# moyun/deneva

Measured on AMD Instinct MI355X. Metric: OCC-validated txns/sec, YCSB theta=0.9, higher is better.
Workload: dtype u64; 1 GPU; YCSB OCC epoch validation, 1048576 txns x 16 keys, zipf theta=0.9, 16,777,216-key table, 50% RO txns, 50% WR tuples; global_batch=1048576, keys_per_txn=16, parallelism=single GPU

## Files before the change

### deneva_amd/_abi.py

```python
from __future__ import annotations

import ctypes as C
import os

_HERE = os.path.dirname(os.path.abspath(__file__))
LIB_PATH = os.environ.get("DENEVA_AMD_LIB") or os.path.join(_HERE, "libdcc.so")

DCC_OK = 0
DCC_EIO = -5
DCC_ENOMEM = -12
DCC_ENODEV = -19
DCC_EINVAL = -22
DCC_ERANGE = -34
DCC_ECOMM = -70
DCC_ENOTSUP = -95

RD, WR, XP, SCAN = 0, 1, 2, 3
RC_RCOK, RC_ABORT, RC_WAIT = 0, 2, 3
KEY_RESERVED = 0xFFFFFFFFFFFFFFFF
GROUP_NONE = 0xFFFFFFFF
ACCESS_NONE = 0xFFFFFFFF
VTS_BASE, VTS_NONE = 0, 0xFFFFFFFFFFFFFFFF
DEVICE_PTRS = 0x1
OCC_APPEND_HISTORY = 0x2
OCC_DEFER_FINISH = 0x8
KEYS_U32 = 0x10
ACCTYPE_2BIT = 0x20
TN_U32 = 0x40
SHARD_SELF = 0x80
MAAT_READ_AND_PREWRITE = 0x4
ROW_NONE = 0xFFFFFFFFFFFFFFFF
UNIQUE_ID_BYTES = 128
EXCHANGE_FN = C.CFUNCTYPE(C.c_int, C.c_void_p, C.POINTER(C.c_uint8), C.c_uint64)
BACKOFF_REFERENCE, BACKOFF_NONE, BACKOFF_EXP = 0, 1, 2
ABORTQ_SORT_FULL = 0x1
LOCK_EX, LOCK_SH = 0, 1
WD_RUN, WD_GONE = 0x10, 0x11
OPT_RECHECK = 1
OPT_BATCH_MAX = 2
OPT_SOLVER = 5
OPT_SWEEP_LEVELS = 6
OPT_HIST_MERGE = 7
OPT_FAIL_RANK = 8
OPT_RO_SPLIT = 10
OPT_PIPELINE = 11
OPT_CALVIN_PATH = 12
OPT_COMM_SOLO = 13
OPT_PIPE_PARTITION = 14
OPT_PIPE_CHAIN = 15


class Batch(C.Structure):
    _fields_ = [
        ("n_txn", C.c_uint64),
        ("nnz", C.c_uint64),
        ("offsets", C.c_void_p),
        ("keys", C.c_void_p),
        ("acctype", C.c_void_p),
        ("start_tn", C.c_void_p),
        ("finish_tn", C.c_void_p),
        ("order", C.c_void_p),
        ("flags", C.c_uint32),
        ("reserved", C.c_uint32),
    ]


class Snapshot(C.Structure):
    _fields_ = [
        ("hist_top", C.c_void_p),
        ("active_off", C.c_void_p),
        ("active_idx", C.c_void_p),
    ]


class CalvinHeld(C.Structure):
    _fields_ = [("n", C.c_uint64), ("keys", C.c_void_p), ("acctype", C.c_void_p)]


class SelectOut(C.Structure):
    _fields_ = [
        ("cap_txn", C.c_uint64),
        ("cap_nnz", C.c_uint64),
        ("txn_base", C.c_uint64),
        ("nnz_base", C.c_uint64),
        ("offsets", C.c_void_p),
        ("keys", C.c_void_p),
        ("acctype", C.c_void_p),
        ("start_tn", C.c_void_p),
        ("finish_tn", C.c_void_p),
        ("order", C.c_void_p),
        ("src", C.c_void_p),
    ]


class WaitdieCarryArgs(C.Structure):
    _fields_ = [
        ("batch", C.POINTER(Batch)),
        ("ts", C.c_void_p),
        ("rc", C.c_void_p),
        ("pos", C.c_void_p),
        ("revive", C.c_void_p),
        ("src_in", C.c_void_p),
        ("fresh", C.POINTER(Batch)),
        ("fresh_ts", C.c_void_p),
        ("fresh_src_base", C.c_uint32),
        ("out", C.POINTER(SelectOut)),
        ("out_ts", C.c_void_p),
        ("out_rc", C.c_void_p),
        ("out_pos", C.c_void_p),
    ]


class AbortqParams(C.Structure):
    _fields_ = [
        ("cap_txn", C.c_uint64),
        ("cap_nnz", C.c_uint64),
        ("penalty", C.c_uint64),
        ("penalty_max", C.c_uint64),
        ("policy", C.c_uint32),
        ("flags", C.c_uint32),
    ]


class LocktabParams(C.Structure):
    _fields_ = [("cap_rows", C.c_uint64), ("flags", C.c_uint32), ("reserved", C.c_uint32)]


class Stats(C.Structure):
    _fields_ = [
        ("rounds", C.c_uint32),
        ("n_shards", C.c_uint32),
        ("n_commit", C.c_uint64),
        ("n_abort", C.c_uint64),
        ("n_readonly", C.c_uint64),
        ("nnz_w", C.c_uint64),
        ("alg_bytes", C.c_uint64),
        ("device_ms", C.c_double),
        ("total_ms", C.c_double),
        ("phase_ms", C.c_double * 4),
        ("phase_bytes", C.c_uint64 * 4),
        ("peel_prefix", C.c_uint64),
        ("n_survivors", C.c_uint64),
        ("fallback", C.c_uint32),
        ("fin_where", C.c_uint32),
    ]

    def as_dict(self) -> dict:
        out = {}
        for name, _ in self._fields_:
            v = getattr(self, name)
            out[name] = list(v) if name.startswith("phase_") else v
        return out


class YcsbParams(C.Structure):
    _fields_ = [
        ("n_txn", C.c_uint64),
        ("req_per_query", C.c_uint32),
        ("part_cnt", C.c_uint32),
        ("table_size", C.c_uint64),
        ("zipf_theta", C.c_double),
        ("txn_write_perc", C.c_double),
        ("tup_write_perc", C.c_double),
        ("part_per_txn", C.c_uint32),
        ("strict_ppt", C.c_uint32),
        ("first_part_local", C.c_uint32),
        ("chunk_txns", C.c_uint32),
        ("seed", C.c_uint64),
        ("n_threads", C.c_uint32),
        ("reserved", C.c_uint32),
    ]


class TpccParams(C.Structure):
    _fields_ = [
        ("n_txn", C.c_uint64),
        ("num_wh", C.c_uint32),
        ("part_cnt", C.c_uint32),
        ("perc_payment", C.c_double),
        ("wh_update", C.c_uint32),
        ("max_items", C.c_uint32),
        ("cust_per_dist", C.c_uint32),
        ("dist_per_wh", C.c_uint32),
        ("max_items_per_txn", C.c_uint32),
        ("part_per_txn", C.c_uint32),
        ("mpr", C.c_double),
        ("first_part_local", C.c_uint32),
        ("chunk_txns", C.c_uint32),
        ("seed", C.c_uint64),
        ("n_threads", C.c_uint32),
        ("reserved", C.c_uint32),
    ]


class FileInfo(C.Structure):
    _fields_ = [
        ("version", C.c_uint32),
        ("kind", C.c_uint32),
        ("sections", C.c_uint32),
        ("reserved", C.c_uint32),
        ("n_txn", C.c_uint64),
        ("nnz", C.c_uint64),
# ... 170 lines not shown
```

### deneva_amd/csrc/dcc_ctx.h

```cpp
#pragma once
#include <hip/hip_runtime.h>

#include <algorithm>
#include <chrono>
#include <cstring>
#include <memory>
#include <string>
#include <utility>
#include <vector>

#include "dcc.h"
#include "occ_history.h"

namespace dcc {
struct SwShard;
struct Slot;
}

struct dcc_ctx;


struct DevBuf {
  void* p = nullptr;
  size_t cap = 0;
// ... 15 lines not shown
    return *this;
  }
  ~DevBuf() { release(); }
  int ensure(dcc_ctx* c, size_t bytes, const char* what);
  void release();
};

struct RowTab {
  const char* name;
  DevBuf buf, ctl;
  uint32_t bits = 0;
  uint64_t rows = 0;
  uint32_t mask() const { return (uint32_t)((1ull << bits) - 1); }
  uint64_t size() const { return rows; }
  template <class P>
  int reserve(dcc_ctx* ctx, uint64_t want);
  int clear(dcc_ctx* ctx);
  template <class P>
  int set(dcc_ctx* ctx, const uint64_t* keys, const uint64_t* a, const uint64_t* b, uint64_t n);
  template <class P>
  int get(dcc_ctx* ctx, const uint64_t* keys, uint64_t* a, uint64_t* b, uint64_t n);
};

struct SegWork {
  static constexpr uint64_t TILE = 1024;
  static constexpr uint32_t C_WORDS = 84;
  static constexpr size_t AGG_BYTES = 40;
  DevBuf misc;
  DevBuf stp;
  DevBuf arec;
  DevBuf k[2], v[2];
  DevBuf stxn, sinfo, sts;
  DevBuf agg;
  DevBuf tdone;
  int reserve(dcc_ctx* ctx, uint64_t n, uint64_t nnz);
};

struct DevBatch {
  uint64_t n = 0, nnz = 0;
  const uint32_t* off = nullptr;
  const uint64_t* keys = nullptr;
  const uint8_t* acctype = nullptr;
  const uint64_t* start_tn = nullptr;
  const uint64_t* finish_tn = nullptr;
  const uint64_t* order = nullptr;
};

struct dcc_comm_state;
struct dcc_multi;

struct HistStore {
  DevBuf fk, ft;
  DevBuf skey, stn, hash;
  DevBuf bm;
  DevBuf nx, tcnt;
  uint64_t m = 0;
  uint32_t hbits = 0;
  bool built = true;
  bool mono = true;
  uint64_t max_tn = 0;
  uint64_t min_tn = ~0ull;
  uint64_t max_key = 0;
  bool chained = false;
  bool overflowed = false;
  uint64_t last_app = 0;
  void reset() {
    m = 0;
    built = false;
    mono = true;
    max_tn = 0;
    min_tn = ~0ull;
    max_key = 0;
  }
};

struct SubProb {
  uint64_t n = 0, nnz = 0, w_bound = 0;
  const uint32_t* off = nullptr;
  const uint64_t* keys = nullptr;
  const uint8_t* acctype = nullptr;
  uint8_t* state = nullptr;
  uint8_t* hasw = nullptr;
  bool hasw_global = false;
};
struct PeelInfo {
  uint64_t prefix = 0, survivors = 0;
};
struct SubBufs {
  DevBuf tid, off, keys, acctype, state;
};

struct dcc_abortq {
  dcc_ctx* owner = nullptr;
  dcc_abortq_params P{};
  struct Pool {
    DevBuf off, keys, at, src, cnt, due;
  } pool[2];
  DevBuf sk[2], sv[2], scratch;
  DevBuf ctl, part;
  DevBuf st_cnt, st_out;
  int cur = 0;
  uint64_t n = 0, nnz = 0;
  uint64_t seq = 0;
  uint64_t due_lo = ~0ull;
};

struct dcc_locktab {
  dcc_ctx* owner = nullptr;
  dcc_locktab_params P{};
  DevBuf tab[2];
  DevBuf ctl;
  DevBuf st_keys, st_type, st_cnt;
  DevBuf st_rc;
  int cur = 0;
  uint64_t n_slots = 0;
  uint64_t slots_used = 0;
  uint64_t rows_held = 0;
  uint64_t holds = 0;
  uint64_t rebuilds = 0;
  double pass_ms[3] = {};
  bool rebuilt = false;
};

struct LtEpoch {
  uint64_t n = 0;
  const uint32_t* off = nullptr;
  const uint64_t* keys = nullptr;
  const uint8_t* at = nullptr;
  const uint32_t* sid = nullptr;
  const uint8_t* state = nullptr;
  dcc::Slot* tab = nullptr;
  uint32_t lp = 0;
  const uint32_t* err = nullptr;
  unsigned grid = 1;
};

struct dcc_ctx {
  int device = 0;
  int n_cu = 256;
  hipStream_t own_stream = nullptr;
  hipStream_t stream = nullptr;
  hipEvent_t ev0 = nullptr, ev1 = nullptr;
  bool profiling = false;
  uint64_t recheck_max = 16384;
  uint32_t batch_max = 8;
  bool bars_used = false;
  int solver = 0;
  bool use_sweep() const { return solver != 1; }
  bool ro_split = true;
  bool ro_on = false;
  uint32_t wt_bits = 18;
  uint32_t wf_bits = 0;
  uint32_t sw_levels = 0;
  uint32_t sw_mode = 1;
  uint32_t sw_l1_last = ~0u;
  bool sw_debug = false;
  hipEvent_t pev[8] = {};
  std::string last_error;
  void* hmisc = nullptr;
  void* hpart = nullptr;
  struct GraphKey {
    const void *off, *keys, *acc;
    uint64_t n, nnz;
    const void* out_rc;
    bool dev_out;
    uint32_t levels;
    uint64_t gen;
    const void *start_tn, *finish_tn, *out_tn;
    uint32_t fin;
    bool operator==(const GraphKey& o) const {
      return off == o.off && keys == o.keys && acc == o.acc && n == o.n && nnz == o.nnz &&
             out_rc == o.out_rc && dev_out == o.dev_out && levels == o.levels && gen == o.gen &&
             start_tn == o.start_tn && finish_tn == o.finish_tn && out_tn == o.out_tn && fin == o.fin;
    }
  };
  hipGraphExec_t graph_exec = nullptr;
  struct CvGraphKey {
    const void *off, *keys, *acc, *order, *grp, *rc;
    uint64_t n, nnz, gen;
    uint32_t ulen, have_seq, bucket;
    uint8_t kp[112], op[112];
  };
  hipGraphExec_t cv_graph_exec = nullptr;
  CvGraphKey cv_graph_key{}, cv_seen_key{};
  bool cv_seen = false;
  bool cv_last_sorted = false, cv_last_bucket = false;
  uint64_t cv_spec_miss = 0;
  GraphKey graph_key{};
  uint64_t buf_gen = 0;
  void* hmisc_dev = nullptr;
  void* hpart_dev = nullptr;
  void* hdyn = nullptr;
  void* hdyn_dev = nullptr;
  static constexpr size_t HDYN_TOTALS = 256, HDYN_BYTES = 512;

  DevBuf misc;
  DevBuf part;
  DevBuf off, keys, acctype, start_tn, finish_tn, order;
  DevBuf nar_keys, nar_at, nar_tn;
  DevBuf table;
  DevBuf state, hasw, rc, stat;
  DevBuf cflag, bsum, tn;
  DevBuf dyn, fin_part;
  DevBuf gst;
  DevBuf hasw_scr;
  DevBuf sw_ctl, sw_status, sw_ckeys, sw_dbg;
  DevBuf sw_rec, sw_rk, sw_gtab, sw_fw, sw_aent, sw_mg;
  DevBuf sw_rflag, sw_ro, sw_wtab, sw_cw, sw_wtab_big;
  DevBuf sw_xcnt, sw_xsend, sw_xrec, sw_mcnt, sw_moff, sw_mkeys, sw_mat, sw_kill;
  SubBufs sw_list[2];
  DevBuf l_tid[2], l_coff[2], l_cent[2];
  HistStore hs[2];
  uint64_t hist_merge_min = 65536;
  DevBuf h_K[2], h_V[2], h_scr, h_bsum;
  DevBuf h_bm;
  bool h_bm_stale = true;
  uint32_t fin_tag = 0;
  DevBuf perm, calvin_a, calvin_b, calvin_c, calvin_d;
  DevBuf cv_scratch, cv_agg, cv_group, cv_wave, cv_pgx, cv_gsx, cv_gsize, cv_done, cv_maxl, cv_cwmax, cv_cwpos, cv_cwmark, cv_cwhot, cv_cwpa, cv_cwoa, cv_cwhelp, cv_cwrec2;
  DevBuf cv_seq_b, cv_ok, cv_len, cv_off2, cv_tsum;
  DevBuf held_keys, held_at;
  DevBuf cb_e, cb_out, cb_cnt, cb_small;
  DevBuf snap_top, snap_aoff, snap_aidx, snap_cnt;
  RowTab mt_rows{"maat"};
  uint64_t mt_new_last = 0;
  uint64_t mt_full_redo = 0;
  DevBuf mt_misc, mt_slot, mt_sval, mt_slot2, mt_sval2, mt_sfl, mt_stx, mt_txn, mt_agg;
  DevBuf mt_sflB, mt_stxB, mt_k1, mt_tcnt, mt_ul;
  DevBuf mt_lb;
  DevBuf mt_ptab;
  uint32_t mt_tag = 0;
  DevBuf ix_keys, ix_ord, ix_rows, ix_cnt, wv_buf, ix_scr, wv_hbuf, wv_obuf;
  DevBuf nw_misc, nw_sid, nw_list, nw_conf;
  DevBuf sel_misc, sel_part, sel_rc, sel_src, sel_out;
  std::vector<std::unique_ptr<dcc_abortq>> abortqs;
  uint32_t ix_bits = 0;
  uint64_t ix_nkeys = 0, ix_nrows = 0;
  double ix_last_ms = 0;
  uint64_t tnc = 0;

  dcc_comm_state* comm = nullptr;
  dcc_multi* multi = nullptr;
  int comm_ranks() const;
  bool sharded() const;
  bool comm_solo = false;
  int comm_allreduce_max_u8(uint8_t* dev, uint64_t n);
  int comm_allgather_u8(const uint8_t* send, uint8_t* recv, uint64_t bytes);
  int comm_rank() const;

  int fail(int code, const char* fmt, ...);
  int hip_fail(hipError_t e, const char* what);
  int reserve_occ(uint64_t n, uint64_t nnz, uint64_t nnz_w, uint32_t tw);
  void list_geometry(uint64_t n, uint32_t tw, uint64_t& seg_ts, uint64_t& seg_es) const;
  static uint64_t table_capacity(uint64_t nnz_w);
  uint64_t hist_size() const { return hs[0].m + hs[1].m; }
  int hist_grow_flat(HistStore& h, uint64_t need);
  dcc::HistInsert hist_insert_args(HistStore& h);
  void hist_note(HistStore& h, uint64_t lo_tn, uint64_t hi_tn);
  int hist_build(HistStore& h);
  int hist_prepare();
  dcc::HistView hist_view() const;
  int hist_append_epoch(const DevBatch& d, const uint64_t* tn_dev, uint64_t nnz_w, uint64_t n_cw);
  int check_batch(const dcc_batch* b, bool scan_offsets = true);
  int stage_batch(const dcc_batch* b, DevBatch& d);
  template <typename T>
  int stage(DevBuf& buf, const T* src, size_t bytes, bool dev, const char* what, const T*& out) {
    if (dev) {
      out = src;
      return DCC_OK;
    }
    if (int e = buf.ensure(this, bytes, what)) return e;
    if (bytes) {
      const hipError_t he = hipMemcpyAsync(buf.p, src, bytes, hipMemcpyHostToDevice, stream);
      if (he != hipSuccess) return hip_fail(he, what);
    }
    out = (const T*)buf.p;
    return DCC_OK;
  }
  int stage_held(const dcc_calvin_held* held, bool dev, const uint64_t*& keys, const uint8_t*& at);
  int device_prep(const DevBatch& d, uint32_t& maxlen, uint64_t& nnz_w, uint64_t p = 0,
                  uint64_t* nnz_w_prefix = nullptr);
  int read_partials(size_t bytes);
  int occ_epoch(const dcc_batch* b, uint8_t* out_rc, uint64_t* out_tn, dcc_stats* st);
  struct OccRun {
    uint64_t n_txn = 0;
    uint32_t flags = 0;
    uint8_t* out_rc = nullptr;
    uint64_t* out_tn = nullptr;
    DevBatch d;
    bool sh = false, dev_out = false, defer = false, sweep = false, want_tn = false;
    bool app = false, hist_on = false;
    bool whole = false;
    DevBatch full;
    bool replay = false, capturing = false, pending = false, active = false;
    uint32_t glv = 0, maxlen = 0, rounds = 0, handoffs = 0;
    uint64_t nnz_w = 0;
    int next_level = 0, serial_tail = -1;
    uint8_t* rc_dev = nullptr;
    uint32_t* cf = nullptr;
    uint64_t* tn_dev = nullptr;
    PeelInfo info;
    GraphKey gkey{};
    dcc_stats S;
    double t_wall0 = 0;
    uint64_t n_cw = 0;
    uint32_t fin_runs = 0;
    bool fin_later = false;
  };
  OccRun run;
  int occ_begin(const dcc_batch* b, uint8_t* out_rc, uint64_t* out_tn, bool async, bool fin_later = false);
  int pipe_finish(dcc_ctx* l, bool chained = false);
  int chain_enqueue(dcc_ctx* l, uint64_t seq, hipEvent_t after, bool reset);
  int chain_set(dcc_ctx* l, uint64_t seq);
  int chain_accept(dcc_ctx* l);
  uint64_t hist_room() const;
  DevBuf fin_ctl;
  DevBuf fdyn;
  void* hfin = nullptr;
  void* hfin_dev = nullptr;
  hipEvent_t ev_done = nullptr;
  uint32_t pipe_chain = 1;
  int occ_end(dcc_stats* st);
  int occ_final(bool async);
  struct OccPipe* pipe = nullptr;
  uint32_t pipe_lanes = 3;
  uint32_t pipe_part = 0;
// ... 155 lines not shown
```

### deneva_amd/csrc/dcc_ctx.hip

```cpp
#include <hip/hip_runtime.h>

#include <algorithm>
#include <chrono>
#include <cstdarg>
#include <cstdio>
#include <cstring>
#include <string>
#include <vector>

#include "dcc.h"
#include "dcc_ctx.h"
#include "dcc_env.h"
#include "radix_sort.h"
#include "dcc_device.h"
#include "occ_kernels.h"

using namespace dcc;

int dcc_ctx::fail(int code, const char* fmt, ...) {
  char buf[512];
  va_list ap;
  va_start(ap, fmt);
  vsnprintf(buf, sizeof buf, fmt, ap);
  va_end(ap);
// ... 56 lines not shown
  int n = 0;
  if (hipGetDeviceCount(&n) != hipSuccess) {
    (void)hipGetLastError();
    return 0;
  }
  int g = 0;
  for (int i = 0; i < n; i++) {
    hipDeviceProp_t p;
    if (hipGetDeviceProperties(&p, i) == hipSuccess && strncmp(p.gcnArchName, "gfx950", 6) == 0) g++;
  }
  return g;
}

extern "C" int dcc_version(void) { return 100; }

extern "C" const char* dcc_strerror(int code) {
  switch (code) {
    case DCC_OK: return "success";
    case DCC_EIO: return "HIP runtime failure";
    case DCC_ENOMEM: return "out of memory";
    case DCC_ENODEV: return "no usable gfx950 device";
    case DCC_EINVAL: return "invalid argument or malformed batch";
    case DCC_ERANGE: return "size exceeds an engine limit";
    case DCC_ECOMM: return "RCCL communicator failure";
    case DCC_ENOTSUP: return "not supported";
    default: return "unknown error";
  }
}

extern "C" const char* dcc_last_error(const dcc_ctx* ctx) {
  return ctx ? ctx->last_error.c_str() : "null context";
}

extern "C" int dcc_init(dcc_ctx** out, int device_id) {
  if (!out) return DCC_EINVAL;
  *out = nullptr;
  int ndev = 0;
  if (hipGetDeviceCount(&ndev) != hipSuccess || ndev == 0) {
    (void)hipGetLastError();
    return DCC_ENODEV;
  }
  if (device_id < 0) {
    if (hipGetDevice(&device_id) != hipSuccess) return DCC_ENODEV;
  }
  if (device_id >= ndev) return DCC_ENODEV;
  hipDeviceProp_t prop;
  if (hipGetDeviceProperties(&prop, device_id) != hipSuccess) return DCC_ENODEV;
  if (strncmp(prop.gcnArchName, "gfx950", 6) != 0) return DCC_ENODEV;
  if (hipSetDevice(device_id) != hipSuccess) return DCC_ENODEV;
  dcc_ctx* ctx = new dcc_ctx();
  ctx->device = device_id;
  ctx->n_cu = prop.multiProcessorCount;
  CK(hipStreamCreateWithFlags(&ctx->own_stream, hipStreamNonBlocking));
  ctx->stream = ctx->own_stream;
  CK(hipEventCreate(&ctx->ev0));
  CK(hipEventCreate(&ctx->ev1));
  for (auto& e : ctx->pev) CK(hipEventCreate(&e));
  CK(hipHostMalloc((void**)&ctx->hmisc, 16384, hipHostMallocDefault));
  CK(hipHostMalloc((void**)&ctx->hpart, 1 << 17, hipHostMallocDefault));
  CK(hipHostGetDevicePointer(&ctx->hmisc_dev, ctx->hmisc, 0));
  CK(hipHostGetDevicePointer(&ctx->hpart_dev, ctx->hpart, 0));
  ctx->hs[1].chained = true;
  CK(hipHostMalloc((void**)&ctx->hdyn, dcc_ctx::HDYN_BYTES, hipHostMallocDefault));
  CK(hipHostGetDevicePointer(&ctx->hdyn_dev, ctx->hdyn, 0));
  memset(ctx->hdyn, 0, dcc_ctx::HDYN_BYTES);
  int rc = ctx->misc.ensure(ctx, 16384, "misc");
  if (!rc) rc = ctx->part.ensure(ctx, 1 << 17, "partials");
  if (!rc && (hipMemset(ctx->misc.p, 0, 16384) != hipSuccess ||
              hipMemset(ctx->part.p, 0, 1 << 17) != hipSuccess))
    rc = DCC_EIO;
  if (rc) {
    dcc_destroy(ctx);
    return rc;
  }
  *out = ctx;
  return DCC_OK;
}

extern "C" void dcc_destroy(dcc_ctx* ctx) {
  if (!ctx) return;
  dcc_pipe_destroy(ctx);
  ctx->abortqs.clear();
  ctx->locktabs.clear();
  dcc_multi_destroy(ctx);
  (void)hipSetDevice(ctx->device);
  if (ctx->stream) (void)hipStreamSynchronize(ctx->stream);
  if (ctx->graph_exec) (void)hipGraphExecDestroy(ctx->graph_exec);
  if (ctx->cv_graph_exec) (void)hipGraphExecDestroy(ctx->cv_graph_exec);
  dcc_comm_destroy(ctx);
  if (ctx->hmisc) (void)hipHostFree(ctx->hmisc);
  if (ctx->hpart) (void)hipHostFree(ctx->hpart);
  if (ctx->hdyn) (void)hipHostFree(ctx->hdyn);
  if (ctx->hfin) (void)hipHostFree(ctx->hfin);
  if (ctx->ev_done) (void)hipEventDestroy(ctx->ev_done);
  if (ctx->ev0) (void)hipEventDestroy(ctx->ev0);
  if (ctx->ev1) (void)hipEventDestroy(ctx->ev1);
  for (auto& e : ctx->pev)
    if (e) (void)hipEventDestroy(e);
  if (ctx->own_stream) (void)hipStreamDestroy(ctx->own_stream);
  delete ctx;
}

extern "C" int dcc_set_profiling(dcc_ctx* ctx, int enable) {
  if (!ctx) return DCC_EINVAL;
  if (ctx->multi)
    for (int r = 0; r < dcc_multi_size(ctx); r++) dcc_multi_sub(ctx, r)->profiling = enable != 0;
  ctx->profiling = enable != 0;
  return DCC_OK;
}

int dcc_multi_set_fail_rank(dcc_ctx* ctx, int rank);

extern "C" int dcc_set_option(dcc_ctx* ctx, int option, int64_t value) {
  if (!ctx) return DCC_EINVAL;
  if (option == DCC_OPT_FAIL_RANK) {
    if (!ctx->multi) return ctx->fail(DCC_EINVAL, "DCC_OPT_FAIL_RANK: multi-GPU contexts only");
    return dcc_multi_set_fail_rank(ctx, (int)value);
  }
  if (option == DCC_OPT_PIPELINE) {
    if (value < 1 || value > 8) return DCC_EINVAL;
    dcc_pipe_drain(ctx);
    ctx->pipe_lanes = (uint32_t)value;
    return DCC_OK;
  }
  if (option == DCC_OPT_PIPE_PARTITION) {
    if (value != 0 && value != 1) return DCC_EINVAL;
    dcc_pipe_drain(ctx);
    ctx->pipe_part = (uint32_t)value;
    return DCC_OK;
  }
  if (option == DCC_OPT_PIPE_CHAIN) {
    if (value != 0 && value != 1) return DCC_EINVAL;
    dcc_pipe_drain(ctx);
    ctx->pipe_chain = (uint32_t)value;
    return DCC_OK;
  }
  if (ctx->multi)
    for (int r = 0; r < dcc_multi_size(ctx); r++) {
      const int e = dcc_set_option(dcc_multi_sub(ctx, r), option, value);
      if (e != DCC_OK) return e;
    }
  switch (option) {
    case DCC_OPT_RECHECK:
      if (value < 0) return DCC_EINVAL;
      ctx->recheck_max = (uint64_t)value;
      return DCC_OK;
    case DCC_OPT_SOLVER:
      if (value != 0 && value != 1 && value != 3) return DCC_EINVAL;
      ctx->solver = (int)value;
      return DCC_OK;
    case DCC_OPT_SWEEP_LEVELS:
      if (value < 0 || value > SW_MAX_LEVEL) return DCC_EINVAL;
      ctx->sw_levels = (uint32_t)value;
      return DCC_OK;
    case DCC_OPT_RO_SPLIT:
      if (value != 0 && value != 1 && (value < 4 || value > 24)) return DCC_EINVAL;
      ctx->ro_split = value != 0;
      ctx->wt_bits = value >= 4 ? (uint32_t)value : WT_BITS_DEFAULT;
      return DCC_OK;
    case DCC_OPT_HIST_MERGE:
      if (value < 1) return DCC_EINVAL;
      ctx->hist_merge_min = (uint64_t)value;
      return DCC_OK;
    case DCC_OPT_CALVIN_PATH:
      if (value < 0 || value > 2) return DCC_EINVAL;
      ctx->cv_path = (int)value;
      return DCC_OK;
    case DCC_OPT_COMM_SOLO:
      if (value != 0 && value != 1) return DCC_EINVAL;
      if (ctx->comm) return ctx->fail(DCC_EINVAL, "DCC_OPT_COMM_SOLO: set before dcc_comm_init");
      ctx->comm_solo = value != 0;
      return DCC_OK;
    case DCC_OPT_BATCH_MAX:
      if (value < 1 || value > 32) return DCC_EINVAL;
      ctx->batch_max = (uint32_t)value;
      return DCC_OK;
    default: return DCC_EINVAL;
  }
}

extern "C" int dcc_set_stream(dcc_ctx* ctx, void* s) {
  if (!ctx) return DCC_EINVAL;
  if (ctx->multi) return ctx->fail(DCC_ENOTSUP, "multi-GPU context: one stream per sub-context");
  ctx->stream = s ? (hipStream_t)s : ctx->own_stream;
  return DCC_OK;
}

extern "C" int dcc_reserve(dcc_ctx* ctx, uint64_t max_txn, uint64_t max_nnz) {
  if (!ctx) return DCC_EINVAL;
  if (ctx->multi)
    for (int r = 0; r < dcc_multi_size(ctx); r++) {
      const int e = dcc_reserve(dcc_multi_sub(ctx, r), max_txn, max_nnz);
      if (e != DCC_OK) return e;
    }
  (void)hipSetDevice(ctx->device);
  const uint32_t tw = ROUND_CAP / MAX_TXN_LEN;
  int rc = ctx->state.ensure(ctx, max_txn + 16, "state");
  if (!rc) rc = ctx->hasw.ensure(ctx, max_txn + 16, "hasw");
  if (!rc) rc = ctx->rc.ensure(ctx, max_txn + 16, "rc");
  if (!rc) rc = ctx->nowait_reserve(max_txn, max_nnz, true);
  if (!rc) rc = ctx->select_reserve(max_txn, max_nnz);
  if (!rc) rc = ctx->tso_reserve(max_txn, max_nnz, true);
  if (!rc) rc = ctx->mvcc_reserve(max_txn, max_nnz, true, true);
  if (!rc) rc = ctx->waitdie_reserve(max_txn, max_nnz, true);
  if (!rc) rc = ctx->carry_reserve(max_txn, max_nnz);
  if (rc) return rc;
  return ctx->reserve_occ(max_txn, max_nnz, max_nnz, tw);
}

int dcc_ctx::hist_grow_flat(HistStore& h, uint64_t need) {
  dcc_ctx* ctx = this;
  if (need * 8 <= h.fk.cap && need * 8 <= h.ft.cap && (!h.chained || need * 4 <= h.nx.cap)) return DCC_OK;
  if (h.chained && need >= HIST_NIL) return fail(DCC_ENOMEM, "history delta level of %llu pairs",
                                                 (unsigned long long)need);
  const uint64_t want = std::max<uint64_t>(need + need / 2, 4096);
  for (DevBuf* b : {&h.fk, &h.ft, &h.nx}) {
    if (b == &h.nx && !h.chained) continue;
    const uint64_t w = b == &h.nx ? 4 : 8;
    DevBuf nb;
    CR(nb.ensure(this, want * w, "history pairs"));
    if (h.m) CK(hipMemcpyAsync(nb.p, b->p, h.m * w, hipMemcpyDeviceToDevice, stream));
    CK(hipStreamSynchronize(stream));
    *b = std::move(nb);
  }
  return DCC_OK;
}

void dcc_ctx::hist_note(HistStore& h, uint64_t lo_tn, uint64_t hi_tn) {
  if (lo_tn < h.max_tn) h.mono = false;
  h.max_tn = std::max(h.max_tn, hi_tn);
  h.min_tn = std::min(h.min_tn, lo_tn);
  h.built = false;
}

int dcc_ctx::hist_build(HistStore& h) {
  dcc_ctx* ctx = this;
  if (h.built) return DCC_OK;
  h_bm_stale = true;
  if (h.m == 0 && !h.chained) {
    h.built = true;
    h.mono = true;
    return DCC_OK;
  }
  static const uint64_t slots_per_pair = [] {
    const char* e = DCC_ENV("DCC_HIST_SLOTS");
    return e && atoi(e) >= 2 ? (uint64_t)atoi(e) : 4ull;
  }();
  uint64_t need = slots_per_pair * h.m;
  if (h.chained)
    need = std::max<uint64_t>({need, 65536,
                               4 * (std::max<uint64_t>(hist_merge_min, hs[0].m / 4) + h.last_app)});
  if (h.overflowed) need = std::max<uint64_t>(need, 4ull << h.hbits);
  h.hbits = 4;
  while ((1ull << h.hbits) < need) h.hbits++;
  const uint64_t mm = std::max<uint64_t>(h.m, 1);
  CR(h.skey.ensure(this, mm * 8, "history keys"));
  CR(h.stn.ensure(this, mm * 8, "history tns"));
  CR(h.hash.ensure(this, 32ull << h.hbits, "history table"));
  CR(h.tcnt.ensure(this, 16, "history table overflow flag"));
  CR(h.bm.ensure(this, (1u << HIST_BM_LOG) / 8, "history key bitmap"));
  CK(hipMemsetAsync(h.tcnt.p, 0, 16, stream));
  if (h.m == 0) {
    CK(hipMemsetAsync(h.hash.p, 0xFF, 32ull << h.hbits, stream));
    CK(hipMemsetAsync(h.bm.p, 0, (1u << HIST_BM_LOG) / 8, stream));
    h.built = true;
    h.mono = true;
    h.overflowed = false;
    return DCC_OK;
  }
  for (int q = 0; q < 2; q++) {
    CR(h_K[q].ensure(this, h.m * 8, "history sort keys"));
    CR(h_V[q].ensure(this, h.m * 4, "history sort values"));
  }
  CR(h_scr.ensure(this, rs_scratch_words(h.m) * 4, "history sort scratch"));
  HistBuild b{h.m,
              (const uint64_t*)h.fk.p,
              (const uint64_t*)h.ft.p,
              h.mono,
              {(uint64_t*)h_K[0].p, (uint64_t*)h_K[1].p},
              {(uint32_t*)h_V[0].p, (uint32_t*)h_V[1].p},
              (uint32_t*)h_scr.p,
              (uint64_t*)h.skey.p,
              (uint64_t*)h.stn.p,
              (uint64_t*)h.hash.p,
              h.hbits,
              h.max_key ? 64u - (uint32_t)__builtin_clzll(h.max_key) : 1u,
              64u - (uint32_t)__builtin_clzll(h.max_tn | 1ull),
              (uint32_t*)h.tcnt.p};
  if (hist_build_level(b, stream)) CK(hipGetLastError());
  launch_hist_bm((const uint64_t*)h.fk.p, h.m, (uint32_t*)h.bm.p, stream);
  CK(hipGetLastError());
  CK(hipMemcpyAsync(hmisc, h.tcnt.p, 4, hipMemcpyDeviceToHost, stream));
  CK(hipStreamSynchronize(stream));
  if (*(const uint32_t*)hmisc) {
    h.overflowed = true;
    return hist_build(h);
  }
  h.overflowed = false;
  h.built = true;
  return DCC_OK;
}

HistInsert dcc_ctx::hist_insert_args(HistStore& h) {
  return HistInsert{(const uint64_t*)h.fk.p, (const uint64_t*)h.ft.p, (uint64_t*)h.hash.p,
                    (uint32_t*)h.nx.p, (uint32_t*)h.bm.p, (uint32_t*)h_bm.p, (uint32_t*)h.tcnt.p,
                    h.hbits, 0u};
// ... 410 lines not shown
```

### deneva_amd/csrc/occ_driver.hip

```cpp
#include <hip/hip_runtime.h>

#include <algorithm>
#include <chrono>
#include <cstdio>
#include <cstdlib>
#include <cstring>
#include <vector>

#include "dcc.h"
#include "dcc_ctx.h"
#include "dcc_device.h"
#include "dcc_env.h"
#include "occ_kernels.h"

using namespace dcc;

static uint64_t next_pow2(uint64_t x) {
  uint64_t p = 1;
  while (p < x) p <<= 1;
  return p;
}

uint64_t dcc_ctx::table_capacity(uint64_t nnz_w) {
  return std::max<uint64_t>(1024, next_pow2(nnz_w + nnz_w / 4 + 1));
// ... 88 lines not shown
  BuildArgs ba{sp.n, tw_b, sp.off, sp.keys, sp.acctype, tab, mask, sp.state, sp.hasw, err};
  if (prof) CK(hipEventRecord(pev[0], stream));
  launch_build(ba, (unsigned)n_cu * 16, stream);
  CK(hipGetLastError());
  if (sh && sp.hasw_global) CR(comm_allreduce_max_u8(sp.hasw, sp.n));
  if (prof) CK(hipEventRecord(pev[1], stream));

  int cur = 0;
  uint32_t rt = 1;
  uint32_t k = 0;
  uint64_t m_bound = sp.n;
  uint32_t rounds = 0;
  const unsigned max_grid = (unsigned)n_cu * 8;
  const unsigned resident_grid = (unsigned)n_cu * 4;
  uint32_t batch = std::min<uint32_t>(sp.n > 65536 ? 2 : 4, batch_max);
  bool done = false;
  while (!done) {
    const uint32_t k0 = k;
    for (uint32_t q = 0; q < batch; q++, k++) {
      const bool first = k == 0;
      const unsigned long long* prev = first ? nullptr : &ring[((k - 1) % CTR_RING) * NSEG];
      if (!first) {
        PubArgs pa;
        pa.m_in = prev;
        pa.tw = tw;
        pa.kill_flag = sh ? one : &kflag[(k - 1) % CTR_RING];
        pa.force = 0;
        pa.state = sp.state;
        if (rt > MAX_ROUND_TAG) {
          launch_retag(tab, cap, stream);
          rt = 1;
          pa.kill_flag = one;
          pa.force = 1;
        }
        pa.r = rt;
        pa.tid = (const uint32_t*)l_tid[cur].p;
        pa.coff = (const uint32_t*)l_coff[cur].p;
        pa.cent = (const uint64_t*)l_cent[cur].p;
        pa.seg_ts = seg_ts;
        pa.seg_es = seg_es;
        pa.tab = tab;
        pa.err = err;
        launch_pub(pa, m_bound, (unsigned)n_cu * 2, stream);
      }
      RoundArgs ra;
      ra.m_in = prev;
      ra.m = sp.n;
      ra.tw = tw;
      ra.r = rt;
      ra.k = k + 1;
      ra.end_total = 0;
      ra.tid = first ? nullptr : (const uint32_t*)l_tid[cur].p;
      ra.coff = first ? sp.off : (const uint32_t*)l_coff[cur].p;
      ra.keys = sp.keys;
      ra.acctype = sp.acctype;
      ra.cent = first ? nullptr : (const uint64_t*)l_cent[cur].p;
      ra.seg_ts = seg_ts;
      ra.seg_es = seg_es;
      ra.tab = tab;
      ra.mask = mask;
      ra.state = sp.state;
      ra.tid_out = (uint32_t*)l_tid[cur ^ 1].p;
      ra.coff_out = (uint32_t*)l_coff[cur ^ 1].p;
      ra.cent_out = (uint64_t*)l_cent[cur ^ 1].p;
      ra.ctr = &ring[(k % CTR_RING) * NSEG];
      ra.ctr_zero = &ring[((k + 1) % CTR_RING) * NSEG];
      ra.kill_flag = &kflag[k % CTR_RING];
      ra.kill_zero = &kflag[(k + 1) % CTR_RING];
      const bool recheck = !sh && !first && m_bound <= recheck_max;
      ra.bar = recheck ? (GridBar*)(bars + (k % CTR_RING) * 16) : nullptr;
      bars_used |= recheck;
      ra.bar_zero = (uint32_t*)(bars + ((k + 1) % CTR_RING) * 16);
      ra.gst = gstat;
      ra.err = err;
      launch_round(ra, first, m_bound, recheck ? resident_grid : max_grid, stream);
      if (sh) {
        CR(comm_allreduce_max_u8(gstat, sp.n));
        launch_decide(sp.state, gstat, sp.n, st_abort(k + 1), &und[k % CTR_RING],
                      &und[(k + 1) % CTR_RING], stream);
      }
      if (prof && first) CK(hipEventRecord(pev[2], stream));
      cur ^= 1;
      rt++;
    }
    CK(hipGetLastError());
    CK(hipMemcpyAsync(hmisc, ring, CTR_RING * NSEG * 8, hipMemcpyDeviceToHost, stream));
    if (sh) CK(hipMemcpyAsync((char*)hmisc + MISC_UND, und, CTR_RING * 4, hipMemcpyDeviceToHost, stream));
    CK(hipStreamSynchronize(stream));
    const unsigned long long* hr = (const unsigned long long*)hmisc;
    const uint32_t* hu = (const uint32_t*)((const char*)hmisc + MISC_UND);
    for (uint32_t q = k0; q < k; q++) {
      uint64_t mq = 0;
      for (uint32_t g = 0; g < NSEG; g++) mq += hr[(q % CTR_RING) * NSEG + g] >> CTR_E_BITS;
      if (sh ? hu[q % CTR_RING] == 0 : mq == 0) {
        rounds = q + 1;
        done = true;
        break;
      }
      m_bound = mq;
    }
    if (!done && k > sp.n + 2) return fail(DCC_EIO, "fixed point did not converge");
    batch = std::min<uint32_t>(batch * 2, batch_max);
  }
  if (prof) CK(hipEventRecord(pev[4], stream));
  rounds_out = rounds;
  return DCC_OK;
}

static constexpr size_t SW_PREP_OFF = 32768;
static constexpr size_t SW_HCTL = 13312;
static constexpr uint32_t SW_PMAX_TOP = 65536;
static uint32_t sw_pmax(int level, int mode) {
  static const std::vector<uint32_t> ov = [] {
    std::vector<uint32_t> v;
    if (const char* e = DCC_ENV("DCC_SW_PMAX"))
      for (const char* c = e; *c;) {
        char* x;
        const unsigned long p = strtoul(c, &x, 10);
        if (x == c) break;
        v.push_back((uint32_t)std::min<unsigned long>(std::max<unsigned long>(p, SW_T), SW_PMAX_TOP));
        c = *x ? x + 1 : x;
      }
    return v;
  }();
  if (level < (int)ov.size()) return ov[level];
  if (mode == 2) {
    if (level == 0) return 1024u;
    return level >= 4 ? SW_PMAX_TOP : (8192u << (level - 1));
  }
  if (mode) {
    if (level == 0) return 1024u;
    if (level == 1) return 3072u;
    return level >= 5 ? SW_PMAX_TOP : (8192u << (level - 2));
  }
  return level >= 6 ? SW_PMAX_TOP : (1024u << level);
}
static size_t sw_ctl_bytes() { return (SW_MAX_LEVEL + 2) * sizeof(SwLevel) + 64; }
static uint32_t sw_budget_bits(int level, int mode) {
  uint32_t b = 12;
  while (b < SW_GBITS_MAX && (1ull << b) < 4ull * sw_pmax(level, mode) * 16) b++;
  return b;
}
static uint32_t sw_budget(int level, int mode) { return 1u << (sw_budget_bits(level, mode) - 2); }
static uint32_t sw_gbits(int level, int mode) {
  static const int ov = [] {
    const char* c = DCC_ENV("DCC_SW_GBITS");
    return c ? atoi(c) : 0;
  }();
  uint32_t b = ov > 0 ? (uint32_t)ov : (level == 0 ? 18u : 19u);
  b = std::max(b, sw_budget_bits(level, mode));
  return std::min<uint32_t>(b, SW_GBITS_MAX);
}

int dcc_ctx::sweep_reserve(const DevBatch& d) {
  const uint64_t tiles = SW_PMAX_TOP / SW_T;
  sw_debug = DCC_ENV("DCC_SW_DEBUG") != nullptr;
  if (sw_debug) {
    CR(sw_dbg.ensure(this, (4096 + 4 * 256 * 8 + 4 * 64 * 8) * 8, "sweep debug"));
    dcc_ctx* ctx = this;
    CK(hipMemsetAsync(sw_dbg.p, 0, (4096 + 4 * 256 * 8 + 4 * 64 * 8) * 8, stream));
  }
  CR(sw_ctl.ensure(this, sw_ctl_bytes(), "sweep control"));
  CR(sw_status.ensure(this, ((d.n + 63) / 64 + 64) * 16 + (4ull * n_cu + 64) * 8,
                        "sweep survivor bits + tile counts"));
  CR(sw_ckeys.ensure(this, ((1ull << SW_GBITS_MAX) / 32 + (1ull << SW_BLOOM_LOG) / 32) * 4 +
                                (1ull << SW_GBITS_MAX) * 8,
                     "sweep committed set"));
  CR(sw_rec.ensure(this, tiles * sizeof(SwRec), "sweep tile records"));
  CR(sw_rk.ensure(this, tiles * SW_OVF * 4, "sweep tile-list overflow"));
  CR(sw_gtab.ensure(this, 2 * (1ull << SW_GBITS_MAX) * 8, "sweep key tables"));
  CR(sw_fw.ensure(this, 2 * (1ull << SW_GBITS_MAX) * 4, "sweep first writer / last accessor"));
  CR(sw_aent.ensure(this, 2 * (1ull << (SW_GBITS_MAX - 1)) * 4, "sweep access entries"));
  CR(sw_mg.ensure(this, SW_PMAX_TILES * 8, "sweep tile commit masks"));
  if (ro_on) {
    const uint64_t n64 = (d.n + 63) / 64 + 32;
    CR(sw_rflag.ensure(this, (2 * n64 + 4ull * n_cu + 64) * 8, "sweep read-only survivor bits"));
    CR(sw_ro.ensure(this, d.n * sizeof(RoEnt) + 64, "sweep read-only list"));
    CR(sw_wtab.ensure(this, sizeof(WrSlot) << wt_bits, "committed-writer table"));
    CR(sw_cw.ensure(this, d.n * 4 + 64, "committed writers"));
  }
  for (SubBufs& b : sw_list) {
    CR(b.tid.ensure(this, d.n * 4 + 16, "sweep list tid"));
    CR(b.off.ensure(this, (d.n + 1) * 4 + 16, "sweep list offsets"));
    CR(b.keys.ensure(this, std::max<uint64_t>(8, d.nnz * 8), "sweep list keys"));
    CR(b.acctype.ensure(this, std::max<uint64_t>(16, d.nnz), "sweep list acctype"));
    CR(b.state.ensure(this, d.n + 16, "sweep list state"));
  }
  return DCC_OK;
}

int dcc_ctx::sweep_enqueue(const DevBatch& d, int l0, int l1, const SwShard* shl, bool resume,
                           bool tail_serial) {
  dcc_ctx* ctx = this;
  SwLevel* ctl = (SwLevel*)sw_ctl.p;
  uint32_t* abandon = (uint32_t*)(ctl + SW_MAX_LEVEL + 1);
  uint32_t* err = (uint32_t*)misc.p;
  const uint32_t n = (uint32_t)d.n;
  static const unsigned fgrid_ov = [] {
    const char* e = DCC_ENV("DCC_SW_FGRID");
    return e ? (unsigned)atoi(e) : 0u;
  }();
  const unsigned fgrid = fgrid_ov ? fgrid_ov : (unsigned)std::max<uint64_t>(1, 4ull * n_cu);
  static const unsigned fgrid1_ov = [] {
    const char* e = DCC_ENV("DCC_SW_FGRID1");
    return e ? (unsigned)atoi(e) : 0u;
  }();
  uint64_t* gtab0 = (uint64_t*)sw_gtab.p;
  uint32_t* cbits_d = (uint32_t*)sw_ckeys.p;
  uint32_t* bloom_d = cbits_d + (1u << SW_GBITS_MAX) / 32;
  uint64_t* ckeys_d = (uint64_t*)(bloom_d + (1u << SW_BLOOM_LOG) / 32);
  const uint64_t n64 = (d.n + 63) / 64;
  uint64_t* sflag_d = (uint64_t*)sw_status.p;
  unsigned long long* tcount_d = (unsigned long long*)(sflag_d + n64 + 32);
  unsigned long long* bsum_d = tcount_d + n64 + 32;
  const bool ros = ro_on && (!shl || shl->full_off);
  const int rmode = ros ? (int)sw_mode : 0;
  uint32_t* const wctl = abandon;
  for (int l = l0; l < l1; l++) {
    const bool top = l == 0;
    SwList in;
    if (top) {
      in = SwList{nullptr, d.off, d.keys, d.acctype, d.nnz};
    } else {
      const SubBufs& b = sw_list[(l - 1) & 1];
      in = SwList{(const uint32_t*)b.tid.p, (const uint32_t*)b.off.p, (const uint64_t*)b.keys.p,
                  (const uint8_t*)b.acctype.p, d.nnz};
    }
    SubBufs& out = sw_list[l & 1];
    SwLevel* lv = ctl + l;
    const uint32_t* mdev = top ? nullptr : &lv->m;
    const uint32_t pmax = sw_pmax(l, rmode);
    const uint64_t tiles = (std::min<uint64_t>(pmax, d.n) + SW_T - 1) / SW_T;
    uint32_t* fw = (uint32_t*)sw_fw.p;
    uint32_t* la = fw + (1u << SW_GBITS_MAX);
    uint32_t* aent = (uint32_t*)sw_aent.p;
    uint32_t* apos = aent + (1u << (SW_GBITS_MAX - 1));
    const SwList sin = shl ? shl->serial : in;
    const uint32_t* smdev = shl ? shl->m_dev : mdev;
    const uint32_t sm_host = (shl && !shl->m_dev) ? shl->P : n;
    SwPreArgs pa{sin, smdev, sm_host, pmax, top ? (const uint8_t*)state.p : nullptr,
                 (SwRec*)sw_rec.p, (uint32_t*)sw_rk.p,
                 gtab0 + (size_t)(l & 1) * (1ull << SW_GBITS_MAX), sw_gbits(l, rmode),
                 sw_budget(l, rmode), fw, la, aent, apos, abandon, err, nullptr};
    if (sw_debug && l < 4) pa.dbg = (uint64_t*)sw_dbg.p + 4096 + 4 * 256 * 8 + (size_t)l * 64 * 8;
    const bool serial_part = !(resume && l == l0);
    if (serial_part) {
      launch_sw_pre(pa, (unsigned)tiles, stream);
      launch_sw_rows(pa, (unsigned)tiles, stream);
    }
    SwSeqArgs sa{smdev, sm_host, pmax, top ? 1 : 0, (const SwRec*)sw_rec.p, (const uint32_t*)sw_rk.p,
                 gtab0 + (size_t)(l & 1) * (1ull << SW_GBITS_MAX), sw_gbits(l, rmode),
                 (uint8_t*)state.p, (uint8_t*)hasw.p,
                 cbits_d, ckeys_d, bloom_d, lv, lv + 1, (uint32_t*)out.off.p, (uint64_t*)sw_mg.p,
                 abandon, err, nullptr};
    if (sw_debug && l < 4) sa.dbg = (uint64_t*)sw_dbg.p + (size_t)l * 1024;
    if (ros) {
      sa.cw_list = (uint32_t*)sw_cw.p;
      sa.cw_count = wctl + 4;
    }
    if (serial_part) launch_sw_seq(sa, stream);
    if (tail_serial && l == l1 - 1) break;
    SwCoutArgs ca{sin,     aent,    apos,    (const uint64_t*)sw_mg.p, lv, cbits_d, ckeys_d,
                  bloom_d, abandon, smdev, sm_host, shl ? 0 : 1};
    if (top && serial_part) {
      const bool whole = shl && shl->full_off;
      ca.prep_off = whole ? shl->full_off : d.off;
      ca.prep_n = d.n;
      ca.prep_at = whole ? shl->full_at : d.acctype;
      ca.prep_nnz = whole ? shl->full_nnz : d.nnz;
      ca.prep_part = (PrepPart*)((char*)hpart_dev + SW_PREP_OFF);
      ca.hasw = (uint8_t*)hasw.p;
      ca.prep_err = err;
      if (ros) {
        ca.wclear = (uint4*)sw_wtab.p;
        ca.wclear_n16 = (sizeof(WrSlot) << wt_bits) / 16;
      }
    }
    launch_sw_cout(ca, (unsigned)std::min<uint64_t>((pa.budget + 1023) / 1024, 4ull * n_cu), stream);
    SwFilterArgs fa;
    fa.in = in;
    fa.m_dev = mdev;
    fa.m_host = n;
    fa.cand_state = top ? 1 : 0;
    fa.level = (uint32_t)l;
    fa.gtab = gtab0 + (size_t)(l & 1) * (1ull << SW_GBITS_MAX);
    fa.gbits = sw_gbits(l, rmode);
    fa.cbits = cbits_d;
    fa.bloom = bloom_d;
    fa.ckeys = ckeys_d;
    fa.sflag = sflag_d;
    fa.tcount = tcount_d;
    fa.bsum = bsum_d;
    const unsigned lgrid = (!top && fgrid1_ov) ? std::min(fgrid1_ov, fgrid) : fgrid;
    fa.nblocks = lgrid;
    fa.lv = lv;
    fa.lv_next = lv + 1;
    fa.state = (uint8_t*)state.p;
    fa.hasw = (uint8_t*)hasw.p;
    fa.tid_out = (uint32_t*)out.tid.p;
    fa.off_out = (uint32_t*)out.off.p;
    fa.keys_out = (uint64_t*)out.keys.p;
    fa.acc_out = (uint8_t*)out.acctype.p;
    fa.abandon = abandon;
    fa.abandon_out = abandon;
    fa.abandon_min = 65536;
    fa.abandon_num = top ? 1 : 3;
    fa.abandon_den = 4;
    fa.gclear = gtab0 + (size_t)((l + 1) & 1) * (1ull << SW_GBITS_MAX);
    fa.gclear_n = 1ull << sw_gbits(l + 1, rmode);
    fa.fw_clear = fw;
    fa.la_clear = la;
    fa.err = err;
    fa.dbg = (sw_debug && l < 4) ? (uint64_t*)sw_dbg.p + 4096 + (size_t)l * 256 * 8 : nullptr;
    fa.cdbg = pa.dbg ? pa.dbg + 32 : nullptr;
    fa.kill_out = shl ? shl->kill_out : nullptr;
    fa.kill_in = shl ? shl->kill_all : nullptr;
    fa.kill_ranks = shl ? (uint32_t)comm_ranks() : 0u;
    fa.kill_stride = shl ? shl->kill_words : 0u;
    fa.ro_split = (ros && top) ? 1 : 0;
    fa.rflag = (uint64_t*)sw_rflag.p;
    fa.rtcount = (unsigned long long*)(fa.rflag + n64 + 32);
    fa.rbsum = fa.rtcount + n64 + 32;
    fa.ro_out = (RoEnt*)sw_ro.p;
    fa.ro_count = wctl + 2;
    if (top && profiling) CK(hipEventRecord(pev[1], stream));
    launch_sw_filter(fa, lgrid, stream);
    if (top && profiling) CK(hipEventRecord(pev[2], stream));
    if (shl) {
      CR(comm_allgather_u8((const uint8_t*)shl->kill_out, (uint8_t*)shl->kill_all, shl->kill_words * 8));
      if (top && !shl->full_off) CR(comm_allreduce_max_u8((uint8_t*)hasw.p, d.n));
      launch_sw_apply(fa, lgrid, stream);
    }
    launch_sw_compact(fa, lgrid, stream);
  }
  CK(hipGetLastError());
  return DCC_OK;
}

int dcc_ctx::sweep_sharded(const DevBatch& d, int& next_level) {
  dcc_ctx* ctx = this;
  const int R = comm_ranks(), me = comm_rank();
  SwLevel* ctl = (SwLevel*)sw_ctl.p;
  const uint32_t* abandon = (const uint32_t*)(ctl + SW_MAX_LEVEL + 1);
  CR(sw_xcnt.ensure(this, 64ull * R + 64, "sweep exchange counts"));
  for (int l = 0; l < SW_MAX_LEVEL - 1; l++) {
    next_level = l;
    const bool top = l == 0;
    SwList in;
    if (top) {
      in = SwList{nullptr, d.off, d.keys, d.acctype, d.nnz};
    } else {
      const SubBufs& b = sw_list[(l - 1) & 1];
      in = SwList{(const uint32_t*)b.tid.p, (const uint32_t*)b.off.p, (const uint64_t*)b.keys.p,
                  (const uint8_t*)b.acctype.p, d.nnz};
    }
    uint32_t* cnt = (uint32_t*)sw_xcnt.p;
    CK(hipMemsetAsync(cnt, 0, 4ull * (R + 2), stream));
    launch_sw_share(top ? nullptr : &ctl[l].m, (uint32_t)d.n, abandon, top ? d.off : in.off,
                    sw_pmax(l, 0), (uint32_t)me, cnt, stream);
    CR(comm_allreduce_max_u8((uint8_t*)cnt, 4ull * (R + 2)));
    std::vector<uint32_t> hc(R + 2);
    CK(hipMemcpyAsync(hc.data(), cnt, 4ull * (R + 2), hipMemcpyDeviceToHost, stream));
    CK(hipStreamSynchronize(stream));
    const uint32_t m = hc[0];
    if (hc[1]) return DCC_OK;
    if (m == 0) return DCC_OK;
    const uint32_t P = std::min<uint32_t>(sw_pmax(l, 0), m);
    const uint32_t* share = hc.data() + 2;
    uint64_t total = 0, before = 0;
    for (int r = 0; r < R; r++) {
      if (r < me) before += share[r];
      total += share[r];
    }
    uint32_t maxshare = 0;
    for (int r = 0; r < R; r++) maxshare = std::max(maxshare, share[r]);
    const uint64_t chunk = std::max<uint64_t>(1, maxshare) * 12;
    CR(sw_xsend.ensure(this, chunk, "sweep exchange send"));
    CR(sw_xrec.ensure(this, chunk * R, "sweep exchange records"));
    CR(sw_mcnt.ensure(this, 8ull * (P + 1) + 64, "sweep merge counts"));
    CR(sw_moff.ensure(this, 4ull * (P + 1) + 64, "sweep merged offsets"));
    CR(sw_mkeys.ensure(this, std::max<uint64_t>(64, total * 8), "sweep merged keys"));
    CR(sw_mat.ensure(this, std::max<uint64_t>(64, total), "sweep merged types"));
    const uint64_t kw = (m + 63) / 64 + 1;
    CR(sw_kill.ensure(this, kw * 8 * (R + 1) + 64, "sweep kill bits"));
    uint32_t* xrec = (uint32_t*)sw_xrec.p;
    uint32_t* mcnt = (uint32_t*)sw_mcnt.p;
    CK(hipMemsetAsync(sw_xsend.p, 0xFF, chunk, stream));
    CK(hipMemsetAsync(mcnt, 0, 4ull * (P + 1), stream));
    launch_sw_merge(in, P, (uint32_t*)sw_xsend.p, 0, 0, nullptr, nullptr, nullptr, nullptr,
                    nullptr, true, stream);
    CR(comm_allgather_u8((const uint8_t*)sw_xsend.p, (uint8_t*)xrec, chunk));
    (void)before;
    launch_sw_merge(in, P, xrec, 0, (uint32_t)(R * (chunk / 12)), mcnt, mcnt + (P + 1),
                    (uint32_t*)sw_moff.p, (uint64_t*)sw_mkeys.p, (uint8_t*)sw_mat.p, false, stream);
    CK(hipGetLastError());
    SwShard shl{};
    shl.serial = SwList{top ? nullptr : in.tid, (const uint32_t*)sw_moff.p,
                        (const uint64_t*)sw_mkeys.p, (const uint8_t*)sw_mat.p, total};
    shl.P = P;
    shl.kill_out = (uint64_t*)sw_kill.p;
    shl.kill_all = (uint64_t*)sw_kill.p + kw;
    shl.kill_words = kw;
    CR(sweep_enqueue(d, l, l + 1, &shl));
  }
  next_level = SW_MAX_LEVEL - 1;
  return DCC_OK;
}


int dcc_ctx::sweep_sharded_full(const DevBatch& d, const DevBatch& full, int l0, int L) {
  dcc_ctx* ctx = this;
  const int R = comm_ranks();
  SwLevel* ctl = (SwLevel*)sw_ctl.p;
  uint32_t* err = (uint32_t*)misc.p;
  uint64_t cap = d.n, wmax = 0;
  std::vector<uint64_t> words(std::max(L, 1));
  for (int l = 0; l < L; l++) {
    words[l] = (cap + 63) / 64 + 1;
    wmax = std::max(wmax, words[l]);
    cap = std::min<uint64_t>(cap, std::max<uint64_t>(65536, l == 0 ? (cap + 3) / 4 : (cap * 3 + 3) / 4));
  }
  CR(sw_kill.ensure(this, wmax * 8 * (R + 1) + 64, "sweep kill bits"));
  const uint32_t pm = sw_pmax(SW_MAX_LEVEL - 1, ro_on ? (int)sw_mode : 0);
  CR(sw_moff.ensure(this, 4ull * (std::min<uint64_t>(pm, d.n) + 1) + 64, "sweep serial offsets"));
  CR(sw_mkeys.ensure(this, 8ull * std::min<uint64_t>(pm, d.n) * MAX_TXN_LEN + 64, "sweep serial keys"));
  CR(sw_mat.ensure(this, std::min<uint64_t>(pm, d.n) * MAX_TXN_LEN + 64, "sweep serial types"));
  for (int l = l0; l < L; l++) {
    SwShard shl{};
    if (l == 0) {
      shl.serial = SwList{nullptr, full.off, full.keys, full.acctype, full.nnz};
      shl.P = (uint32_t)d.n;
    } else {
      const SubBufs& b = sw_list[(l - 1) & 1];
      launch_sw_sgather((const uint32_t*)b.tid.p, &ctl[l].m, sw_pmax(l, ro_on ? (int)sw_mode : 0), full.off, full.keys,
                        full.acctype, full.nnz, (uint32_t*)sw_moff.p, (uint64_t*)sw_mkeys.p,
                        (uint8_t*)sw_mat.p, err, stream);
      CK(hipGetLastError());
      shl.serial = SwList{(const uint32_t*)b.tid.p, (const uint32_t*)sw_moff.p, (const uint64_t*)sw_mkeys.p,
                          (const uint8_t*)sw_mat.p, std::min<uint64_t>(pm, d.n) * MAX_TXN_LEN};
      shl.m_dev = &ctl[l].m;
    }
    shl.kill_out = (uint64_t*)sw_kill.p;
    shl.kill_all = (uint64_t*)sw_kill.p + wmax;
    shl.kill_words = words[l];
    shl.full_off = full.off;
    shl.full_at = full.acctype;
    shl.full_nnz = full.nnz;
// ... 218 lines not shown
    HistStore& D = hs[1];
    if (tot[1] > d.nnz) return fail(DCC_EIO, "history append: %llu writes > %llu accesses",
                                    (unsigned long long)tot[1], (unsigned long long)d.nnz);
    if (tot[1]) {
      D.m += tot[1];
      D.max_key = std::max<uint64_t>(D.max_key, tot[2]);
      D.last_app = tot[1];
      const bool b = D.built;
      hist_note(D, tnc + 1, tnc + r.n_cw);
      D.built = b;
    }
    if (tot[3]) {
      D.overflowed = true;
      D.built = false;
    }
  }
  tnc += r.n_cw;
  return DCC_OK;
}

int dcc_ctx::chain_set(dcc_ctx* l, uint64_t seq) {
  dcc_ctx* ctx = this;
  CR(fin_ctl.ensure(this, sizeof(FinCtl), "chained finish control"));
  launch_fin_ctl_set((FinCtl*)fin_ctl.p, tnc, hs[1].m, seq, l->stream);
  CK(hipGetLastError());
  return DCC_OK;
}

int dcc_ctx::sweep_ro(const DevBatch& d0, bool big, bool scan, uint64_t nnz_w, const DevBatch* full) {
  const DevBatch& d = full ? *full : d0;
  dcc_ctx* ctx = this;
  uint32_t* wctl = (uint32_t*)((SwLevel*)sw_ctl.p + SW_MAX_LEVEL + 1);
  WrTab wt{(WrSlot*)sw_wtab.p, wt_bits, WT_PROBES, wctl + 1};
  if (big) {
    uint32_t bits = 10;
    while (bits < 31 && (1ull << bits) < 2 * std::max<uint64_t>(nnz_w, 1)) bits++;
    CR(sw_wtab_big.ensure(this, sizeof(WrSlot) << bits, "committed-writer fallback table"));
    CK(hipMemsetAsync(sw_wtab_big.p, 0xFF, sizeof(WrSlot) << bits, stream));
    wt = WrTab{(WrSlot*)sw_wtab_big.p, bits, 1u << bits, wctl + 3};
  }
  SwWallArgs wa{d.n, d.off, d.keys, d.acctype, d.nnz, (const uint8_t*)state.p,
                (const uint8_t*)hasw.p, scan ? nullptr : (const uint32_t*)sw_cw.p, wctl + 4, wt};
  launch_sw_wall(wa, (unsigned)std::max<uint64_t>(1, std::min<uint64_t>(scan ? 4096 : 256, (d.n + 255) / 256)),
                 stream);
  SwRoArgs ra{(const RoEnt*)sw_ro.p, wctl + 2, d.keys, wt, (uint8_t*)state.p, full ? full->off : nullptr};
  static const uint64_t ro_grid = [] {
    const char* e = DCC_ENV("DCC_SW_ROGRID");
    return e && atoi(e) > 0 ? (uint64_t)atoi(e) : 1024ull;
  }();
  launch_sw_ro(ra, (unsigned)std::max<uint64_t>(1, std::min<uint64_t>(ro_grid, (d.n + 255) / 256)), stream);
  CK(hipGetLastError());
  return DCC_OK;
}

int dcc_ctx::occ_epoch(const dcc_batch* b, uint8_t* out_rc, uint64_t* out_tn, dcc_stats* st) {
  CR(occ_begin(b, out_rc, out_tn, false));
  return occ_end(st);
}

static double wall_ms() {
  return std::chrono::duration<double, std::milli>(std::chrono::steady_clock::now().time_since_epoch())
      .count();
}

int dcc_ctx::occ_begin(const dcc_batch* b, uint8_t* out_rc, uint64_t* out_tn, bool async, bool fin_later) {
  dcc_ctx* ctx = this;
  if (run.active) return fail(DCC_EINVAL, "an epoch of this context is still in flight");
  run = OccRun{};
  OccRun& r = run;
  r.out_rc = out_rc;
  r.out_tn = out_tn;
  r.sh = sharded();
  r.t_wall0 = wall_ms();
  CR(check_batch(b, !(use_sweep() && !r.sh)));
  r.n_txn = b->n_txn;
  r.flags = b->flags;
  r.dev_out = (b->flags & DCC_DEVICE_PTRS) != 0;
  r.defer = (b->flags & DCC_OCC_DEFER_FINISH) != 0;
  if (fin_pending)
    return fail(DCC_EINVAL, "an epoch validated with DCC_OCC_DEFER_FINISH awaits dcc_occ_finish_epoch");
  if (r.defer && (out_tn || (b->flags & DCC_OCC_APPEND_HISTORY)))
    return fail(DCC_EINVAL, "DCC_OCC_DEFER_FINISH: commit tn and history come from dcc_occ_finish_epoch");
  r.S.n_shards = (uint32_t)comm_ranks();
  if (b->n_txn == 0) {
    if (r.defer) {
      fin_d = DevBatch{};
      fin_nnz_w = 0;
      fin_pending = true;
    }
    r.active = true;
    return DCC_OK;
  }
  DevBatch& d = r.d;
  const bool self_shard = r.sh && (b->flags & DCC_SHARD_SELF);
  r.whole = self_shard && use_sweep();
  if (self_shard) {
    dcc_batch sb;
    CR(shard_stage(b, (uint32_t)comm_rank(), (uint32_t)comm_ranks(), sb, r.whole ? &r.full : nullptr));
    CR(stage_batch(&sb, d));
  } else {
    CR(stage_batch(b, d));
  }
  r.sweep = use_sweep();
  const bool sh = r.sh, sweep = r.sweep;
  ro_on = sweep && ro_split && (!sh || r.whole);
  if (sweep) CR(sweep_reserve(d));
  CR(state.ensure(this, d.n + 16, "state"));
  CR(hasw.ensure(this, d.n + 16, "hasw"));
  CR(rc.ensure(this, d.n + 16, "rc"));
  r.want_tn = out_tn != nullptr || (b->flags & DCC_OCC_APPEND_HISTORY);
  r.app = (b->flags & DCC_OCC_APPEND_HISTORY) != 0;
  r.fin_later = fin_later && r.want_tn;
  const bool app_here = r.app && !r.fin_later;
  if (r.want_tn) {
    CR(cflag.ensure(this, d.n * 4, "cflag"));
    {
      const size_t old_cap = fin_part.cap;
      CR(fin_part.ensure(this, fin_part_bytes(d.n), "finish look-back words"));
      if (fin_part.cap != old_cap || fin_tag + 4 >= (1u << 30)) {
        CK(hipMemsetAsync(fin_part.p, 0, fin_part.cap, stream));
        fin_tag = 0;
      }
    }
    CR(tn.ensure(this, d.n * 8, "tn"));
  }
  CR(dyn.ensure(this, sizeof(OccDyn), "epoch parameters"));
  r.hist_on = d.start_tn && hist_size() > 0;
  if (r.hist_on || app_here) CR(hist_prepare());
  if (app_here) CR(hist_grow_flat(hs[1], hs[1].m + d.nnz));
  static_assert(sizeof(OccDyn) <= HDYN_TOTALS, "epoch parameters overlap the totals");
  {
    OccDyn& y = *(OccDyn*)hdyn;
    y.tnc = tnc;
    y.fin_tag = ++fin_tag;
    y.hist_m = hs[1].m;
    y.app_k = app_here ? (uint64_t*)hs[1].fk.p : nullptr;
    y.app_t = app_here ? (uint64_t*)hs[1].ft.p : nullptr;
    y.ins = app_here ? hist_insert_args(hs[1]) : HistInsert{};
    y.view = hist_view();
  }
  if (app_here) hs[1].built = false;
  const bool graph_ok = sweep && !profiling && !sw_debug && !sh && !DCC_ENV("DCC_NO_GRAPH");
  if (ro_on && !sw_levels && !sh) {
    if (sw_l1_last <= 6144) sw_mode = 2;
    else if (sw_l1_last > 8192) sw_mode = 1;
  } else {
    sw_mode = 1;
  }
  r.glv = sw_levels ? sw_levels : (ro_on ? (sw_mode == 2 ? 2u : 3u) : 4u);
  r.gkey = GraphKey{d.off, d.keys, d.acctype, d.n, d.nnz, r.dev_out ? out_rc : nullptr, r.dev_out,
                    r.glv | (ro_on ? 0x80u | (wt_bits << 8) : 0u), buf_gen,
                    d.start_tn, d.finish_tn, r.dev_out ? out_tn : (const void*)(uintptr_t)(out_tn != nullptr),
                    (r.want_tn ? 1u : 0u) | (r.app ? 2u : 0u) | (r.hist_on ? 4u : 0u) |
                        (r.fin_later ? 8u : 0u)};
  r.replay = graph_ok && graph_exec && r.gkey == graph_key;
  struct CaptureGuard {
    hipStream_t s;
    bool* on;
    ~CaptureGuard() {
      if (*on) {
        *on = false;
        hipGraph_t g = nullptr;
        (void)hipStreamEndCapture(s, &g);
        if (g) (void)hipGraphDestroy(g);
        (void)hipGetLastError();
      }
    }
  } capture_guard{stream, &r.capturing};
  if (graph_ok && !r.replay) {
    if (graph_exec) {
      (void)hipGraphExecDestroy(graph_exec);
      graph_exec = nullptr;
    }
    CK(hipStreamBeginCapture(stream, hipStreamCaptureModeThreadLocal));
    r.capturing = true;
  }
  if (!r.replay && !r.capturing) CK(hipEventRecord(ev0, stream));

  if (!sweep) CR(device_prep(d, r.maxlen, r.nnz_w));
  if (!r.replay) {
    uint32_t* mw = (uint32_t*)misc.p;
    FillArgs fa{};
    fa.job[fa.n++] = FillJob{mw, 1, 0u};
    fa.job[fa.n++] = FillJob{mw + 1, 1, 1u};
    fa.job[fa.n++] = FillJob{mw + 2, 14, 0u};
    fa.job[fa.n++] = FillJob{(uint32_t*)state.p, (d.n + 3) / 4, 0u};
    fa.job[fa.n++] = FillJob{(uint32_t*)dyn.p, sizeof(OccDyn) / 4, 0u, (const uint32_t*)hdyn_dev};
    if (sweep) {
      fa.job[fa.n++] = FillJob{(uint32_t*)sw_ctl.p, sw_ctl_bytes() / 4, 0u};
      const int m0 = ro_on ? (int)sw_mode : 0;
      fa.job[fa.n++] = FillJob{(uint32_t*)sw_gtab.p, (1ull << sw_gbits(0, m0)) * 2, 0xFFFFFFFFu};
      fa.job[fa.n++] = FillJob{(uint32_t*)sw_fw.p, 1ull << sw_gbits(0, m0), 0xFFFFFFFFu};
      fa.job[fa.n++] = FillJob{(uint32_t*)sw_fw.p + (1u << SW_GBITS_MAX), 1ull << sw_gbits(0, m0), 0u};
    }
    launch_fill(fa, stream);
  }

  if (r.hist_on && !r.replay) {
    HistArgs ha{d.n, d.nnz, d.off, d.keys, d.acctype, d.start_tn, d.finish_tn, (const OccDyn*)dyn.p, 0u,
                (uint8_t*)state.p, (uint32_t*)misc.p};
    launch_hist(ha, stream);
  }
  if (sh && d.start_tn) CR(comm_allreduce_max_u8((uint8_t*)state.p, d.n));

  SubProb top;
  top.n = d.n;
  top.nnz = d.nnz;
  top.off = d.off;
  top.keys = d.keys;
  top.acctype = d.acctype;
  top.state = (uint8_t*)state.p;
  top.hasw = (uint8_t*)hasw.p;
  top.hasw_global = true;
  top.w_bound = r.nnz_w;
  bars_used = false;
  if (sweep) {
    if (profiling) CK(hipEventRecord(pev[0], stream));
    r.next_level = (int)std::min<uint32_t>(r.glv, SW_MAX_LEVEL - 1);
    if (!sh && r.next_level >= 2) r.serial_tail = r.next_level - 1;
    if (r.whole) {
      CR(sweep_sharded_full(d, r.full, 0, r.next_level));
      if (ro_on) CR(sweep_ro(d, false, false, 0, &r.full));
    } else if (sh) {
      CR(sweep_sharded(d, r.next_level));
    } else if (!r.replay) {
      CR(sweep_enqueue(d, 0, r.next_level, nullptr, false, r.serial_tail >= 0));
      if (ro_on) CR(sweep_ro(d, false, false, 0));
    }
  } else {
    CR(occ_rounds(top, r.maxlen, profiling, r.rounds));
  }
  if (profiling) CK(hipEventRecord(pev[3], stream));

  r.rc_dev = (r.dev_out && out_rc) ? out_rc : (uint8_t*)rc.p;
  r.cf = r.want_tn ? (uint32_t*)cflag.p : nullptr;
  r.tn_dev = r.want_tn ? ((r.dev_out && out_tn) ? out_tn : (uint64_t*)tn.p) : nullptr;
  const bool go_async = async && r.replay;
  CR(occ_final(go_async));
  r.pending = go_async;
  r.active = true;
  return DCC_OK;
}

int dcc_ctx::occ_final(bool async) {
  dcc_ctx* ctx = this;
  OccRun& r = run;
  const DevBatch& d = r.d;
  auto copy_out = [&]() -> int {
    if (r.dev_out) return DCC_OK;
    if (r.out_rc) CK(hipMemcpyAsync(r.out_rc, rc.p, d.n, hipMemcpyDeviceToHost, stream));
    if (r.out_tn && !r.fin_later) CK(hipMemcpyAsync(r.out_tn, tn.p, d.n * 8, hipMemcpyDeviceToHost, stream));
    return DCC_OK;
  };
  if (r.replay) {
    r.replay = false;
    if (r.want_tn) r.fin_runs = 1;
    CK(hipEventRecord(ev0, stream));
    CK(hipGraphLaunch(graph_exec, stream));
    CR(copy_out());
    CK(hipEventRecord(ev1, stream));
    if (!async) CK(hipStreamSynchronize(stream));
    return DCC_OK;
  }
  GatherArgs ga{};
  auto job = [&](void* hdst_dev, const void* src, size_t bytes) {
    ga.job[ga.n++] = CopyJob{(const uint32_t*)src, (uint32_t*)hdst_dev, (uint32_t)(bytes / 4)};
  };
  job(hmisc_dev, misc.p, 64);
  job((char*)hmisc_dev + MISC_BARS, (char*)misc.p + MISC_BARS, CTR_RING * 16);
  if (r.sweep) job((char*)hmisc_dev + SW_HCTL, sw_ctl.p, sw_ctl_bytes());
  FinalArgs fa{d.n, (const uint8_t*)state.p, (const uint8_t*)hasw.p, r.rc_dev, r.cf,
               (FinalPart*)hpart_dev};
  launch_final(fa, ga, stream);
  if (r.want_tn && !r.fin_later)
    launch_fin(OccFinArgs{d.n, d.nnz, r.cf, d.off, d.keys, d.acctype, (uint64_t*)fin_part.p,
                          (const OccDyn*)dyn.p, r.tn_dev, (uint64_t*)((char*)hdyn_dev + HDYN_TOTALS),
                          r.fin_runs++ ? ++fin_tag : 0u, 0u},
               stream);
  CK(hipGetLastError());
  if (r.capturing) {
    r.capturing = false;
    hipGraph_t g = nullptr;
    CK(hipStreamEndCapture(stream, &g));
    const hipError_t ie = hipGraphInstantiate(&graph_exec, g, nullptr, nullptr, 0);
    (void)hipGraphDestroy(g);
    if (ie != hipSuccess) {
      graph_exec = nullptr;
      return fail(DCC_EIO, "hipGraphInstantiate: %s", hipGetErrorString(ie));
    }
    graph_key = r.gkey;
    CK(hipEventRecord(ev0, stream));
    CK(hipGraphLaunch(graph_exec, stream));
  }
  CR(copy_out());
  CK(hipEventRecord(ev1, stream));
  CK(hipStreamSynchronize(stream));
  return DCC_OK;
}

int dcc_ctx::occ_end(dcc_stats* st) {
  dcc_ctx* ctx = this;
  OccRun& r = run;
  if (!r.active) return fail(DCC_EINVAL, "no epoch of this context is in flight");
  struct Inactive {
    bool* a;
    ~Inactive() { *a = false; }
  } inactive{&r.active};
// ... 296 lines not shown
```

### deneva_amd/csrc/occ_kernels.h

```cpp
#pragma once
#include <hip/hip_runtime.h>
#include <stdint.h>
#include <string>
#include "occ_history.h"

namespace dcc {

struct Slot;

constexpr int TILE_CAP = 1024;
constexpr int ROUND_CAP = 512;
constexpr int TILE_WAVES = 4;
constexpr int PUB_LDS = 2048;
constexpr int PUB_WAVES = 16;
constexpr uint32_t MAX_TXN_LEN = 64;
constexpr uint32_t MAX_ROUND_TAG = 61;

constexpr uint32_t CTR_E_BITS = 38;
constexpr unsigned long long CTR_E_MASK = (1ull << CTR_E_BITS) - 1ull;
constexpr uint32_t CTR_RING = 64;
constexpr uint32_t NSEG = 8;

constexpr uint32_t ERR_OFFSETS = 1;
constexpr uint32_t ERR_TILE = 2;
// ... 131 lines not shown
__host__ __device__ constexpr uint32_t sw_ppack(uint32_t id) {
  return ((id >> 5) << 7) | (id & 31u);
}
__host__ __device__ constexpr uint32_t sw_ipack(uint32_t id, uint32_t t) {
  return ((id >> 5) << 13) | ((id & 31u) << 6) | t;
}
constexpr uint32_t SW_ID_NONE = 1u << SW_GBITS_MAX;
constexpr uint32_t SW_A_NONE = sw_apack(SW_ID_NONE, false);
constexpr uint32_t SW_P_NONE = sw_ppack(SW_ID_NONE);
__host__ __device__ constexpr uint32_t sw_idummy(uint32_t q) {
  return sw_ipack(SW_ID_NONE + 32u * (1u + (q & 63u)), 0);
}
constexpr uint32_t SWM_VALID = 1, SWM_PRE = 2, SWM_HASW = 4, SWM_STOP = 16;
constexpr uint32_t SW_RC = 3;
constexpr uint32_t SW_RC_I = 2;
struct SwRec {
  uint32_t probe[SW_PL];
  uint32_t ins[SW_IL];
  uint64_t dep[SW_T];
  uint32_t meta[SW_T];
  uint32_t rtid[SW_T];
  uint32_t pspan[SW_T];
  uint64_t seg[SW_RC][SW_T];
  uint32_t np, ni;
  uint32_t hdr;
  uint32_t pad[5 + 128];
};
constexpr uint32_t SWH_PLONG = 1, SWH_ILONG = 2, SWH_STOP = 4;
struct SwLevel {
  uint32_t m;
  uint32_t acc;
  uint32_t pos;
  uint32_t ccount;
  uint32_t ticket;
  uint32_t pad[3];
};
struct SwList {
  const uint32_t* tid;
  const uint32_t* off;
  const uint64_t* keys;
  const uint8_t* acctype;
  uint64_t nnz;
};
struct __attribute__((aligned(16))) WrSlot {
  uint64_t key;
  uint32_t tid;
  uint32_t pad;
};
struct WrTab {
  WrSlot* slot;
  uint32_t bits;
  uint32_t probes;
  uint32_t* full;
};
constexpr uint32_t WT_PROBES = 64;
constexpr uint32_t WT_BITS_DEFAULT = 18;
struct RoEnt {
  uint32_t tid, s, e, pad;
};
struct SwRoArgs {
  const RoEnt* ro;
  const uint32_t* ro_count;
  const uint64_t* keys;
  WrTab wt;
  uint8_t* state;
  const uint32_t* full_off;
};
struct SwWallArgs {
  uint64_t n;
  const uint32_t* off;
  const uint64_t* keys;
  const uint8_t* acctype;
  uint64_t nnz;
  const uint8_t* state;
  const uint8_t* hasw;
  const uint32_t* cw_list;
  const uint32_t* cw_count;
  WrTab wt;
};
void launch_sw_ro(const SwRoArgs& a, unsigned grid, hipStream_t st);
void launch_sw_wall(const SwWallArgs& a, unsigned grid, hipStream_t st);

struct SwPreArgs {
  SwList in;
  const uint32_t* m_dev;
  uint32_t m_host;
  uint32_t p_max;
  const uint8_t* state;
  SwRec* rec;
  uint32_t* lst_ovf;
  uint64_t* gtab;
  uint32_t gbits;
  uint32_t budget;
  uint32_t* first_w;
  uint32_t* last_a;
  uint32_t* aent;
  uint32_t* apos;
  const uint32_t* abandon;
  uint32_t* err;
  uint64_t* dbg;
};
struct SwSeqArgs {
  const uint32_t* m_dev;
  uint32_t m_host;
  uint32_t p_max;
  int write_hasw;
  const SwRec* rec;
  const uint32_t* lst_ovf;
  const uint64_t* gtab;
  uint32_t gbits;
  uint8_t* state;
  uint8_t* hasw;
  uint32_t* cbits_out;
  uint64_t* ckeys_out;
  uint32_t* bloom_out;
  SwLevel* lv;
  SwLevel* lv_next;
  uint32_t* next_off;
  uint64_t* mg;
  const uint32_t* abandon;
  uint32_t* err;
  uint64_t* dbg;
  uint32_t* cw_list;
  uint32_t* cw_count;
};
#ifndef DCC_SW_PREP_BLOCKS
#define DCC_SW_PREP_BLOCKS 1024
#endif
constexpr unsigned SW_PREP_BLOCKS = DCC_SW_PREP_BLOCKS;
struct SwCoutArgs {
  SwList in;
  const uint32_t* aent;
  const uint32_t* apos;
  const uint64_t* mg;
  SwLevel* lv;
  uint32_t* cbits_out;
  uint64_t* ckeys_out;
  uint32_t* bloom_out;
  const uint32_t* abandon;
  const uint32_t* m_dev;
  uint32_t m_host;
  int skip_done;
  uint32_t cout_grid;
  const uint32_t* prep_off;
  uint64_t prep_n;
  const uint8_t* prep_at;
  uint64_t prep_nnz;
  PrepPart* prep_part;
  uint8_t* hasw;
  uint4* wclear;
  uint64_t wclear_n16;
  uint32_t* prep_err;
};
struct SwFilterArgs {
  SwList in;
  const uint32_t* m_dev;
  uint32_t m_host;
  int cand_state;
  uint32_t level;
  const uint64_t* gtab;
  uint32_t gbits;
  const uint32_t* cbits;
  const uint32_t* bloom;
  const uint64_t* ckeys;
  SwLevel* lv;
  SwLevel* lv_next;
  uint8_t* state;
  uint8_t* hasw;
  uint64_t* sflag;
  unsigned long long* tcount;
  unsigned long long* bsum;
  uint32_t nblocks;
  uint32_t* tid_out;
  uint32_t* off_out;
  uint64_t* keys_out;
  uint8_t* acc_out;
  const uint32_t* abandon;
  uint32_t* abandon_out;
  uint32_t abandon_min, abandon_num, abandon_den;
  uint64_t* kill_out;
  const uint64_t* kill_in;
  uint32_t kill_ranks;
  uint64_t kill_stride;
  int ro_split;
  uint64_t* rflag;
  unsigned long long* rtcount;
  unsigned long long* rbsum;
  RoEnt* ro_out;
  uint32_t* ro_count;
  uint64_t* gclear;
  uint64_t gclear_n;
  uint32_t* fw_clear;
  uint32_t* la_clear;
  uint32_t* err;
  uint64_t* dbg;
  uint64_t* cdbg;
};
struct SwShard {
  SwList serial;
  const uint32_t* m_dev;
  uint32_t P;
  uint64_t* kill_out;
  uint64_t* kill_all;
  uint64_t kill_words;
  const uint32_t* full_off;
  const uint8_t* full_at;
  uint64_t full_nnz;
};
void launch_sw_sgather(const uint32_t* tid, const uint32_t* m_dev, uint32_t p_max,
                       const uint32_t* full_off, const uint64_t* full_keys, const uint8_t* full_at,
                       uint64_t full_nnz, uint32_t* soff, uint64_t* skeys, uint8_t* sat,
                       uint32_t* err, hipStream_t st);
void launch_sw_pre(const SwPreArgs& a, unsigned grid, hipStream_t st);
void launch_sw_seq(const SwSeqArgs& a, hipStream_t st);
void launch_sw_rows(const SwPreArgs& a, unsigned grid, hipStream_t st);
void launch_sw_cout(const SwCoutArgs& a, unsigned grid, hipStream_t st);
void launch_sw_filter(const SwFilterArgs& a, unsigned grid, hipStream_t st);
void launch_sw_compact(const SwFilterArgs& a, unsigned grid, hipStream_t st);
void launch_sw_apply(const SwFilterArgs& a, unsigned grid, hipStream_t st);
void launch_sw_share(const uint32_t* m_dev, uint32_t m_host, const uint32_t* abandon,
                     const uint32_t* off, uint32_t p_max, uint32_t rank, uint32_t* cnt,
                     hipStream_t st);
void launch_sw_merge(const SwList& in, uint32_t P, uint32_t* xbuf, uint32_t xoff_words,
                     uint32_t n_all, uint32_t* cnt, uint32_t* cur, uint32_t* moff,
                     uint64_t* mkeys, uint8_t* mat, bool export_only, hipStream_t st);

struct WidenArgs {
  uint64_t n, nnz;
  const uint32_t* k32;
  uint64_t* k64;
  const uint8_t* a2;
  uint8_t* a8;
  const uint32_t *s32, *f32;
  uint64_t *s64, *f64;
};
void launch_widen(const WidenArgs& a, unsigned n_cu, hipStream_t st);
void launch_copy16(const void* src, void* dst, uint64_t bytes, unsigned grid, hipStream_t st);
void launch_copy16_chunk(const void* src, void* dst, uint64_t bytes, unsigned grid, hipStream_t st);

struct FillJob {
  uint32_t* p;
  uint64_t words;
  uint32_t value;
  const uint32_t* src = nullptr;
};
struct FillArgs {
  FillJob job[12];
  uint32_t n;
};
void launch_fill(const FillArgs& a, hipStream_t st);
struct CopyJob {
  const uint32_t* src;
  uint32_t* dst;
  uint32_t words;
};
struct GatherArgs {
  CopyJob job[12];
  uint32_t n;
};
void launch_gather(const GatherArgs& a, hipStream_t st);

void launch_prep(const uint32_t* off, uint64_t n, const uint8_t* at, uint64_t nnz, uint64_t p,
                 PrepPart* part, hipStream_t st);
void launch_hist(const HistArgs& a, hipStream_t st);
void launch_build(const BuildArgs& a, unsigned max_grid, hipStream_t st);
void launch_round(const RoundArgs& a, bool from_keys, uint64_t m_bound, unsigned max_grid,
                  hipStream_t st);
void launch_retag(Slot* tab, uint64_t cap, hipStream_t st);
void launch_pub(const PubArgs& a, uint64_t m_bound, unsigned max_grid, hipStream_t st);
void launch_final(const FinalArgs& a, const GatherArgs& g, hipStream_t st);
void launch_decide(uint8_t* state, uint8_t* gst, uint64_t n, uint8_t abort_byte, uint32_t* und,
                   uint32_t* und_next, hipStream_t st);
struct FinCtl {
  uint64_t tnc, hist_m, seq, pad;
};
struct OccFinArgs {
  uint64_t n, nnz;
  const uint32_t* cflag;
  const uint32_t* off;
  const uint64_t* keys;
  const uint8_t* acctype;
  uint64_t* part;
  const OccDyn* dyn;
  uint64_t* tn;
  uint64_t* totals;
  uint32_t tag;
  uint32_t var;
  FinCtl* ctl;
  uint64_t seq;
  const uint8_t* state;
  const uint32_t* err;
  const uint32_t* wfull;
  uint64_t cap;
};
void launch_fin(const OccFinArgs& a, hipStream_t st);
void launch_fin_prep(const uint32_t* src, OccDyn* dyn, const FinCtl* ctl, uint64_t seq, hipStream_t st);
void launch_fin_ctl_set(FinCtl* ctl, uint64_t tnc, uint64_t hist_m, uint64_t seq, hipStream_t st);
uint64_t fin_part_bytes(uint64_t n);
std::string fin_diag(const void* words, uint64_t n, uint32_t tag);
void launch_commit_tn(const uint32_t* cflag, uint64_t n, uint64_t* bsum, uint64_t tnc,
                      uint64_t* tn, hipStream_t st);
void launch_finish_flags(const uint8_t* final_rc, const uint8_t* state, const uint8_t* hasw,
                         uint64_t n, uint32_t* cflag, uint32_t* cnt, hipStream_t st);

}
```

### deneva_amd/csrc/occ_pipe.cpp

```cpp
#include <hip/hip_ext.h>
#include <hip/hip_runtime.h>

#include <algorithm>
#include <deque>
#include <string>
#include <unordered_map>
#include <vector>

#include "dcc.h"
#include "dcc_ctx.h"

struct OccPipe {
  std::vector<dcc_ctx*> lanes;
  struct Flight {
    uint64_t ticket;
    int lane;
    uint64_t seq;
    bool chain;
    bool app;
    uint64_t res;
  };
  std::deque<Flight> flight;
  struct Result {
    int rc;
    dcc_stats st;
    std::string err;
  };
  std::unordered_map<uint64_t, Result> done;
  uint64_t next = 1;
  uint32_t next_lane = 0;
  hipEvent_t ready = nullptr;
  uint32_t part = 0;
  uint32_t app_in_flight = 0;
  uint64_t seq = 0;
  uint64_t app_res = 0;
  uint64_t app_max = 0;
  bool broken = false;
};

static bool chain_behind(const OccPipe* p) {
  for (const OccPipe::Flight& f : p->flight)
    if (f.chain) return true;
  return false;
}

static void pipe_complete_front(dcc_ctx* ctx) {
  OccPipe* p = ctx->pipe;
  const OccPipe::Flight f = p->flight.front();
  p->flight.pop_front();
  dcc_ctx* lane = p->lanes[f.lane];
  OccPipe::Result r{};
  (void)hipSetDevice(lane->device);
  r.rc = lane->occ_end(&r.st);
  if (r.rc != DCC_OK) r.err = lane->last_error;
  bool host_done = true;
  if (f.chain) {
    uint64_t st = 0;
    const hipError_t e = hipEventSynchronize(lane->ev_done);
    if (e == hipSuccess) {
      st = ((const uint64_t*)((const char*)lane->hfin + dcc_ctx::HDYN_TOTALS))[4];
    } else if (r.rc == DCC_OK) {
      r.rc = ctx->hip_fail(e, "chained central_finish");
      r.err = ctx->last_error;
    }
    if (st == 2 && lane->run.app) ctx->hs[1].built = false;
    if (p->broken) {
      r.rc = DCC_EIO;
      r.err = "an epoch before this one in the pipeline failed after its central_finish ran on the device";
      host_done = false;
    } else if (r.rc != DCC_OK) {
      if (st == 1) {
        p->broken = true;
        ctx->hs[1].built = false;
        host_done = false;
      }
    } else if (st == 1) {
      r.rc = ctx->chain_accept(lane);
      r.st.fin_where = 1;
      host_done = false;
      if (r.rc != DCC_OK) {
        r.err = ctx->last_error;
        p->broken = true;
        ctx->hs[1].built = false;
      }
    } else {
      r.rc = ctx->pipe_finish(lane, true);
      r.st.fin_where = 2;
      if (r.rc != DCC_OK) r.err = ctx->last_error;
    }
  } else if (r.rc == DCC_OK && lane->run.fin_later) {
    r.rc = ctx->pipe_finish(lane, chain_behind(p));
    r.st.fin_where = 2;
    if (r.rc != DCC_OK) r.err = ctx->last_error;
  } else if (r.rc == DCC_OK) {
    ctx->tnc += lane->run.n_cw;
  }
  if (host_done && !p->broken && chain_behind(p) && ctx->chain_set(lane, f.seq + 1) != DCC_OK) {
    p->broken = true;
    ctx->hs[1].built = false;
  }
  if (lane->run.fin_later && lane->run.app) p->app_in_flight--;
  if (f.chain && f.app) {
    p->app_res -= f.res;
    p->app_max = std::max<uint64_t>(p->app_max, ctx->hs[1].last_app);
  }
  lane->tnc = 0;
  p->done[f.ticket] = std::move(r);
}

void dcc_pipe_drain(dcc_ctx* ctx) {
  if (!ctx || !ctx->pipe) return;
  while (!ctx->pipe->flight.empty()) pipe_complete_front(ctx);
  ctx->pipe->broken = false;
}

void dcc_pipe_destroy(dcc_ctx* ctx) {
  if (!ctx || !ctx->pipe) return;
  dcc_pipe_drain(ctx);
  for (dcc_ctx* l : ctx->pipe->lanes) dcc_destroy(l);
  if (ctx->pipe->ready) (void)hipEventDestroy(ctx->pipe->ready);
  delete ctx->pipe;
  ctx->pipe = nullptr;
}

static int lane_partition(dcc_ctx* ctx, dcc_ctx* l, uint32_t i, uint32_t L) {
  const uint32_t n = (uint32_t)ctx->n_cu;
  if (L < 2 || n % (8 * L)) return DCC_OK;
  std::vector<uint32_t> mask((n + 31) / 32, 0u);
  const uint32_t b0 = i * n / L, b1 = (i + 1) * n / L;
  for (uint32_t b = b0; b < b1; b++) mask[b / 32] |= 1u << (b % 32);
  hipStream_t s = nullptr;
  const hipError_t e = hipExtStreamCreateWithCUMask(&s, (uint32_t)mask.size(), mask.data());
  if (e != hipSuccess) return ctx->hip_fail(e, "pipeline lane: hipExtStreamCreateWithCUMask");
  if (l->own_stream) (void)hipStreamDestroy(l->own_stream);
  l->own_stream = l->stream = s;
  l->n_cu = (int)(b1 - b0);
  return DCC_OK;
}

static int pipe_lanes(dcc_ctx* ctx) {
  OccPipe* p = ctx->pipe;
  const size_t want = ctx->pipe_lanes;
  if (p->lanes.size() == want && p->part == ctx->pipe_part) return DCC_OK;
  dcc_pipe_drain(ctx);
  if (p->part != ctx->pipe_part) {
    for (dcc_ctx* l : p->lanes) dcc_destroy(l);
    p->lanes.clear();
    p->part = ctx->pipe_part;
  }
  while (p->lanes.size() > want) {
    dcc_destroy(p->lanes.back());
    p->lanes.pop_back();
  }
  if (p->part)
    while (!p->lanes.empty() && p->lanes.size() != want) {
      dcc_destroy(p->lanes.back());
      p->lanes.pop_back();
    }
  while (p->lanes.size() < want) {
    dcc_ctx* l = nullptr;
    const int e = dcc_init(&l, ctx->device);
    if (e != DCC_OK) return ctx->fail(e, "pipeline lane on device %d: %s", ctx->device, dcc_strerror(e));
    p->lanes.push_back(l);
    if (p->part) {
      const int x = lane_partition(ctx, l, (uint32_t)p->lanes.size() - 1, (uint32_t)want);
      if (x != DCC_OK) return x;
    }
  }
  p->next_lane = 0;
  return DCC_OK;
}

static void lane_options(const dcc_ctx* ctx, dcc_ctx* l) {
  l->solver = ctx->solver;
  l->ro_split = ctx->ro_split;
  l->wt_bits = std::max(l->wt_bits, ctx->wt_bits);
  l->sw_levels = ctx->sw_levels;
  l->recheck_max = ctx->recheck_max;
  l->batch_max = ctx->batch_max;
}

extern "C" int dcc_occ_submit_epoch(dcc_ctx* ctx, const dcc_batch* b, uint8_t* out_rc,
                                    uint64_t* out_tn, uint64_t* out_ticket) {
  if (!ctx || !b || !out_ticket) return DCC_EINVAL;
  if (hipSetDevice(ctx->device) != hipSuccess) return DCC_ENODEV;
  if (!ctx->pipe) {
    ctx->pipe = new OccPipe();
    if (hipEventCreateWithFlags(&ctx->pipe->ready, hipEventDisableTiming) != hipSuccess) {
      (void)hipGetLastError();
      ctx->pipe->ready = nullptr;
      return ctx->fail(DCC_EIO, "pipeline event");
    }
  }
  OccPipe* p = ctx->pipe;
  const uint64_t ticket = p->next;
  const bool shared = (b->flags & DCC_OCC_DEFER_FINISH) || ctx->fin_pending ||
                      (b->start_tn && (ctx->hist_size() > 0 || p->app_in_flight > 0));
  const bool lanes_ok = !ctx->multi && !ctx->sharded() && !ctx->profiling &&
                        ctx->use_sweep() && !shared && b->n_txn > 0;
  if (!lanes_ok) {
    dcc_pipe_drain(ctx);
    OccPipe::Result r{};
    r.rc = dcc_occ_validate_epoch(ctx, b, out_rc, out_tn, &r.st);
    if (r.rc != DCC_OK) r.err = ctx->last_error;
    p->next++;
    p->done[ticket] = std::move(r);
    *out_ticket = ticket;
    return DCC_OK;
  }
  if (int e = pipe_lanes(ctx)) return e;
  const bool fin = out_tn || (b->flags & DCC_OCC_APPEND_HISTORY);
  const bool chain = fin && ctx->pipe_chain;
  const bool app = chain && (b->flags & DCC_OCC_APPEND_HISTORY);
  const uint64_t res = app ? (p->app_max ? 2 * p->app_max : b->nnz / 16) + 4096 : 0;
  if (p->broken) dcc_pipe_drain(ctx);
  if (app && ctx->hs[1].m + p->app_res + res > ctx->hist_room()) dcc_pipe_drain(ctx);
  const int li = (int)(p->next_lane++ % p->lanes.size());
  dcc_ctx* lane = p->lanes[li];
  while (lane->run.active && !p->flight.empty()) pipe_complete_front(ctx);
  const bool reset = chain && p->flight.empty();
  if (reset && app) {
    if (int e = ctx->hist_prepare()) return e;
    const uint64_t want = ctx->hs[1].m + 4 * (p->lanes.size() + 1) * res;
    if (want > ctx->hist_room())
      if (int e = ctx->hist_grow_flat(ctx->hs[1], want)) return e;
  }
  lane_options(ctx, lane);
  if (hipEventRecord(p->ready, ctx->stream) != hipSuccess ||
      hipStreamWaitEvent(lane->stream, p->ready, 0) != hipSuccess)
    return ctx->hip_fail(hipGetLastError(), "pipeline stream ordering");
  p->next++;
  *out_ticket = ticket;
  const int e = lane->occ_begin(b, out_rc, out_tn, true, true);
  if (e == DCC_OK && lane->run.fin_later && lane->run.app) p->app_in_flight++;
  if (e != DCC_OK) {
    OccPipe::Result r{};
    r.rc = e;
    r.err = lane->last_error;
    p->done[ticket] = std::move(r);
    return DCC_OK;
  }
  OccPipe::Flight f{ticket, li, ++p->seq, false, false, 0};
  if (ctx->pipe_chain) {
    if (!lane->ev_done && hipEventCreateWithFlags(&lane->ev_done, hipEventDisableTiming) != hipSuccess)
      return ctx->hip_fail(hipGetLastError(), "pipeline lane event");
    if (chain && lane->run.fin_later) {
      hipEvent_t after = p->flight.empty() ? nullptr : p->lanes[p->flight.back().lane]->ev_done;
      f.chain = ctx->chain_enqueue(lane, f.seq, after, reset) == DCC_OK;
      if (!f.chain) {
        (void)hipGetLastError();
        ctx->hs[1].built = false;
      }
      f.app = f.chain && app;
      f.res = f.app ? res : 0;
      p->app_res += f.res;
    }
    if (hipEventRecord(lane->ev_done, lane->stream) != hipSuccess)
      return ctx->hip_fail(hipGetLastError(), "pipeline lane event");
  }
  p->flight.push_back(f);
  return DCC_OK;
}

extern "C" int dcc_occ_wait_epoch(dcc_ctx* ctx, uint64_t ticket, dcc_stats* st) {
  if (!ctx) return DCC_EINVAL;
  OccPipe* p = ctx->pipe;
  if (!p || ticket == 0 || ticket >= p->next) return ctx->fail(DCC_EINVAL, "unknown epoch ticket %llu",
                                                               (unsigned long long)ticket);
  while (!p->done.count(ticket) && !p->flight.empty() && p->flight.front().ticket <= ticket)
    pipe_complete_front(ctx);
  auto it = p->done.find(ticket);
  if (it == p->done.end())
    return ctx->fail(DCC_EINVAL, "epoch ticket %llu was already waited", (unsigned long long)ticket);
  const int rc = it->second.rc;
  if (st) *st = it->second.st;
  if (rc != DCC_OK) ctx->last_error = it->second.err;
  p->done.erase(it);
  return rc;
}
```

### deneva_amd/csrc/occ_sweep.hip

```cpp
#include <hip/hip_runtime.h>

#include <algorithm>

#include "dcc_device.h"
#include "occ_kernels.h"
#include "prep_body.h"

namespace dcc {

constexpr uint32_t LB_ACC_BITS = 34;

__device__ inline uint32_t sw_hash(uint64_t key, uint32_t log2s) {
  const uint32_t h = (uint32_t)key * 0x9E3779B1u ^ (uint32_t)(key >> 32) * 0x85EBCA77u;
  return h >> (32 - log2s);
}

__device__ inline uint32_t gtab_step(uint64_t key, uint32_t gbits, uint32_t step) {
  const uint32_t h = sw_hash(key, gbits);
  const uint32_t nbm = (1u << (gbits - 2)) - 1u;
  const uint32_t b = ((h >> 2) + (step >> 2)) & nbm;
  return 4 * b + (((h & 3u) + step) & 3u);
}
__device__ inline unsigned long long gtab_cas(uint64_t* gt, uint32_t slot, uint64_t key) {
  return atomicCAS((unsigned long long*)(gt + slot), (unsigned long long)KEY_EMPTY,
                   (unsigned long long)key);
}
__device__ inline uint32_t gtab_insert(uint64_t* gt, uint32_t gbits, uint64_t key, uint32_t step) {
  for (uint32_t q = step; q < (4u << (gbits - 2)); q++) {
    const uint32_t sl = gtab_step(key, gbits, q);
    const unsigned long long prev = gtab_cas(gt, sl, key);
    if (prev == KEY_EMPTY || prev == key) return sl;
  }
  return 0;
}

__device__ inline void bloom_bits(uint64_t key, uint32_t& b1, uint32_t& b2) {
  const uint32_t h = (uint32_t)key * 0x9E3779B1u ^ (uint32_t)(key >> 32) * 0x85EBCA77u;
  b1 = h >> (32 - SW_BLOOM_LOG);
  b2 = (h * 0xC2B2AE35u + 0x27D4EB2Fu) >> (32 - SW_BLOOM_LOG);
}

__device__ inline void wt_insert(const WrTab& wt, uint64_t key, uint32_t tid) {
  const uint32_t mask = (1u << wt.bits) - 1u;
  uint32_t s = sw_hash(key, wt.bits);
  for (uint32_t q = 0; q < wt.probes; q++, s = (s + 1) & mask) {
    const unsigned long long prev = atomicCAS((unsigned long long*)&wt.slot[s].key,
                                              (unsigned long long)KEY_EMPTY, (unsigned long long)key);
    if (prev == KEY_EMPTY || prev == key) {
      wt.slot[s].tid = tid;
      return;
    }
  }
  atomicOr(wt.full, 1u);
}
__device__ inline uint32_t wt_find(const WrTab& wt, uint64_t key) {
  const uint32_t mask = (1u << wt.bits) - 1u;
  uint32_t s = sw_hash(key, wt.bits);
  for (uint32_t q = 0; q < wt.probes; q++, s = (s + 1) & mask) {
    const uint4 v = *(const uint4*)&wt.slot[s];
    const uint64_t k = ((uint64_t)v.y << 32) | v.x;
    if (k == key) return v.z;
    if (k == KEY_EMPTY) break;
  }
  return ~0u;
}

template <uint32_t S>
__device__ inline bool lset_find(const uint64_t* cs, uint64_t key) {
  constexpr uint32_t NB = S / 4, LB = __builtin_ctz(NB);
  uint32_t b = sw_hash(key, LB);
#pragma unroll 1
  for (uint32_t q = 0; q < NB; q++) {
    const uint4* p = (const uint4*)(cs + 4 * b);
    const uint4 x = p[0], y = p[1];
    const uint64_t v0 = ((uint64_t)x.y << 32) | x.x, v1 = ((uint64_t)x.w << 32) | x.z;
    const uint64_t v2 = ((uint64_t)y.y << 32) | y.x, v3 = ((uint64_t)y.w << 32) | y.z;
    if (v0 == key || v1 == key || v2 == key || v3 == key) return true;
    if (v3 == KEY_EMPTY) return false;
    b = (b + 1) & (NB - 1);
  }
  return false;
}
template <uint32_t S>
__device__ inline bool lset_insert(uint64_t* cs, uint64_t key) {
  constexpr uint32_t NB = S / 4, LB = __builtin_ctz(NB);
  uint32_t b = sw_hash(key, LB);
#pragma unroll 1
  for (uint32_t q = 0; q < NB; q++) {
#pragma unroll
    for (uint32_t i = 0; i < 4; i++) {
      uint64_t* slot = cs + 4 * b + i;
      const uint64_t v = *slot;
      if (v == key) return false;
      if (v == KEY_EMPTY) {
        const unsigned long long prev = atomicCAS((unsigned long long*)slot,
                                                  (unsigned long long)KEY_EMPTY,
                                                  (unsigned long long)key);
        if (prev == KEY_EMPTY) return true;
        if (prev == key) return false;
      }
    }
    b = (b + 1) & (NB - 1);
  }
  return false;
}

__device__ inline bool range_any(const uint64_t* bm, uint32_t lo, uint32_t len) {
  if (len == 0) return false;
  const uint32_t hi = lo + len - 1;
  const uint32_t w0 = lo >> 6, w1 = hi >> 6;
  uint64_t acc = 0;
  for (uint32_t w = w0; w <= w1; w++) {
    uint64_t m = ~0ull;
    if (w == w0) m &= ~0ull << (lo & 63);
    if (w == w1) m &= ~0ull >> (63 - (hi & 63));
    acc |= bm[w] & m;
  }
  return acc != 0;
}
__device__ inline uint32_t range_next(const uint64_t* bm, uint32_t lo, uint32_t hi) {
  for (uint32_t w = lo >> 6; (w << 6) < hi; w++) {
    uint64_t v = bm[w];
    if (w == (lo >> 6)) v &= ~0ull << (lo & 63);
    if (v) {
      const uint32_t x = (w << 6) + (uint32_t)__builtin_ctzll(v);
      return x < hi ? x : hi;
    }
  }
  return hi;
}
__device__ inline void range_set(uint64_t* bm, uint32_t lo, uint32_t len) {
  if (len == 0) return;
  const uint32_t hi = lo + len - 1;
  const uint32_t w0 = lo >> 6, w1 = hi >> 6;
  for (uint32_t w = w0; w <= w1; w++) {
    uint64_t m = ~0ull;
    if (w == w0) m &= ~0ull << (lo & 63);
    if (w == w1) m &= ~0ull >> (63 - (hi & 63));
    atomicOr((unsigned long long*)&bm[w], (unsigned long long)m);
  }
}

__device__ inline uint32_t list_len(const uint32_t* m_dev, uint32_t m_host) {
  return m_dev ? *m_dev : m_host;
}

__device__ inline uint32_t sw_tiles_per_wg(uint32_t n64, uint32_t nblocks) {
  return max((n64 + nblocks - 1) / nblocks, SW_CHUNK / 64);
}

constexpr uint32_t PRE_MAP = 4096;
constexpr uint32_t PRE_B = 1024;

__device__ inline uint32_t pre_map_insert(uint64_t* mkey, uint64_t key, bool& first) {
  uint32_t h = sw_hash(key, 12);
  for (uint32_t q = 0; q < PRE_MAP; q++) {
    const uint64_t v = mkey[h];
    if (v == key) {
      first = false;
      return h;
    }
    if (v == KEY_EMPTY) {
      const unsigned long long prev = atomicCAS((unsigned long long*)&mkey[h],
                                                (unsigned long long)KEY_EMPTY,
                                                (unsigned long long)key);
      if (prev == KEY_EMPTY) {
        first = true;
        return h;
      }
      if (prev == key) {
        first = false;
        return h;
      }
    }
    h = (h + 1) & (PRE_MAP - 1);
  }
  first = false;
  return 0;
}

struct PreLds {
  uint64_t mkey[PRE_MAP];
  uint64_t mmask[PRE_MAP];
  uint64_t mamask[PRE_MAP];
  uint32_t mgid[PRE_MAP];
  uint64_t s_dep[SW_T];
  uint32_t s_off[SW_T + 1];
  uint32_t s_meta[SW_T];
  uint32_t s_bad;
};
template <uint32_t U>
__device__ inline void pre_tile(const SwPreArgs& a, PreLds& L, uint32_t k, uint32_t j, uint32_t nt,
                                uint32_t A0, uint32_t cnt, uint64_t off0) {
  uint64_t* const mkey = L.mkey;
  uint64_t* const mmask = L.mmask;
  uint64_t* const mamask = L.mamask;
  uint32_t* const mgid = L.mgid;
  uint64_t* const s_dep = L.s_dep;
  const uint32_t* const s_off = L.s_off;
  uint32_t* const s_meta = L.s_meta;
  uint64_t key[U];
  uint32_t lt[U], slot[U];
  uint32_t vm = 0, wmk = 0;
  {
    uint8_t atv[U];
    const uint32_t xmax = cnt ? A0 + cnt - 1 : A0;
#pragma unroll
    for (uint32_t u = 0; u < U; u++) {
      const uint32_t x = min(A0 + j + PRE_B * u, xmax);
      key[u] = a.in.keys[x];
      atv[u] = a.in.acctype[x];
    }
    uint32_t bad_key = 0;
#pragma unroll
    for (uint32_t u = 0; u < U; u++) {
      lt[u] = 0;
      slot[u] = 0;
      const uint32_t xr = j + PRE_B * u;
      if (xr >= cnt) continue;
      const uint32_t x = A0 + xr;
      uint32_t lo = 0, hi = nt;
      while (hi - lo > 1) {
        const uint32_t mid = (lo + hi) >> 1;
        if (s_off[mid] <= x) lo = mid;
        else hi = mid;
      }
      lt[u] = lo;
      if (atv[u] == 1) {
        wmk |= 1u << u;
        atomicOr(&s_meta[lo], SWM_HASW);
      }
      if (key[u] == KEY_EMPTY) {
        bad_key = 1;
        a.aent[A0 - (uint32_t)off0 + xr] = SW_A_NONE;
        a.apos[A0 - (uint32_t)off0 + xr] = k * SW_T;
      } else {
        vm |= 1u << u;
      }
    }
    if (bad_key) atomicOr(a.err, ERR_KEY);
  }
  const uint32_t P = cnt <= PRE_MAP / 2 ? 1u : 2u;
  for (uint32_t p = 0; p < P; p++) {
    for (uint32_t q = j; q < PRE_MAP; q += PRE_B) {
      mkey[q] = KEY_EMPTY;
      mmask[q] = 0;
      mamask[q] = 0;
    }
    __syncthreads();
  if (a.dbg && blockIdx.x == 0 && threadIdx.x == 0) a.dbg[3] = __builtin_amdgcn_s_memrealtime();
    uint32_t pm = vm;
    if (P > 1)
#pragma unroll
      for (uint32_t u = 0; u < U; u++)
        if ((sw_hash(key[u], 13) & 1u) != p) pm &= ~(1u << u);
    uint32_t fm = 0;
#pragma unroll
    for (uint32_t u = 0; u < U; u++) {
      if (!((pm >> u) & 1u)) continue;
      bool first;
      slot[u] = pre_map_insert(mkey, key[u], first);
      if (first) fm |= 1u << u;
      if ((wmk >> u) & 1u) atomicOr((unsigned long long*)&mmask[slot[u]], 1ull << lt[u]);
      atomicOr((unsigned long long*)&mamask[slot[u]], 1ull << lt[u]);
    }
    if (a.dbg && blockIdx.x == 0) {
      __syncthreads();
      if (j == 0 && p == 0) a.dbg[12] = __builtin_amdgcn_s_memrealtime();
    }
    {
      unsigned long long prev[U];
      uint32_t gid[U];
#pragma unroll
      for (uint32_t u = 0; u < U; u++) {
        gid[u] = gtab_step(key[u], a.gbits, 0);
        prev[u] = KEY_EMPTY;
        if ((fm >> u) & 1u) prev[u] = gtab_cas(a.gtab, gid[u], key[u]);
      }
      uint32_t lost = 0;
#pragma unroll
      for (uint32_t u = 0; u < U; u++)
        if (((fm >> u) & 1u) && prev[u] != KEY_EMPTY && prev[u] != key[u]) lost |= 1u << u;
      if (a.dbg && blockIdx.x == 0) {
        __syncthreads();
        if (j == 0 && p == 0) a.dbg[13] = __builtin_amdgcn_s_memrealtime();
      }
#pragma unroll
      for (uint32_t u = 0; u < U; u++)
        if ((lost >> u) & 1u) {
          gid[u] = gtab_step(key[u], a.gbits, 1);
          prev[u] = gtab_cas(a.gtab, gid[u], key[u]);
        }
      uint32_t slow = 0;
#pragma unroll
      for (uint32_t u = 0; u < U; u++)
        if (((lost >> u) & 1u) && prev[u] != KEY_EMPTY && prev[u] != key[u]) slow |= 1u << u;
      if (a.dbg && blockIdx.x == 0) {
        __syncthreads();
        if (j == 0 && p == 0) a.dbg[14] = __builtin_amdgcn_s_memrealtime();
        if (lost) atomicAdd((unsigned long long*)&a.dbg[15], (unsigned long long)__popc(lost));
        if (fm) atomicAdd((unsigned long long*)&a.dbg[16], (unsigned long long)__popc(fm));
// ... 440 lines not shown
          cb_insert_m(cbits, e, M);
        }
      }
      s_M[k] = M;
      __hip_atomic_store(&s_done, kn, __ATOMIC_RELAXED, __HIP_MEMORY_SCOPE_WORKGROUP);
      slot = sn;
    }
    if (lane == 0) {
      s_k = k;
      lds_st(&s_stop, 1u);
      if (dbg) {
        dbg[2] = __builtin_amdgcn_s_memrealtime();
        dbg[5] = cw;
        dbg[6] = k;
        dbg[8] = __builtin_amdgcn_s_memtime() - cyc0;
        dbg[9] = st_u;
        dbg[10] = st_it;
      }
    }
  }
  __syncthreads();
  const uint32_t k = s_k;
  constexpr uint32_t WO_U = 8;
  for (uint32_t q0 = 0; q0 < k * SW_T; q0 += SEQ_B * WO_U) {
    uint32_t mt[WO_U], tid[WO_U];
#pragma unroll
    for (uint32_t u = 0; u < WO_U; u++) {
      const uint32_t q = q0 + u * SEQ_B + j;
      mt[u] = 0;
      tid[u] = 0;
      if (q < k * SW_T) {
        mt[u] = a.rec[q / SW_T].meta[q % SW_T];
        tid[u] = a.rec[q / SW_T].rtid[q % SW_T];
      }
    }
    bool cw[WO_U];
#pragma unroll
    for (uint32_t u = 0; u < WO_U; u++) {
      const uint32_t q = q0 + u * SEQ_B + j;
      cw[u] = false;
      if (mt[u] & SWM_VALID) {
        const bool com = (s_M[q / SW_T] >> (q % SW_T)) & 1ull;
        if (!(mt[u] & SWM_PRE)) a.state[tid[u]] = com ? ST_COMMIT : ST_ABORT;
        if (a.write_hasw) a.hasw[tid[u]] = (mt[u] & SWM_HASW) ? 1 : 0;
        cw[u] = com && !(mt[u] & SWM_PRE) && (mt[u] & SWM_HASW);
      }
    }
    if (a.cw_list) {
      uint64_t bm[WO_U];
      uint32_t tot = 0;
#pragma unroll
      for (uint32_t u = 0; u < WO_U; u++) {
        bm[u] = ballot64(cw[u]);
        tot += (uint32_t)__popcll(bm[u]);
      }
      uint32_t base = 0;
      if (lane == 0 && tot) base = atomicAdd(a.cw_count, tot);
      base = __shfl(base, 0);
#pragma unroll
      for (uint32_t u = 0; u < WO_U; u++) {
        if (cw[u]) a.cw_list[base + (uint32_t)__popcll(bm[u] & lanemask_lt())] = tid[u];
        base += (uint32_t)__popcll(bm[u]);
      }
    }
  }
  if (dbg) {
    __syncthreads();
    if (j == 0) dbg[3] = __builtin_amdgcn_s_memrealtime();
  }
  for (uint32_t q = j; q < k; q += SEQ_B) a.mg[q] = s_M[q];
  for (uint32_t q = j; q < nwords; q += SEQ_B) a.cbits_out[q] = 0;
  for (uint32_t q = j; q < (1u << SW_BLOOM_LOG) / 32; q += SEQ_B) a.bloom_out[q] = 0;
  if (j == 0) {
    a.lv->pos = min(k * SW_T, lim);
    a.lv->ccount = 0;
    if (dbg) dbg[4] = __builtin_amdgcn_s_memrealtime();
  }
}

__global__ __launch_bounds__(256) void k_sw_cout(SwCoutArgs a) {
  __shared__ uint32_t s_cnt[4];
  __shared__ uint32_t s_base;
  if (blockIdx.x >= a.cout_grid) {
    const uint32_t b = blockIdx.x - a.cout_grid, nb = gridDim.x - a.cout_grid;
    prep_body_hasw(a.prep_off, a.prep_n, a.prep_at, a.prep_nnz, a.hasw, a.prep_part, b, nb, a.prep_err);
    const uint4 e = make_uint4(~0u, ~0u, ~0u, ~0u);
    for (uint64_t q = (uint64_t)b * 256 + threadIdx.x; q < a.wclear_n16; q += (uint64_t)nb * 256)
      a.wclear[q] = e;
    return;
  }
  const uint32_t ab = *a.abandon;
  const uint32_t pos = a.lv->pos;
  const uint32_t m = list_len(a.m_dev, a.m_host);
  const uint32_t o0_raw = a.in.off[0];
  if (ab) return;
  if (a.skip_done && pos >= m) return;
  const uint32_t lane = lane_id(), wv = threadIdx.x >> 6;
  const uint64_t nnz = a.in.nnz;
  const uint32_t off0 = (uint32_t)min((uint64_t)o0_raw, nnz);
  const uint32_t range = (uint32_t)min((uint64_t)a.in.off[pos], nnz) - off0;
  for (uint32_t x0 = blockIdx.x * 1024; x0 < range; x0 += gridDim.x * 1024) {
    uint32_t ent[4], ap[4];
    uint64_t kx[4];
    bool c[4];
#pragma unroll
    for (uint32_t u = 0; u < 4; u++) {
      const uint32_t x = x0 + wv * 256 + u * 64 + lane;
      const bool in = x < range;
      ent[u] = in ? a.aent[x] : 0u;
      ap[u] = in ? a.apos[x] : 0u;
      kx[u] = in ? a.in.keys[off0 + x] : 0ull;
    }
    uint64_t mw[4];
#pragma unroll
    for (uint32_t u = 0; u < 4; u++) mw[u] = (ent[u] & 32u) ? a.mg[ap[u] >> 6] : 0ull;
#pragma unroll
    for (uint32_t u = 0; u < 4; u++) c[u] = (ent[u] & 32u) && ((mw[u] >> (ap[u] & 63u)) & 1ull);
    uint64_t cm[4];
    uint32_t wc = 0;
#pragma unroll
    for (uint32_t u = 0; u < 4; u++) {
      cm[u] = ballot64(c[u]);
      wc += (uint32_t)__popcll(cm[u]);
    }
    if (lane == 0) s_cnt[wv] = wc;
    __syncthreads();
    if (threadIdx.x == 0) {
      const uint32_t tot = s_cnt[0] + s_cnt[1] + s_cnt[2] + s_cnt[3];
      s_base = tot ? atomicAdd(&a.lv->ccount, tot) : 0u;
    }
    __syncthreads();
    uint32_t base = s_base;
    for (uint32_t w = 0; w < wv; w++) base += s_cnt[w];
#pragma unroll
    for (uint32_t u = 0; u < 4; u++) {
      if (c[u]) {
        const uint64_t key = kx[u];
        a.ckeys_out[base + (uint32_t)__popcll(cm[u] & lanemask_lt())] = key;
        const uint32_t id = sw_aid(ent[u]);
        if (id < SW_ID_NONE) atomicOr(&a.cbits_out[id >> 5], 1u << (id & 31u));
        uint32_t b1, b2;
        bloom_bits(key, b1, b2);
        atomicOr(&a.bloom_out[b1 >> 5], 1u << (b1 & 31));
        atomicOr(&a.bloom_out[b2 >> 5], 1u << (b2 & 31));
      }
      base += (uint32_t)__popcll(cm[u]);
    }
    __syncthreads();
  }
}

constexpr uint32_t FW = SW_CHUNK / 64;
constexpr uint32_t FK = 16;
constexpr uint32_t SW_CMP_MAXR = 4096;

__device__ inline bool c_exact(const SwFilterArgs& a, uint64_t key) {
  const uint32_t nbm = (1u << (a.gbits - 2)) - 1u;
  uint32_t b = sw_hash(key, a.gbits - 2);
  for (uint32_t q = 0; q <= nbm; q++) {
    const uint4* p = (const uint4*)(a.gtab + 4 * (uint64_t)b);
    const uint4 x = p[0], y = p[1];
    const uint32_t nib = (a.cbits[b >> 3] >> ((b & 7u) * 4u)) & 15u;
    const uint64_t v0 = ((uint64_t)x.y << 32) | x.x, v1 = ((uint64_t)x.w << 32) | x.z;
    const uint64_t v2 = ((uint64_t)y.y << 32) | y.x, v3 = ((uint64_t)y.w << 32) | y.z;
    if (v0 == key) return nib & 1u;
    if (v1 == key) return (nib >> 1) & 1u;
    if (v2 == key) return (nib >> 2) & 1u;
    if (v3 == key) return (nib >> 3) & 1u;
    if (v0 == KEY_EMPTY || v1 == KEY_EMPTY || v2 == KEY_EMPTY || v3 == KEY_EMPTY) return false;
    b = (b + 1) & nbm;
  }
  return false;
}
constexpr uint32_t F_STASH = 256;
#ifndef DCC_F_XS
#define DCC_F_XS 2048
#endif
#ifndef DCC_F_WPE
#define DCC_F_WPE 1
#endif
constexpr uint32_t F_XS = DCC_F_XS;
constexpr uint32_t F_XCAP = F_XS / 2;
constexpr uint32_t F_XBITS_LOG = 16;

__global__ __launch_bounds__(SW_CHUNK, DCC_F_WPE) void k_sw_filter(SwFilterArgs a) {
  constexpr uint32_t B = SW_CHUNK, FW = B / 64;
  constexpr uint32_t CS = F_XS;
  struct XSet {
    uint32_t bl[(1u << F_XBITS_LOG) / 32];
    uint64_t cex[F_XS];
  };
  union FSet {
    XSet x;
    uint32_t bl[(1u << SW_BLOOM_LOG) / 32];
  };
  __shared__ __attribute__((aligned(16))) FSet fs;
  uint32_t* const bl = fs.bl;
  uint64_t* const cex = fs.x.cex;
  __shared__ uint64_t s_hit[FW][SW_WA / 64];
  __shared__ uint64_t s_stash[FW][F_STASH];
  __shared__ uint32_t s_wpre[FW][SW_WA / 64];
  const uint32_t j = threadIdx.x, lane = lane_id(), wv = j >> 6;
  const uint32_t ab = *a.abandon;
  const uint32_t m = list_len(a.m_dev, a.m_host);
  const uint32_t pos = a.lv->pos;
  const uint32_t ccount = a.lv->ccount;
  if (ab) return;
  const bool X = ccount <= F_XCAP;
  uint64_t* dbg = (a.dbg && blockIdx.x < 256 && j == 0) ? a.dbg + 8 * blockIdx.x : nullptr;
  if (dbg) dbg[0] = __builtin_amdgcn_s_memrealtime();
  if (pos >= m && !a.kill_out) return;
  for (uint64_t q = (uint64_t)blockIdx.x * B + j; q < a.gclear_n;
       q += (uint64_t)gridDim.x * B) {
    a.gclear[q] = KEY_EMPTY;
    a.fw_clear[q] = ~0u;
    a.la_clear[q] = 0u;
  }
  if (pos >= m) return;
  const uint32_t n64 = (m - pos + 63) / 64;
  const uint64_t nnz = a.in.nnz;
  const uint32_t R = sw_tiles_per_wg(n64, gridDim.x);
  const uint32_t t_lo = min(blockIdx.x * R, n64), t_hi = min(t_lo + R, n64);
  if (t_lo >= t_hi) {
    if (!a.kill_out && j == 0) {
      a.bsum[blockIdx.x] = 0;
      if (a.ro_split) a.rbsum[blockIdx.x] = 0;
    }
    return;
  }
  const bool small = X;
  {
    if (!X) {
      const uint4* src = (const uint4*)a.bloom;
      uint4* dst = (uint4*)bl;
      for (uint32_t q = j; q < (1u << SW_BLOOM_LOG) / 128; q += B) dst[q] = src[q];
    } else {
      for (uint32_t q = j; q < (1u << F_XBITS_LOG) / 32; q += B) bl[q] = 0;
      for (uint32_t q = j; q < CS; q += B) cex[q] = KEY_EMPTY;
    }
  }
  __syncthreads();
  if (small) {
    for (uint32_t q = j; q < ccount; q += B) {
      const uint64_t kq = a.ckeys[q];
      lset_insert<CS>(cex, kq);
      if (X) {
        uint32_t b1, b2;
        bloom_bits(kq, b1, b2);
        b1 >>= SW_BLOOM_LOG - F_XBITS_LOG;
        atomicOr(&bl[b1 >> 5], 1u << (b1 & 31u));
      }
    }
    __syncthreads();
  }
  if (dbg) dbg[1] = __builtin_amdgcn_s_memrealtime();
  uint64_t* hit = s_hit[wv];
  uint64_t* stash = s_stash[wv];
  uint64_t wsum = 0, rsum = 0;
  uint32_t ns = 0, ne = 0, ntid = 0, nst = 0, nhw = 1;
  auto prefetch = [&](uint32_t wt) {
    const uint32_t pc = min(pos + wt * 64 + lane, m - 1);
    ns = a.in.off[pc];
    ne = a.in.off[pc + 1];
    ntid = a.in.tid ? a.in.tid[pc] : pc;
    nst = a.cand_state ? a.state[pc] : 0u;
    if (a.ro_split) nhw = a.hasw[pc];
  };
  if (t_lo + wv < t_hi) prefetch(t_lo + wv);
  for (uint32_t wt = t_lo + wv; wt < t_hi; wt += FW) {
    const uint32_t p = pos + wt * 64 + lane;
    const bool valid = p < m;
    uint32_t s = 0, e = 0, tid = 0;
    bool cand = false, ro = false;
    if (valid) {
      s = (uint32_t)min((uint64_t)ns, nnz);
      e = (uint32_t)min((uint64_t)ne, nnz);
      if (e < s) e = s;
      tid = ntid;
      cand = nst == ST_UNDECIDED;
      ro = nhw == 0;
    }
    bool pref = false;
    const uint64_t vm = ballot64(valid);
    const uint32_t A0 = vm ? __shfl(s, 0) : 0u;
    const uint32_t A1 = wave_reduce<MaxOp<uint32_t>>(valid ? e : 0u);
    uint32_t span = A1 > A0 ? A1 - A0 : 0u;
    if (span > SW_WA) {
      if (lane == 0) atomicOr(a.err, ERR_TILE);
      span = 0;
    }
    const uint32_t nw = (span + 63) / 64;
    uint32_t npos = 0;
    bool bad_key = false;
    for (uint32_t b0 = 0; b0 < span; b0 += 64 * FK) {
      uint64_t key[FK];
#pragma unroll
      for (uint32_t u = 0; u < FK; u++) {
        const uint32_t xr = b0 + 64 * u + lane;
        const uint32_t x = A0 + (xr < span ? xr : 0u);
        key[u] = a.in.keys[x];
      }
      if (!pref) {
        pref = true;
        if (wt + FW < t_hi) prefetch(wt + FW);
      }
#pragma unroll
      for (uint32_t u = 0; u < FK; u++) {
        const uint32_t xr = b0 + 64 * u + lane;
        if (b0 + 64 * u >= span) continue;
        const bool in = xr < span;
        bad_key |= in && key[u] == KEY_EMPTY;
        bool h;
        uint32_t b1, b2;
        bloom_bits(key[u], b1, b2);
        if (X) {
          b1 >>= SW_BLOOM_LOG - F_XBITS_LOG;
          h = in && ((bl[b1 >> 5] >> (b1 & 31u)) & 1u) != 0;
        } else {
          const uint32_t wa = bl[b1 >> 5], wb = bl[b2 >> 5];
          h = in && (((wa >> (b1 & 31u)) & (wb >> (b2 & 31u)) & 1u) != 0);
        }
        const uint64_t hb = ballot64(h);
        if (h) {
          const uint32_t ci = npos + (uint32_t)__popcll(hb & lanemask_lt());
          if (ci < F_STASH) stash[ci] = key[u];
        }
        npos += (uint32_t)__popcll(hb);
        if (lane == 0) hit[(b0 >> 6) + u] = hb;
      }
    }
    if (!pref && wt + FW < t_hi) prefetch(wt + FW);
    if (ballot64(bad_key) && lane == 0) atomicOr(a.err, ERR_KEY);
    if (dbg && wt == t_lo) dbg[2] = __builtin_amdgcn_s_memrealtime();
    const uint32_t rlo = s - A0, rlen = e - s;
    const bool ok = valid && (rlen == 0 || (uint64_t)rlo + rlen <= span);
    bool killed = false;
    {
      {
        const uint32_t pw = lane < nw ? (uint32_t)__popcll(hit[lane]) : 0u;
        uint32_t ptot;
        const uint32_t pre = wave_excl<AddOp<uint32_t>>(pw, ptot);
        if (lane < nw) s_wpre[wv][lane] = pre;
      }
      if (cand && ok && rlen) {
        for (uint32_t x = rlo; x < rlo + rlen; x++) {
          const uint32_t nx = range_next(hit, x, rlo + rlen);
          if (nx >= rlo + rlen) break;
          const uint32_t ci = s_wpre[wv][nx >> 6] +
                              (uint32_t)__popcll(hit[nx >> 6] & ((1ull << (nx & 63)) - 1ull));
          const uint64_t kx = ci < F_STASH ? stash[ci] : a.in.keys[A0 + nx];
          if (small ? lset_find<CS>(cex, kx) : c_exact(a, kx)) {
            killed = true;
            break;
          }
          x = nx;
        }
      }
    }
    if (dbg && wt == t_lo) dbg[3] = __builtin_amdgcn_s_memrealtime();
    if (dbg) dbg[6]++;
    if (a.kill_out) {
      const uint64_t km = ballot64(valid && killed);
      if (lane == 0) a.kill_out[wt] = km;
      continue;
    }
    if (killed) a.state[tid] = ST_ABORT;
    if (cand && ok && rlen == 0) a.state[tid] = ST_COMMIT;
    const bool surv = cand && ok && rlen && !killed;
    const uint64_t sm = ballot64(surv);
    const uint64_t acc = wave_reduce<AddOp<uint64_t>>(surv ? rlen : 0u);
    const uint64_t cnt = ((uint64_t)__popcll(sm) << LB_ACC_BITS) | acc;
    wsum += cnt;
    if (lane == 0) {
      a.sflag[wt] = sm;
      a.tcount[wt] = cnt;
    }
    if (a.ro_split) {
      const uint64_t rm = ballot64(surv && ro);
      const uint64_t racc = wave_reduce<AddOp<uint64_t>>(surv && ro ? rlen : 0u);
      const uint64_t rc = ((uint64_t)__popcll(rm) << LB_ACC_BITS) | racc;
      rsum += rc;
      if (lane == 0) {
        a.rflag[wt] = rm;
        a.rtcount[wt] = rc;
      }
    }
    if (dbg && wt == t_lo) {
      __builtin_amdgcn_s_waitcnt(0);
      dbg[4] = __builtin_amdgcn_s_memrealtime();
    }
  }
  if (a.kill_out) return;
  __shared__ unsigned long long s_bs[FW][2];
  if (lane == 0) {
    s_bs[wv][0] = wsum;
    s_bs[wv][1] = rsum;
  }
  __syncthreads();
  if (j == 0) {
    uint64_t t = 0, r = 0;
    for (uint32_t w = 0; w < FW; w++) {
      t += s_bs[w][0];
      r += s_bs[w][1];
    }
    a.bsum[blockIdx.x] = t;
    if (a.ro_split) a.rbsum[blockIdx.x] = r;
  }
  if (dbg) {
    __builtin_amdgcn_s_waitcnt(0);
    dbg[5] = __builtin_amdgcn_s_memrealtime();
  }
}

__global__ __launch_bounds__(SW_CHUNK) void k_sw_apply(SwFilterArgs a) {
  const uint32_t lane = lane_id(), wv = threadIdx.x >> 6;
  if (*a.abandon) return;
  const uint32_t m = list_len(a.m_dev, a.m_host);
  const uint32_t pos = a.lv->pos;
  if (pos >= m) return;
  const uint32_t n64 = (m - pos + 63) / 64;
  const uint64_t nnz = a.in.nnz;
  const uint32_t R = sw_tiles_per_wg(n64, gridDim.x);
  const uint32_t t_lo = min(blockIdx.x * R, n64), t_hi = min(t_lo + R, n64);
  uint64_t wsum = 0, rsum = 0;
  for (uint32_t wt = t_lo + wv; wt < t_hi; wt += SW_CHUNK / 64) {
    const uint32_t p = pos + wt * 64 + lane;
    uint64_t kw = 0;
    for (uint32_t r = 0; r < a.kill_ranks; r++) kw |= a.kill_in[r * a.kill_stride + wt];
    const bool kill = (kw >> lane) & 1ull;
    bool surv = false, ro = false;
    uint32_t len = 0;
    if (p < m) {
      const uint32_t tid = a.in.tid ? a.in.tid[p] : p;
      const bool cand = a.cand_state ? a.state[p] == ST_UNDECIDED : true;
      const uint32_t s = (uint32_t)min((uint64_t)a.in.off[p], nnz);
      const uint32_t e = (uint32_t)min((uint64_t)a.in.off[p + 1], nnz);
      len = e > s ? e - s : 0u;
      if (cand && kill) a.state[tid] = ST_ABORT;
      surv = cand && !kill;
      ro = a.ro_split && a.hasw[tid] == 0;
    }
    const uint64_t sm = ballot64(surv);
    const uint64_t acc = wave_reduce<AddOp<uint64_t>>(surv ? len : 0u);
    const uint64_t cnt = ((uint64_t)__popcll(sm) << LB_ACC_BITS) | acc;
    wsum += cnt;
    if (lane == 0) {
      a.sflag[wt] = sm;
      a.tcount[wt] = cnt;
    }
    if (a.ro_split) {
      const uint64_t rm = ballot64(surv && ro);
      const uint64_t racc = wave_reduce<AddOp<uint64_t>>(surv && ro ? len : 0u);
      const uint64_t rc = ((uint64_t)__popcll(rm) << LB_ACC_BITS) | racc;
      rsum += rc;
      if (lane == 0) {
        a.rflag[wt] = rm;
        a.rtcount[wt] = rc;
      }
    }
  }
  __shared__ unsigned long long s_bs[SW_CHUNK / 64][2];
  if (lane == 0) {
    s_bs[wv][0] = wsum;
    s_bs[wv][1] = rsum;
  }
  __syncthreads();
  if (threadIdx.x == 0) {
    uint64_t t = 0, r = 0;
    for (uint32_t w = 0; w < SW_CHUNK / 64; w++) {
      t += s_bs[w][0];
      r += s_bs[w][1];
    }
    a.bsum[blockIdx.x] = t;
    if (a.ro_split) a.rbsum[blockIdx.x] = r;
  }
}

constexpr uint32_t SG_T = 1024;
__global__ __launch_bounds__(SG_T) void k_sw_sg_scan(const uint32_t* tid, const uint32_t* m_dev, uint32_t p_max,
                                                     const uint32_t* full_off, uint64_t full_nnz, uint32_t* soff,
                                                     uint32_t* err) {
  __shared__ uint32_t s_w[SG_T / 64];
  __shared__ uint32_t s_carry;
  const uint32_t P = min(p_max, *m_dev);
  if (threadIdx.x == 0) s_carry = 0;
  __syncthreads();
  for (uint32_t q0 = 0; q0 < P; q0 += SG_T) {
    const uint32_t q = q0 + threadIdx.x;
    uint32_t len = 0;
    if (q < P) {
      const uint32_t t = tid[q];
      const uint64_t s = min((uint64_t)full_off[t], full_nnz), e = min((uint64_t)full_off[t + 1], full_nnz);
      len = e > s ? (uint32_t)(e - s) : 0u;
      if (len > MAX_TXN_LEN) {
        atomicOr(err, ERR_OFFSETS);
        len = 0;
      }
    }
    uint32_t tot;
    const uint32_t ex = s_carry + block_excl<SG_T / 64, AddOp<uint32_t>>(len, s_w, tot);
    if (q < P) soff[q] = ex;
    __syncthreads();
    if (threadIdx.x == SG_T - 1) s_carry = ex + len;
    __syncthreads();
  }
  if (threadIdx.x == 0) soff[P] = s_carry;
}
__global__ __launch_bounds__(256) void k_sw_sg_copy(const uint32_t* tid, const uint32_t* m_dev, uint32_t p_max,
                                                    const uint32_t* full_off, const uint64_t* full_keys,
                                                    const uint8_t* full_at, uint64_t full_nnz, const uint32_t* soff,
                                                    uint64_t* skeys, uint8_t* sat) {
  const uint32_t P = min(p_max, *m_dev), sl = threadIdx.x & 15u;
  for (uint32_t q = (blockIdx.x * 256 + threadIdx.x) >> 4; q < P; q += gridDim.x * 16) {
    const uint32_t t = tid[q], o = soff[q], len = soff[q + 1] - o;
    const uint64_t s = min((uint64_t)full_off[t], full_nnz);
    for (uint32_t x = sl; x < len; x += 16) {
      skeys[o + x] = full_keys[s + x];
      sat[o + x] = full_at[s + x];
    }
  }
}

__global__ void k_sw_share(const uint32_t* m_dev, uint32_t m_host, const uint32_t* abandon,
                           const uint32_t* off, uint32_t p_max, uint32_t rank, uint32_t* cnt) {
  const uint32_t m = m_dev ? *m_dev : m_host;
  const uint32_t P = min(p_max, m);
  cnt[0] = m;
  cnt[1] = *abandon;
  cnt[2 + rank] = m ? off[P] - off[0] : 0u;
}

__global__ __launch_bounds__(256) void k_sw_export(SwList in, uint32_t P, uint32_t* rec) {
  const uint64_t nnz = in.nnz;
  const uint32_t off0 = (uint32_t)min((uint64_t)in.off[0], nnz);
  for (uint32_t t = blockIdx.x * 4 + (threadIdx.x >> 6); t < P; t += gridDim.x * 4) {
    const uint32_t s = (uint32_t)min((uint64_t)in.off[t], nnz);
    const uint32_t e = (uint32_t)min((uint64_t)in.off[t + 1], nnz);
    for (uint32_t x = s + lane_id(); x < e; x += 64) {
      const uint64_t k = in.keys[x];
      uint32_t* r = rec + 3ull * (x - off0);
      r[0] = (uint32_t)k;
      r[1] = (uint32_t)(k >> 32);
      r[2] = t | ((uint32_t)(in.acctype[x] & 3u) << 30);
    }
  }
}

__global__ __launch_bounds__(256) void k_sw_mcount(const uint32_t* rec, uint32_t n, uint32_t P,
                                                   uint32_t* cnt) {
  for (uint32_t i = blockIdx.x * 256 + threadIdx.x; i < n; i += gridDim.x * 256) {
    const uint32_t t = rec[3ull * i + 2] & 0x3FFFFFFFu;
    if (t < P) atomicAdd(&cnt[t], 1u);
  }
}
__global__ __launch_bounds__(1024) void k_sw_mscan(uint32_t* cnt, uint32_t P, uint32_t* off,
                                                   uint32_t* cur) {
  __shared__ uint32_t s_w[16];
  __shared__ uint32_t s_carry;
  const uint32_t j = threadIdx.x, lane = lane_id(), wv = j >> 6;
  if (j == 0) s_carry = 0;
  __syncthreads();
  for (uint32_t c0 = 0; c0 < P; c0 += 1024) {
    const uint32_t t = c0 + j;
    const uint32_t v = t < P ? cnt[t] : 0u;
    uint32_t tot;
    const uint32_t ex = wave_excl<AddOp<uint32_t>>(v, tot);
    if (lane == 0) s_w[wv] = tot;
    __syncthreads();
    uint32_t base = s_carry;
    for (uint32_t w = 0; w < wv; w++) base += s_w[w];
    if (t < P) {
      off[t] = base + ex;
      cur[t] = base + ex;
    }
    __syncthreads();
    if (j == 0) {
      uint32_t all = 0;
      for (uint32_t w = 0; w < 16; w++) all += s_w[w];
      s_carry += all;
    }
    __syncthreads();
  }
  if (j == 0) off[P] = s_carry;
}
__global__ __launch_bounds__(256) void k_sw_mscatter(const uint32_t* rec, uint32_t n, uint32_t P,
                                                     uint32_t* cur, uint64_t* keys,
                                                     uint8_t* at) {
  for (uint32_t i = blockIdx.x * 256 + threadIdx.x; i < n; i += gridDim.x * 256) {
    const uint32_t w2 = rec[3ull * i + 2];
    if ((w2 & 0x3FFFFFFFu) >= P) continue;
    const uint32_t q = atomicAdd(&cur[w2 & 0x3FFFFFFFu], 1u);
    keys[q] = ((uint64_t)rec[3ull * i + 1] << 32) | rec[3ull * i];
    at[q] = (uint8_t)(w2 >> 30);
  }
}

__global__ __launch_bounds__(SW_CHUNK) void k_sw_compact(SwFilterArgs a) {
  const uint32_t lane = lane_id(), wv = threadIdx.x >> 6;
  const uint32_t ab = *a.abandon;
  const uint32_t m = list_len(a.m_dev, a.m_host);
  const uint32_t pos = a.lv->pos;
  if (ab && ab != a.level + 1) return;
  if (pos >= m) return;
  const uint32_t n64 = (m - pos + 63) / 64;
  const uint64_t nnz = a.in.nnz;
  const uint32_t R = sw_tiles_per_wg(n64, a.nblocks);
  const uint32_t t_lo = min(blockIdx.x * R, n64), t_hi = min(t_lo + R, n64);
  if (t_lo >= t_hi && blockIdx.x) return;
  uint64_t* dbg = (a.cdbg && blockIdx.x == 0 && threadIdx.x == 0) ? a.cdbg : nullptr;
  if (dbg) dbg[0] = __builtin_amdgcn_s_memrealtime();
  __shared__ unsigned long long s_tb[SW_CMP_MAXR];
  __shared__ unsigned long long s_part[SW_CHUNK / 64][4];
  __shared__ uint32_t s_split, s_rnext;
  if (R > SW_CMP_MAXR) {
    if (threadIdx.x == 0) atomicOr(a.err, ERR_TILE);
    return;
  }
  {
    uint64_t pre = 0, all = 0, rpre = 0, rall = 0;
    constexpr uint32_t TU = 4;
    for (uint32_t q0 = threadIdx.x; q0 < a.nblocks; q0 += SW_CHUNK * TU) {
      uint64_t v[TU], r[TU];
#pragma unroll
      for (uint32_t u = 0; u < TU; u++) {
        const uint32_t q = q0 + u * SW_CHUNK;
        v[u] = q < a.nblocks ? a.bsum[q] : 0ull;
        r[u] = (a.ro_split && q < a.nblocks) ? a.rbsum[q] : 0ull;
      }
#pragma unroll
      for (uint32_t u = 0; u < TU; u++) {
        const uint32_t q = q0 + u * SW_CHUNK;
        all += v[u];
        rall += r[u];
        if (q < blockIdx.x) {
          pre += v[u];
          rpre += r[u];
        }
      }
    }
    pre = wave_reduce<AddOp<uint64_t>>(pre);
    all = wave_reduce<AddOp<uint64_t>>(all);
    rpre = wave_reduce<AddOp<uint64_t>>(rpre);
    rall = wave_reduce<AddOp<uint64_t>>(rall);
    if (lane == 0) {
      s_part[wv][0] = pre;
      s_part[wv][1] = all;
      s_part[wv][2] = rpre;
      s_part[wv][3] = rall;
    }
    __syncthreads();
    if (threadIdx.x == 0) {
      uint64_t p0 = 0, a0 = 0, rp = 0, ra = 0;
      for (uint32_t w = 0; w < SW_CHUNK / 64; w++) {
        p0 += s_part[w][0];
        a0 += s_part[w][1];
        rp += s_part[w][2];
        ra += s_part[w][3];
      }
      const uint32_t tot = (uint32_t)(a0 >> LB_ACC_BITS);
      const uint32_t in_n = m - pos;
      const bool handoff =
          tot > a.abandon_min && (uint64_t)tot * a.abandon_den > (uint64_t)in_n * a.abandon_num;
      const bool split = a.ro_split && !handoff;
      s_split = split ? 1u : 0u;
      s_part[0][0] = split ? p0 - rp : p0;
      s_rnext = (uint32_t)(rp >> LB_ACC_BITS);
      if (blockIdx.x == 0) {
        const uint64_t keep = split ? a0 - ra : a0;
        const uint32_t kt = (uint32_t)(keep >> LB_ACC_BITS);
        const uint64_t acc = keep & ((1ull << LB_ACC_BITS) - 1);
        a.lv_next->m = kt;
        a.lv_next->acc = (uint32_t)acc;
        a.off_out[kt] = (uint32_t)acc;
        if (a.ro_split) *a.ro_count = split ? (uint32_t)(ra >> LB_ACC_BITS) : 0u;
        if (handoff) atomicMax(a.abandon_out, a.level + 1);
      }
    }
    __syncthreads();
  }
  const bool split = s_split != 0;
  if (dbg) dbg[1] = __builtin_amdgcn_s_memrealtime();
  if (wv == 0) {
    uint64_t run = s_part[0][0];
    for (uint32_t c0 = t_lo; c0 < t_hi; c0 += 64) {
      const uint32_t q = c0 + lane;
      const uint64_t v = (q < t_hi ? a.tcount[q] : 0ull) - ((split && q < t_hi) ? a.rtcount[q] : 0ull);
      uint64_t tot;
      const uint64_t ex = wave_excl<AddOp<uint64_t>>(v, tot);
      if (q < t_hi) s_tb[q - t_lo] = run + ex;
      run += tot;
    }
  }
  __syncthreads();
  if (dbg) dbg[2] = __builtin_amdgcn_s_memrealtime();
  constexpr uint32_t CB = 4;
  for (uint32_t w0 = t_lo + wv; w0 < t_hi; w0 += FW * CB) {
    uint64_t wordv[CB], rwordv[CB];
    uint32_t sv[CB], ev[CB], tv[CB];
#pragma unroll
    for (uint32_t i = 0; i < CB; i++) {
      const uint32_t wt = w0 + FW * i;
      const uint32_t pc = min(pos + min(wt, n64 - 1) * 64 + lane, m - 1);
      wordv[i] = wt < t_hi ? a.sflag[wt] : 0ull;
      rwordv[i] = (split && wt < t_hi) ? a.rflag[wt] : 0ull;
      sv[i] = a.in.off[pc];
      ev[i] = a.in.off[pc + 1];
      tv[i] = a.in.tid ? a.in.tid[pc] : pc;
    }
#pragma unroll
    for (uint32_t i = 0; i < CB; i++) {
      const uint32_t wt = w0 + FW * i;
      const uint64_t rword = rwordv[i];
      const uint64_t word = wordv[i] & ~rword;
      if (rword) {
        uint32_t rb = 0;
        if (lane == 0) rb = atomicAdd(&s_rnext, (uint32_t)__popcll(rword));
        rb = __shfl(rb, 0);
        if ((rword >> lane) & 1ull) {
          const uint32_t rs = (uint32_t)min((uint64_t)sv[i], nnz);
          a.ro_out[rb + (uint32_t)__popcll(rword & lanemask_lt())] =
              RoEnt{tv[i], rs, max(rs, (uint32_t)min((uint64_t)ev[i], nnz)), 0u};
        }
      }
      if (!word) continue;
      const uint64_t base = s_tb[wt - t_lo];
      const uint32_t tb = (uint32_t)(base >> LB_ACC_BITS);
      const uint32_t abase = (uint32_t)(base & ((1ull << LB_ACC_BITS) - 1));
      const bool surv = (word >> lane) & 1ull;
      uint32_t s = 0, len = 0;
      if (surv) {
        s = (uint32_t)min((uint64_t)sv[i], nnz);
        len = (uint32_t)min((uint64_t)ev[i], nnz) - s;
      }
      uint32_t atot;
      const uint32_t aex = wave_excl<AddOp<uint32_t>>(len, atot);
      if (surv) {
        const uint32_t r = tb + (uint32_t)__popcll(word & lanemask_lt());
        a.tid_out[r] = tv[i];
        a.off_out[r] = abase + aex;
      }
      const uint32_t incl = aex + len;
      for (uint32_t q0 = 0; q0 < atot; q0 += 64 * 4) {
        uint32_t src[4];
        bool in[4];
#pragma unroll
        for (uint32_t r = 0; r < 4; r++) {
          const uint32_t q = q0 + 64 * r + lane;
          uint32_t lo = 0;
#pragma unroll
          for (uint32_t st = 32; st > 0; st >>= 1) {
            const uint32_t v = __shfl(incl, lo + st - 1);
            if (v <= q) lo += st;
          }
          in[r] = q < atot;
          src[r] = __shfl(s, lo) + (q - __shfl(aex, lo));
        }
        uint64_t kk[4];
        uint8_t aa[4];
#pragma unroll
        for (uint32_t r = 0; r < 4; r++) {
          kk[r] = in[r] ? a.in.keys[src[r]] : 0ull;
          aa[r] = in[r] ? a.in.acctype[src[r]] : (uint8_t)0;
        }
#pragma unroll
        for (uint32_t r = 0; r < 4; r++) {
          if (!in[r]) continue;
          const uint32_t q = q0 + 64 * r + lane;
          a.keys_out[abase + q] = kk[r];
          a.acc_out[abase + q] = aa[r];
        }
      }
    }
  }
  if (dbg) {
    __builtin_amdgcn_s_waitcnt(0);
    dbg[4] = __builtin_amdgcn_s_memrealtime();
  }
}

__global__ __launch_bounds__(256) void k_sw_ro(SwRoArgs a) {
  const uint32_t cnt = *a.ro_count;
  const uint32_t lane = lane_id(), g = lane >> 2, sl = lane & 3u;
  const uint32_t ng = gridDim.x * 64;
  const uint32_t mask = (1u << a.wt.bits) - 1u;
  for (uint32_t i = (blockIdx.x * 256 + threadIdx.x) >> 2; i < cnt; i += ng) {
    uint4 r = *(const uint4*)&a.ro[i];
    if (a.full_off) {
      r.y = a.full_off[r.x];
      r.z = a.full_off[r.x + 1];
    }
    bool kill = false;
    for (uint32_t x0 = r.y + sl; x0 < r.z && !kill; x0 += 16) {
      uint64_t k[4];
      bool in[4];
#pragma unroll
      for (uint32_t u = 0; u < 4; u++) {
        in[u] = x0 + 4 * u < r.z;
        k[u] = in[u] ? a.keys[x0 + 4 * u] : KEY_EMPTY;
      }
      uint32_t sv[4];
      uint4 v[4];
#pragma unroll
      for (uint32_t u = 0; u < 4; u++) {
        sv[u] = sw_hash(k[u], a.wt.bits);
        v[u] = in[u] ? *(const uint4*)&a.wt.slot[sv[u]] : make_uint4(~0u, ~0u, ~0u, ~0u);
      }
#pragma unroll
      for (uint32_t u = 0; u < 4; u++) {
        if (!in[u]) continue;
        uint32_t q = 0, s0 = sv[u];
        for (;;) {
          const uint64_t kk = ((uint64_t)v[u].y << 32) | v[u].x;
          if (kk == k[u]) {
            kill |= v[u].z < r.x;
            break;
          }
          if (kk == KEY_EMPTY || ++q >= a.wt.probes) break;
          s0 = (s0 + 1) & mask;
          v[u] = *(const uint4*)&a.wt.slot[s0];
        }
      }
    }
    const uint64_t b = ballot64(kill);
    if (sl == 0) a.state[r.x] = ((b >> (4 * g)) & 0xFull) ? ST_ABORT : ST_COMMIT;
  }
}

__device__ inline void wall_txn(const SwWallArgs& a, uint64_t tt, uint32_t sl) {
  const uint64_t s = min((uint64_t)a.off[tt], a.nnz), e = min((uint64_t)a.off[tt + 1], a.nnz);
  for (uint64_t x = s + sl; x < e; x += 16)
    if (a.acctype[x] == 1) wt_insert(a.wt, a.keys[x], (uint32_t)tt);
}
__global__ __launch_bounds__(256) void k_sw_wall(SwWallArgs a) {
  const uint32_t lane = lane_id(), g = lane >> 4, sl = lane & 15u;
  if (a.cw_list) {
    const uint32_t cnt = *a.cw_count;
    for (uint32_t i = (blockIdx.x * 256 + threadIdx.x) >> 4; i < cnt; i += gridDim.x * 16)
      wall_txn(a, a.cw_list[i], sl);
    return;
  }
  for (uint64_t t0 = ((uint64_t)blockIdx.x * 256 + threadIdx.x) & ~63ull; t0 < a.n;
       t0 += (uint64_t)gridDim.x * 256) {
    const uint64_t t = t0 + lane;
    const bool cw = t < a.n && a.state[t] == ST_COMMIT && a.hasw[t];
    uint64_t w = ballot64(cw);
    while (w) {
      uint32_t pick[4];
#pragma unroll
      for (int q = 0; q < 4; q++) {
        pick[q] = w ? (uint32_t)__builtin_ctzll(w) : 64u;
        if (w) w &= w - 1;
      }
      if (pick[g] < 64) wall_txn(a, t0 + pick[g], sl);
    }
  }
}

void launch_sw_ro(const SwRoArgs& a, unsigned grid, hipStream_t st) {
  k_sw_ro<<<grid ? grid : 1u, 256, 0, st>>>(a);
}
void launch_sw_wall(const SwWallArgs& a, unsigned grid, hipStream_t st) {
  k_sw_wall<<<grid ? grid : 1u, 256, 0, st>>>(a);
}
void launch_sw_pre(const SwPreArgs& a, unsigned grid, hipStream_t st) {
  k_sw_pre<<<grid ? grid : 1u, PRE_B, 0, st>>>(a);
}
void launch_sw_seq(const SwSeqArgs& a, hipStream_t st) {
  k_sw_seq<<<1, SEQ_B, 0, st>>>(a);
}
void launch_sw_rows(const SwPreArgs& a, unsigned grid, hipStream_t st) {
  k_sw_rows<<<grid ? grid : 1u, 256, 0, st>>>(a);
}
void launch_sw_cout(const SwCoutArgs& a0, unsigned grid, hipStream_t st) {
  SwCoutArgs a = a0;
  a.cout_grid = grid ? grid : 1u;
  k_sw_cout<<<a.cout_grid + (a.prep_part ? SW_PREP_BLOCKS : 0u), 256, 0, st>>>(a);
}
void launch_sw_filter(const SwFilterArgs& a, unsigned grid, hipStream_t st) {
  k_sw_filter<<<grid ? grid : 1u, SW_CHUNK, 0, st>>>(a);
}
void launch_sw_share(const uint32_t* m_dev, uint32_t m_host, const uint32_t* abandon,
                     const uint32_t* off, uint32_t p_max, uint32_t rank, uint32_t* cnt,
                     hipStream_t st) {
  k_sw_share<<<1, 1, 0, st>>>(m_dev, m_host, abandon, off, p_max, rank, cnt);
}
void launch_sw_sgather(const uint32_t* tid, const uint32_t* m_dev, uint32_t p_max,
                       const uint32_t* full_off, const uint64_t* full_keys, const uint8_t* full_at,
                       uint64_t full_nnz, uint32_t* soff, uint64_t* skeys, uint8_t* sat,
                       uint32_t* err, hipStream_t st) {
  k_sw_sg_scan<<<1, SG_T, 0, st>>>(tid, m_dev, p_max, full_off, full_nnz, soff, err);
  k_sw_sg_copy<<<std::max<uint32_t>(1, std::min<uint32_t>((p_max + 15) / 16, 1024)), 256, 0, st>>>(
      tid, m_dev, p_max, full_off, full_keys, full_at, full_nnz, soff, skeys, sat);
}
void launch_sw_apply(const SwFilterArgs& a, unsigned grid, hipStream_t st) {
  k_sw_apply<<<grid ? grid : 1u, SW_CHUNK, 0, st>>>(a);
}
void launch_sw_merge(const SwList& in, uint32_t P, uint32_t* xbuf, uint32_t xoff_words,
                     uint32_t n_all, uint32_t* cnt, uint32_t* cur, uint32_t* moff,
                     uint64_t* mkeys, uint8_t* mat, bool export_only, hipStream_t st) {
  if (export_only) {
    k_sw_export<<<256, 256, 0, st>>>(in, P, xbuf + xoff_words);
    return;
  }
  const unsigned g = (unsigned)std::min<uint32_t>((n_all + 255) / 256 + 1, 2048);
  k_sw_mcount<<<g, 256, 0, st>>>(xbuf, n_all, P, cnt);
  k_sw_mscan<<<1, 1024, 0, st>>>(cnt, P, moff, cur);
  k_sw_mscatter<<<g, 256, 0, st>>>(xbuf, n_all, P, cur, mkeys, mat);
}
void launch_sw_compact(const SwFilterArgs& a, unsigned grid, hipStream_t st) {
  k_sw_compact<<<grid ? grid : 1u, SW_CHUNK, 0, st>>>(a);
}

}
```

### include/dcc.h

```cpp
#ifndef DCC_H_
#define DCC_H_

#include <stddef.h>
#include <stdint.h>

#ifdef __cplusplus
extern "C" {
#endif

#define DCC_OK 0
#define DCC_EIO (-5)
#define DCC_ENOMEM (-12)
#define DCC_ENODEV (-19)
#define DCC_EINVAL (-22)
#define DCC_ERANGE (-34)
#define DCC_ECOMM (-70)
#define DCC_ENOTSUP (-95)

#define DCC_RD 0
#define DCC_WR 1
#define DCC_XP 2
#define DCC_SCAN 3

#define DCC_RC_RCOK 0
#define DCC_RC_ABORT 2
#define DCC_RC_WAIT 3

#define DCC_KEY_RESERVED 0xFFFFFFFFFFFFFFFFull

#define DCC_GROUP_NONE 0xFFFFFFFFu

#define DCC_DEVICE_PTRS 0x1u
#define DCC_MAAT_READ_AND_PREWRITE 0x4u
#define DCC_OCC_APPEND_HISTORY 0x2u
#define DCC_OCC_DEFER_FINISH 0x8u

#define DCC_KEYS_U32 0x10u
#define DCC_ACCTYPE_2BIT 0x20u
#define DCC_TN_U32 0x40u
#define DCC_COMPACT_FLAGS (DCC_KEYS_U32 | DCC_ACCTYPE_2BIT | DCC_TN_U32)
#define DCC_SHARD_SELF 0x80u

typedef struct dcc_batch {
  uint64_t n_txn;
  uint64_t nnz;
  const uint32_t* offsets;
  const uint64_t* keys;
  const uint8_t* acctype;
  const uint64_t* start_tn;
  const uint64_t* finish_tn;
  const uint64_t* order;
  uint32_t flags;
  uint32_t reserved;
} dcc_batch;

typedef struct dcc_stats {
  uint32_t rounds;
  uint32_t n_shards;
  uint64_t n_commit;
  uint64_t n_abort;
  uint64_t n_readonly;
  uint64_t nnz_w;
  uint64_t alg_bytes;
  double device_ms;
  double total_ms;
  double phase_ms[4];
  uint64_t phase_bytes[4];
  uint64_t peel_prefix;
  uint64_t n_survivors;
  uint32_t fallback;
  uint32_t fin_where;
} dcc_stats;

typedef struct dcc_ctx dcc_ctx;

int dcc_init(dcc_ctx** out, int device_id);
int dcc_init_multi(dcc_ctx** out, int n_gpus, const int* device_ids);
void dcc_destroy(dcc_ctx* ctx);
const char* dcc_strerror(int code);
const char* dcc_last_error(const dcc_ctx* ctx);
int dcc_version(void);
int dcc_device_count(void);

int dcc_set_stream(dcc_ctx* ctx, void* hip_stream);
int dcc_set_profiling(dcc_ctx* ctx, int enable);
#define DCC_OPT_RECHECK 1
#define DCC_OPT_BATCH_MAX 2
#define DCC_OPT_SOLVER 5
#define DCC_OPT_SWEEP_LEVELS 6
#define DCC_OPT_HIST_MERGE 7
#define DCC_OPT_RO_SPLIT 10
#define DCC_OPT_FAIL_RANK 8
#define DCC_OPT_PIPELINE 11
#define DCC_OPT_CALVIN_PATH 12
#define DCC_OPT_COMM_SOLO 13
#define DCC_OPT_PIPE_PARTITION 14
#define DCC_OPT_PIPE_CHAIN 15
int dcc_set_option(dcc_ctx* ctx, int option, int64_t value);
int dcc_reserve(dcc_ctx* ctx, uint64_t max_txn, uint64_t max_nnz);
int dcc_copy_bandwidth(dcc_ctx* ctx, uint64_t bytes, int reps, double* gbps);
int dcc_host_alloc(dcc_ctx* ctx, uint64_t bytes, void** out);
int dcc_host_free(dcc_ctx* ctx, void* p);

#define DCC_UNIQUE_ID_BYTES 128
int dcc_comm_unique_id(void* out_id );
int dcc_comm_init(dcc_ctx* ctx, int rank, int nranks, const void* unique_id);
typedef int (*dcc_exchange_fn)(void* user, uint8_t* host_buf, uint64_t n);
int dcc_comm_init_host(dcc_ctx* ctx, int rank, int nranks, dcc_exchange_fn fn, void* user);
int dcc_comm_destroy(dcc_ctx* ctx);
int dcc_comm_rank(const dcc_ctx* ctx);
int dcc_comm_size(const dcc_ctx* ctx);
uint64_t dcc_comm_calls(const dcc_ctx* ctx);
uint32_t dcc_key_shard(uint64_t key, uint32_t nranks);
int dcc_key_shard_n(const uint64_t* keys, uint64_t n, uint32_t nranks, uint32_t* out);
int dcc_shard_filter(const dcc_batch* in, uint32_t rank, uint32_t nranks,
                     uint32_t* out_offsets, uint64_t* out_keys,
                     uint8_t* out_acctype, uint64_t* out_nnz);

int dcc_occ_validate_epoch(dcc_ctx* ctx, const dcc_batch* batch, uint8_t* out_rc,
                           uint64_t* out_commit_tn, dcc_stats* out_stats);
int dcc_occ_submit_epoch(dcc_ctx* ctx, const dcc_batch* batch, uint8_t* out_rc,
                         uint64_t* out_commit_tn, uint64_t* out_ticket);
int dcc_occ_wait_epoch(dcc_ctx* ctx, uint64_t ticket, dcc_stats* out_stats);
int dcc_occ_finish_epoch(dcc_ctx* ctx, const uint8_t* final_rc, uint64_t* out_commit_tn,
                         uint32_t flags);
int dcc_occ_history_append(dcc_ctx* ctx, const uint64_t* keys, const uint64_t* tn, uint64_t n);
int dcc_occ_history_clear(dcc_ctx* ctx);
uint64_t dcc_occ_history_size(const dcc_ctx* ctx);
int dcc_occ_history_trim(dcc_ctx* ctx, uint64_t tn_floor);
int dcc_occ_history_export(dcc_ctx* ctx, uint64_t* keys, uint64_t* tn, uint64_t cap,
                           uint64_t* out_n);
int dcc_occ_set_tnc(dcc_ctx* ctx, uint64_t tnc);
uint64_t dcc_occ_get_tnc(const dcc_ctx* ctx);

typedef struct dcc_occ_snapshot {
  const uint64_t* hist_top;
  const uint32_t* active_off;
  const uint32_t* active_idx;
} dcc_occ_snapshot;
int dcc_occ_validate_snapshot(dcc_ctx* ctx, const dcc_batch* batch, const dcc_occ_snapshot* snap,
                              uint8_t* out_rc, dcc_stats* out_stats);

int dcc_maat_validate_epoch(dcc_ctx* ctx, const dcc_batch* batch, uint8_t* out_rc,
                            uint64_t* out_commit_ts, dcc_stats* out_stats);
int dcc_maat_rows_set(dcc_ctx* ctx, const uint64_t* keys, const uint64_t* last_read,
                      const uint64_t* last_write, uint64_t n);
int dcc_maat_rows_get(dcc_ctx* ctx, const uint64_t* keys, uint64_t* last_read,
                      uint64_t* last_write, uint64_t n);
int dcc_maat_rows_clear(dcc_ctx* ctx);
uint64_t dcc_maat_rows_size(const dcc_ctx* ctx);
uint64_t dcc_maat_alg_bytes(uint64_t n_txn, uint64_t nnz);

int dcc_calvin_order_epoch(dcc_ctx* ctx, const dcc_batch* batch, uint32_t* out_group,
                           uint8_t* out_rc, uint32_t* out_wave, dcc_stats* out_stats);

typedef struct dcc_calvin_held {
  uint64_t n;
  const uint64_t* keys;
  const uint8_t* acctype;
} dcc_calvin_held;
int dcc_calvin_order_epoch_held(dcc_ctx* ctx, const dcc_batch* batch, const dcc_calvin_held* held,
                                uint32_t* out_group, uint8_t* out_rc, uint32_t* out_wave,
                                dcc_stats* out_stats);

#define DCC_ACCESS_NONE 0xFFFFFFFFu
int dcc_nowait_lock_epoch(dcc_ctx* ctx, const dcc_batch* batch, const dcc_calvin_held* held,
                          uint8_t* out_rc, uint32_t* out_conflict, dcc_stats* out_stats);
uint64_t dcc_nowait_alg_bytes(uint64_t n_txn, uint64_t nnz, int with_conflict);

int dcc_tso_validate_epoch(dcc_ctx* ctx, const dcc_batch* batch, const uint64_t* ts, uint8_t* out_rc,
                           uint32_t* out_conflict, dcc_stats* out_stats);
int dcc_tso_rows_set(dcc_ctx* ctx, const uint64_t* keys, const uint64_t* wts, const uint64_t* rts,
                     uint64_t n);
int dcc_tso_rows_get(dcc_ctx* ctx, const uint64_t* keys, uint64_t* wts, uint64_t* rts, uint64_t n);
int dcc_tso_rows_clear(dcc_ctx* ctx);
uint64_t dcc_tso_rows_size(const dcc_ctx* ctx);
uint64_t dcc_tso_alg_bytes(uint64_t n_txn, uint64_t nnz, int with_conflict);

#define DCC_VTS_BASE 0ull
#define DCC_VTS_NONE 0xFFFFFFFFFFFFFFFFull
int dcc_mvcc_validate_epoch(dcc_ctx* ctx, const dcc_batch* batch, const uint64_t* ts, uint8_t* out_rc,
                            uint32_t* out_conflict, uint64_t* out_vts, dcc_stats* out_stats);
int dcc_mvcc_rows_get(dcc_ctx* ctx, const uint64_t* keys, uint64_t* wts, uint64_t* rts, uint64_t n);
uint64_t dcc_mvcc_rows_size(const dcc_ctx* ctx);
uint64_t dcc_mvcc_versions_size(const dcc_ctx* ctx);
int dcc_mvcc_versions_export(dcc_ctx* ctx, uint64_t* keys, uint64_t* ts, uint64_t cap, uint64_t* n_out);
int dcc_mvcc_trim(dcc_ctx* ctx, uint64_t ts_floor, uint64_t* n_dropped);
int dcc_mvcc_clear(dcc_ctx* ctx);
uint64_t dcc_mvcc_alg_bytes(uint64_t n_txn, uint64_t nnz, int with_conflict, int with_vts);

#define DCC_WD_RUN 0x10
#define DCC_WD_GONE 0x11
int dcc_waitdie_lock_epoch(dcc_ctx* ctx, const dcc_batch* batch, const uint64_t* ts, uint8_t* rc, uint32_t* pos,
                           uint32_t* out_conflict , dcc_stats* out_stats);
int dcc_waitdie_release(dcc_ctx* ctx, const dcc_batch* batch, const uint64_t* ts, uint8_t* rc, uint32_t* pos,
                        const uint8_t* leave, uint64_t* out_left, uint64_t* out_promoted ,
                        dcc_stats* out_stats);
uint64_t dcc_waitdie_alg_bytes(uint64_t n_txn, uint64_t nnz, int with_conflict);

struct dcc_select_out;
typedef struct dcc_waitdie_carry_args {
  const dcc_batch* batch;
  const uint64_t* ts;
  const uint8_t*  rc;
  const uint32_t* pos;
  const uint8_t*  revive;
  const uint32_t* src_in;
  const dcc_batch* fresh;
  const uint64_t* fresh_ts;
  uint32_t fresh_src_base;
  const struct dcc_select_out* out;
  uint64_t* out_ts; uint8_t* out_rc; uint32_t* out_pos;
} dcc_waitdie_carry_args;
int dcc_waitdie_carry(dcc_ctx* ctx, const dcc_waitdie_carry_args* a, uint64_t* out_n,
                      uint64_t* out_nnz, uint64_t* out_kept, dcc_stats* out_stats);
uint64_t dcc_waitdie_carry_alg_bytes(uint64_t n_txn, uint64_t n_kept, uint64_t nnz_kept,
                                     uint64_t n_fresh, uint64_t nnz_fresh, int with_revive, int with_src);

#define DCC_LOCK_EX 0
#define DCC_LOCK_SH 1
typedef struct dcc_locktab dcc_locktab;
typedef struct dcc_locktab_params {
  uint64_t cap_rows;
  uint32_t flags;
  uint32_t reserved;
} dcc_locktab_params;
int dcc_locktab_create(dcc_ctx* ctx, const dcc_locktab_params* params, dcc_locktab** out);
void dcc_locktab_destroy(dcc_locktab* lt);
int dcc_locktab_lock_epoch(dcc_locktab* lt, const dcc_batch* batch, uint8_t* out_rc,
                           uint32_t* out_conflict, dcc_stats* out_stats);
int dcc_locktab_release(dcc_locktab* lt, const dcc_batch* batch, const uint8_t* rc, uint8_t want,
                        uint64_t* out_n, uint64_t* out_nnz, dcc_stats* out_stats);
int dcc_locktab_acquire_rows(dcc_locktab* lt, const dcc_calvin_held* rows, uint32_t flags);
int dcc_locktab_release_rows(dcc_locktab* lt, const uint64_t* keys, uint64_t n, uint32_t flags);
int dcc_locktab_export(dcc_locktab* lt, uint64_t* keys, uint8_t* lock_type, uint32_t* owner_cnt,
                       uint64_t cap, uint32_t flags, uint64_t* out_n);
int dcc_locktab_size(const dcc_locktab* lt, uint64_t* rows_held, uint64_t* slots_used,
                     uint64_t* rebuilds);
int dcc_locktab_clear(dcc_locktab* lt);
int dcc_locktab_pass_ms(const dcc_locktab* lt, double out_ms[3]);
uint64_t dcc_locktab_epoch_alg_bytes(uint64_t n_txn, uint64_t nnz, uint64_t nnz_granted,
                                     int with_conflict);
uint64_t dcc_locktab_release_alg_bytes(uint64_t n_txn, uint64_t n_sel, uint64_t nnz_sel);

typedef struct dcc_select_out {
  uint64_t cap_txn, cap_nnz;
  uint64_t txn_base, nnz_base;
  uint32_t* offsets;
  uint64_t* keys;
  uint8_t*  acctype;
// ... 126 lines not shown
```

Before: 6.240 billion txns/s.

## Decouple sweep filter chunking from grid size with persistent chunk loop

The sweep filter and compaction kernels now split work into a fixed number of chunks (4 per CU by default, capped at 64 tiles per chunk). Each block loops over chunks with a grid stride, where before each block took one contiguous range sized by the grid. The compaction prefix scan now runs in sub-batches of 64 tiles, and a new DCC_OPT_SWEEP_GRID option sets the launch grid independently, with the value included in the graph cache key. The aim is to bound per-chunk scan size and shared memory use and to allow smaller grids, at the cost of extra block syncs and loop overhead.

```diff
diff --git a/deneva_amd/_abi.py b/deneva_amd/_abi.py
--- a/deneva_amd/_abi.py
+++ b/deneva_amd/_abi.py
@@ -48,6 +48,7 @@
 OPT_COMM_SOLO = 13
 OPT_PIPE_PARTITION = 14
 OPT_PIPE_CHAIN = 15
+OPT_SWEEP_GRID = 16
 
 
 class Batch(C.Structure):
diff --git a/deneva_amd/csrc/dcc_ctx.h b/deneva_amd/csrc/dcc_ctx.h
--- a/deneva_amd/csrc/dcc_ctx.h
+++ b/deneva_amd/csrc/dcc_ctx.h
@@ -191,6 +191,7 @@
   uint32_t wt_bits = 18;
   uint32_t wf_bits = 0;
   uint32_t sw_levels = 0;
+  uint32_t sw_grid = 0;
   uint32_t sw_mode = 1;
   uint32_t sw_l1_last = ~0u;
   bool sw_debug = false;
@@ -207,10 +208,12 @@
     uint64_t gen;
     const void *start_tn, *finish_tn, *out_tn;
     uint32_t fin;
+    uint32_t grid = 0;
     bool operator==(const GraphKey& o) const {
       return off == o.off && keys == o.keys && acc == o.acc && n == o.n && nnz == o.nnz &&
              out_rc == o.out_rc && dev_out == o.dev_out && levels == o.levels && gen == o.gen &&
-             start_tn == o.start_tn && finish_tn == o.finish_tn && out_tn == o.out_tn && fin == o.fin;
+             start_tn == o.start_tn && finish_tn == o.finish_tn && out_tn == o.out_tn && fin == o.fin &&
+             grid == o.grid;
     }
   };
   hipGraphExec_t graph_exec = nullptr;
diff --git a/deneva_amd/csrc/dcc_ctx.hip b/deneva_amd/csrc/dcc_ctx.hip
--- a/deneva_amd/csrc/dcc_ctx.hip
+++ b/deneva_amd/csrc/dcc_ctx.hip
@@ -232,6 +232,10 @@
     case DCC_OPT_SWEEP_LEVELS:
       if (value < 0 || value > SW_MAX_LEVEL) return DCC_EINVAL;
       ctx->sw_levels = (uint32_t)value;
+      return DCC_OK;
+    case DCC_OPT_SWEEP_GRID:
+      if (value < 0 || value > 65536) return DCC_EINVAL;
+      ctx->sw_grid = (uint32_t)value;
       return DCC_OK;
     case DCC_OPT_RO_SPLIT:
       if (value != 0 && value != 1 && (value < 4 || value > 24)) return DCC_EINVAL;
diff --git a/deneva_amd/csrc/occ_driver.hip b/deneva_amd/csrc/occ_driver.hip
--- a/deneva_amd/csrc/occ_driver.hip
+++ b/deneva_amd/csrc/occ_driver.hip
@@ -264,6 +264,16 @@
   return std::min<uint32_t>(b, SW_GBITS_MAX);
 }
 
+static uint32_t sw_chunks(uint64_t n, int n_cu) {
+  static const unsigned per_cu = [] {
+    const char* e = DCC_ENV("DCC_SW_NCH");
+    return e && atoi(e) > 0 ? (unsigned)atoi(e) : 4u;
+  }();
+  const uint64_t n64 = (n + 63) / 64;
+  return (uint32_t)std::max<uint64_t>({1, (uint64_t)per_cu * (uint64_t)n_cu,
+                                       (n64 + SW_CHUNK_TILES_MAX - 1) / SW_CHUNK_TILES_MAX});
+}
+
 int dcc_ctx::sweep_reserve(const DevBatch& d) {
   const uint64_t tiles = SW_PMAX_TOP / SW_T;
   sw_debug = DCC_ENV("DCC_SW_DEBUG") != nullptr;
@@ -273,7 +283,7 @@
     CK(hipMemsetAsync(sw_dbg.p, 0, (4096 + 4 * 256 * 8 + 4 * 64 * 8) * 8, stream));
   }
   CR(sw_ctl.ensure(this, sw_ctl_bytes(), "sweep control"));
-  CR(sw_status.ensure(this, ((d.n + 63) / 64 + 64) * 16 + (4ull * n_cu + 64) * 8,
+  CR(sw_status.ensure(this, ((d.n + 63) / 64 + 64) * 16 + ((uint64_t)sw_chunks(d.n, n_cu) + 64) * 8,
                         "sweep survivor bits + tile counts"));
   CR(sw_ckeys.ensure(this, ((1ull << SW_GBITS_MAX) / 32 + (1ull << SW_BLOOM_LOG) / 32) * 4 +
                                 (1ull << SW_GBITS_MAX) * 8,
@@ -286,7 +296,7 @@
   CR(sw_mg.ensure(this, SW_PMAX_TILES * 8, "sweep tile commit masks"));
   if (ro_on) {
     const uint64_t n64 = (d.n + 63) / 64 + 32;
-    CR(sw_rflag.ensure(this, (2 * n64 + 4ull * n_cu + 64) * 8, "sweep read-only survivor bits"));
+    CR(sw_rflag.ensure(this, (2 * n64 + (uint64_t)sw_chunks(d.n, n_cu) + 64) * 8, "sweep read-only survivor bits"));
     CR(sw_ro.ensure(this, d.n * sizeof(RoEnt) + 64, "sweep read-only list"));
     CR(sw_wtab.ensure(this, sizeof(WrSlot) << wt_bits, "committed-writer table"));
     CR(sw_cw.ensure(this, d.n * 4 + 64, "committed writers"));
@@ -312,11 +322,13 @@
     const char* e = DCC_ENV("DCC_SW_FGRID");
     return e ? (unsigned)atoi(e) : 0u;
   }();
-  const unsigned fgrid = fgrid_ov ? fgrid_ov : (unsigned)std::max<uint64_t>(1, 4ull * n_cu);
   static const unsigned fgrid1_ov = [] {
     const char* e = DCC_ENV("DCC_SW_FGRID1");
     return e ? (unsigned)atoi(e) : 0u;
   }();
+  const unsigned grid_opt = sw_grid ? sw_grid : fgrid_ov;
+  const unsigned fgrid = grid_opt ? grid_opt : (unsigned)std::max<uint64_t>(1, 4ull * n_cu);
+  const uint32_t nch = sw_chunks(d.n, n_cu);
   uint64_t* gtab0 = (uint64_t*)sw_gtab.p;
   uint32_t* cbits_d = (uint32_t*)sw_ckeys.p;
   uint32_t* bloom_d = cbits_d + (1u << SW_GBITS_MAX) / 32;
@@ -404,7 +416,7 @@
     fa.tcount = tcount_d;
     fa.bsum = bsum_d;
     const unsigned lgrid = (!top && fgrid1_ov) ? std::min(fgrid1_ov, fgrid) : fgrid;
-    fa.nblocks = lgrid;
+    fa.nblocks = nch;
     fa.lv = lv;
     fa.lv_next = lv + 1;
     fa.state = (uint8_t*)state.p;
@@ -929,7 +941,8 @@
                     r.glv | (ro_on ? 0x80u | (wt_bits << 8) : 0u), buf_gen,
                     d.start_tn, d.finish_tn, r.dev_out ? out_tn : (const void*)(uintptr_t)(out_tn != nullptr),
                     (r.want_tn ? 1u : 0u) | (r.app ? 2u : 0u) | (r.hist_on ? 4u : 0u) |
-                        (r.fin_later ? 8u : 0u)};
+                        (r.fin_later ? 8u : 0u),
+                    sw_grid};
   r.replay = graph_ok && graph_exec && r.gkey == graph_key;
   struct CaptureGuard {
     hipStream_t s;
diff --git a/deneva_amd/csrc/occ_kernels.h b/deneva_amd/csrc/occ_kernels.h
--- a/deneva_amd/csrc/occ_kernels.h
+++ b/deneva_amd/csrc/occ_kernels.h
@@ -307,6 +307,7 @@
   uint64_t wclear_n16;
   uint32_t* prep_err;
 };
+constexpr uint32_t SW_CHUNK_TILES_MAX = 64;
 struct SwFilterArgs {
   SwList in;
   const uint32_t* m_dev;
diff --git a/deneva_amd/csrc/occ_pipe.cpp b/deneva_amd/csrc/occ_pipe.cpp
--- a/deneva_amd/csrc/occ_pipe.cpp
+++ b/deneva_amd/csrc/occ_pipe.cpp
@@ -176,6 +176,7 @@
   l->ro_split = ctx->ro_split;
   l->wt_bits = std::max(l->wt_bits, ctx->wt_bits);
   l->sw_levels = ctx->sw_levels;
+  l->sw_grid = ctx->sw_grid;
   l->recheck_max = ctx->recheck_max;
   l->batch_max = ctx->batch_max;
 }
diff --git a/deneva_amd/csrc/occ_sweep.hip b/deneva_amd/csrc/occ_sweep.hip
--- a/deneva_amd/csrc/occ_sweep.hip
+++ b/deneva_amd/csrc/occ_sweep.hip
@@ -145,8 +145,13 @@
   return m_dev ? *m_dev : m_host;
 }
 
-__device__ inline uint32_t sw_tiles_per_wg(uint32_t n64, uint32_t nblocks) {
-  return max((n64 + nblocks - 1) / nblocks, SW_CHUNK / 64);
+__device__ inline uint32_t sw_chunk_tiles(uint32_t n64, uint32_t nch) {
+  return max((n64 + nch - 1) / nch, SW_CHUNK / 64);
+}
+__device__ inline uint64_t sw_uniform(uint64_t v) {
+  const uint32_t lo = (uint32_t)__builtin_amdgcn_readfirstlane((int)(uint32_t)v);
+  const uint32_t hi = (uint32_t)__builtin_amdgcn_readfirstlane((int)(uint32_t)(v >> 32));
+  return ((uint64_t)hi << 32) | lo;
 }
 
 constexpr uint32_t PRE_MAP = 4096;
@@ -893,7 +898,6 @@
 
 constexpr uint32_t FW = SW_CHUNK / 64;
 constexpr uint32_t FK = 16;
-constexpr uint32_t SW_CMP_MAXR = 4096;
 
 __device__ inline bool c_exact(const SwFilterArgs& a, uint64_t key) {
   const uint32_t nbm = (1u << (a.gbits - 2)) - 1u;
@@ -960,15 +964,11 @@
   if (pos >= m) return;
   const uint32_t n64 = (m - pos + 63) / 64;
   const uint64_t nnz = a.in.nnz;
-  const uint32_t R = sw_tiles_per_wg(n64, gridDim.x);
-  const uint32_t t_lo = min(blockIdx.x * R, n64), t_hi = min(t_lo + R, n64);
-  if (t_lo >= t_hi) {
-    if (!a.kill_out && j == 0) {
-      a.bsum[blockIdx.x] = 0;
-      if (a.ro_split) a.rbsum[blockIdx.x] = 0;
-    }
-    return;
-  }
+  const uint32_t R = sw_chunk_tiles(n64, a.nblocks);
+  const uint32_t nch = (n64 + R - 1) / R;
+  __shared__ unsigned long long s_bs[FW][2];
+  uint32_t c = blockIdx.x;
+  if (c >= nch) return;
   const bool small = X;
   {
     if (!X) {
@@ -997,7 +997,6 @@
   if (dbg) dbg[1] = __builtin_amdgcn_s_memrealtime();
   uint64_t* hit = s_hit[wv];
   uint64_t* stash = s_stash[wv];
-  uint64_t wsum = 0, rsum = 0;
   uint32_t ns = 0, ne = 0, ntid = 0, nst = 0, nhw = 1;
   auto prefetch = [&](uint32_t wt) {
     const uint32_t pc = min(pos + wt * 64 + lane, m - 1);
@@ -1007,145 +1006,152 @@
     nst = a.cand_state ? a.state[pc] : 0u;
     if (a.ro_split) nhw = a.hasw[pc];
   };
-  if (t_lo + wv < t_hi) prefetch(t_lo + wv);
-  for (uint32_t wt = t_lo + wv; wt < t_hi; wt += FW) {
-    const uint32_t p = pos + wt * 64 + lane;
-    const bool valid = p < m;
-    uint32_t s = 0, e = 0, tid = 0;
-    bool cand = false, ro = false;
-    if (valid) {
-      s = (uint32_t)min((uint64_t)ns, nnz);
-      e = (uint32_t)min((uint64_t)ne, nnz);
-      if (e < s) e = s;
-      tid = ntid;
-      cand = nst == ST_UNDECIDED;
-      ro = nhw == 0;
-    }
-    bool pref = false;
-    const uint64_t vm = ballot64(valid);
-    const uint32_t A0 = vm ? __shfl(s, 0) : 0u;
-    const uint32_t A1 = wave_reduce<MaxOp<uint32_t>>(valid ? e : 0u);
-    uint32_t span = A1 > A0 ? A1 - A0 : 0u;
-    if (span > SW_WA) {
-      if (lane == 0) atomicOr(a.err, ERR_TILE);
-      span = 0;
-    }
-    const uint32_t nw = (span + 63) / 64;
-    uint32_t npos = 0;
-    bool bad_key = false;
-    for (uint32_t b0 = 0; b0 < span; b0 += 64 * FK) {
-      uint64_t key[FK];
-#pragma unroll
-      for (uint32_t u = 0; u < FK; u++) {
-        const uint32_t xr = b0 + 64 * u + lane;
-        const uint32_t x = A0 + (xr < span ? xr : 0u);
-        key[u] = a.in.keys[x];
-      }
-      if (!pref) {
-        pref = true;
-        if (wt + FW < t_hi) prefetch(wt + FW);
-      }
-#pragma unroll
-      for (uint32_t u = 0; u < FK; u++) {
-        const uint32_t xr = b0 + 64 * u + lane;
-        if (b0 + 64 * u >= span) continue;
-        const bool in = xr < span;
-        bad_key |= in && key[u] == KEY_EMPTY;
-        bool h;
-        uint32_t b1, b2;
-        bloom_bits(key[u], b1, b2);
-        if (X) {
-          b1 >>= SW_BLOOM_LOG - F_XBITS_LOG;
-          h = in && ((bl[b1 >> 5] >> (b1 & 31u)) & 1u) != 0;
-        } else {
-          const uint32_t wa = bl[b1 >> 5], wb = bl[b2 >> 5];
-          h = in && (((wa >> (b1 & 31u)) & (wb >> (b2 & 31u)) & 1u) != 0);
-        }
-        const uint64_t hb = ballot64(h);
-        if (h) {
-          const uint32_t ci = npos + (uint32_t)__popcll(hb & lanemask_lt());
-          if (ci < F_STASH) stash[ci] = key[u];
-        }
-        npos += (uint32_t)__popcll(hb);
-        if (lane == 0) hit[(b0 >> 6) + u] = hb;
-      }
-    }
-    if (!pref && wt + FW < t_hi) prefetch(wt + FW);
-    if (ballot64(bad_key) && lane == 0) atomicOr(a.err, ERR_KEY);
-    if (dbg && wt == t_lo) dbg[2] = __builtin_amdgcn_s_memrealtime();
-    const uint32_t rlo = s - A0, rlen = e - s;
-    const bool ok = valid && (rlen == 0 || (uint64_t)rlo + rlen <= span);
-    bool killed = false;
-    {
+  for (;;) {
+    const uint32_t t_lo = c * R, t_hi = min(t_lo + R, n64);
+    uint64_t wsum = 0, rsum = 0;
+    if (t_lo + wv < t_hi) prefetch(t_lo + wv);
+    for (uint32_t wt = t_lo + wv; wt < t_hi; wt += FW) {
+      const uint32_t p = pos + wt * 64 + lane;
+      const bool valid = p < m;
+      uint32_t s = 0, e = 0, tid = 0;
+      bool cand = false, ro = false;
+      if (valid) {
+        s = (uint32_t)min((uint64_t)ns, nnz);
+        e = (uint32_t)min((uint64_t)ne, nnz);
+        if (e < s) e = s;
+        tid = ntid;
+        cand = nst == ST_UNDECIDED;
+        ro = nhw == 0;
+      }
+      bool pref = false;
+      const uint64_t vm = ballot64(valid);
+      const uint32_t A0 = vm ? __shfl(s, 0) : 0u;
+      const uint32_t A1 = wave_reduce<MaxOp<uint32_t>>(valid ? e : 0u);
+      uint32_t span = A1 > A0 ? A1 - A0 : 0u;
+      if (span > SW_WA) {
+        if (lane == 0) atomicOr(a.err, ERR_TILE);
+        span = 0;
+      }
+      const uint32_t nw = (span + 63) / 64;
+      uint32_t npos = 0;
+      bool bad_key = false;
+      for (uint32_t b0 = 0; b0 < span; b0 += 64 * FK) {
+        uint64_t key[FK];
+  #pragma unroll
+        for (uint32_t u = 0; u < FK; u++) {
+          const uint32_t xr = b0 + 64 * u + lane;
+          const uint32_t x = A0 + (xr < span ? xr : 0u);
+          key[u] = a.in.keys[x];
+        }
+        if (!pref) {
+          pref = true;
+          if (wt + FW < t_hi) prefetch(wt + FW);
+        }
+  #pragma unroll
+        for (uint32_t u = 0; u < FK; u++) {
+          const uint32_t xr = b0 + 64 * u + lane;
+          if (b0 + 64 * u >= span) continue;
+          const bool in = xr < span;
+          bad_key |= in && key[u] == KEY_EMPTY;
+          bool h;
+          uint32_t b1, b2;
+          bloom_bits(key[u], b1, b2);
+          if (X) {
+            b1 >>= SW_BLOOM_LOG - F_XBITS_LOG;
+            h = in && ((bl[b1 >> 5] >> (b1 & 31u)) & 1u) != 0;
+          } else {
+            const uint32_t wa = bl[b1 >> 5], wb = bl[b2 >> 5];
+            h = in && (((wa >> (b1 & 31u)) & (wb >> (b2 & 31u)) & 1u) != 0);
+          }
+          const uint64_t hb = ballot64(h);
+          if (h) {
+            const uint32_t ci = npos + (uint32_t)__popcll(hb & lanemask_lt());
+            if (ci < F_STASH) stash[ci] = key[u];
+          }
+          npos += (uint32_t)__popcll(hb);
+          if (lane == 0) hit[(b0 >> 6) + u] = hb;
+        }
+      }
+      if (!pref && wt + FW < t_hi) prefetch(wt + FW);
+      if (ballot64(bad_key) && lane == 0) atomicOr(a.err, ERR_KEY);
+      if (dbg && wt == t_lo) dbg[2] = __builtin_amdgcn_s_memrealtime();
+      const uint32_t rlo = s - A0, rlen = e - s;
+      const bool ok = valid && (rlen == 0 || (uint64_t)rlo + rlen <= span);
+      bool killed = false;
       {
-        const uint32_t pw = lane < nw ? (uint32_t)__popcll(hit[lane]) : 0u;
-        uint32_t ptot;
-        const uint32_t pre = wave_excl<AddOp<uint32_t>>(pw, ptot);
-        if (lane < nw) s_wpre[wv][lane] = pre;
-      }
-      if (cand && ok && rlen) {
-        for (uint32_t x = rlo; x < rlo + rlen; x++) {
-          const uint32_t nx = range_next(hit, x, rlo + rlen);
-          if (nx >= rlo + rlen) break;
-          const uint32_t ci = s_wpre[wv][nx >> 6] +
-                              (uint32_t)__popcll(hit[nx >> 6] & ((1ull << (nx & 63)) - 1ull));
-          const uint64_t kx = ci < F_STASH ? stash[ci] : a.in.keys[A0 + nx];
-          if (small ? lset_find<CS>(cex, kx) : c_exact(a, kx)) {
-            killed = true;
-            break;
+        {
+          const uint32_t pw = lane < nw ? (uint32_t)__popcll(hit[lane]) : 0u;
+          uint32_t ptot;
+          const uint32_t pre = wave_excl<AddOp<uint32_t>>(pw, ptot);
+          if (lane < nw) s_wpre[wv][lane] = pre;
+        }
+        if (cand && ok && rlen) {
+          for (uint32_t x = rlo; x < rlo + rlen; x++) {
+            const uint32_t nx = range_next(hit, x, rlo + rlen);
+            if (nx >= rlo + rlen) break;
+            const uint32_t ci = s_wpre[wv][nx >> 6] +
+                                (uint32_t)__popcll(hit[nx >> 6] & ((1ull << (nx & 63)) - 1ull));
+            const uint64_t kx = ci < F_STASH ? stash[ci] : a.in.keys[A0 + nx];
+            if (small ? lset_find<CS>(cex, kx) : c_exact(a, kx)) {
+              killed = true;
+              break;
+            }
+            x = nx;
           }
-          x = nx;
-        }
-      }
-    }
-    if (dbg && wt == t_lo) dbg[3] = __builtin_amdgcn_s_memrealtime();
-    if (dbg) dbg[6]++;
-    if (a.kill_out) {
-      const uint64_t km = ballot64(valid && killed);
-      if (lane == 0) a.kill_out[wt] = km;
-      continue;
-    }
-    if (killed) a.state[tid] = ST_ABORT;
-    if (cand && ok && rlen == 0) a.state[tid] = ST_COMMIT;
-    const bool surv = cand && ok && rlen && !killed;
-    const uint64_t sm = ballot64(surv);
-    const uint64_t acc = wave_reduce<AddOp<uint64_t>>(surv ? rlen : 0u);
-    const uint64_t cnt = ((uint64_t)__popcll(sm) << LB_ACC_BITS) | acc;
-    wsum += cnt;
-    if (lane == 0) {
-      a.sflag[wt] = sm;
-      a.tcount[wt] = cnt;
-    }
-    if (a.ro_split) {
-      const uint64_t rm = ballot64(surv && ro);
-      const uint64_t racc = wave_reduce<AddOp<uint64_t>>(surv && ro ? rlen : 0u);
-      const uint64_t rc = ((uint64_t)__popcll(rm) << LB_ACC_BITS) | racc;
-      rsum += rc;
+        }
+      }
+      if (dbg && wt == t_lo) dbg[3] = __builtin_amdgcn_s_memrealtime();
+      if (dbg) dbg[6]++;
+      if (a.kill_out) {
+        const uint64_t km = ballot64(valid && killed);
+        if (lane == 0) a.kill_out[wt] = km;
+        continue;
+      }
+      if (killed) a.state[tid] = ST_ABORT;
+      if (cand && ok && rlen == 0) a.state[tid] = ST_COMMIT;
+      const bool surv = cand && ok && rlen && !killed;
+      const uint64_t sm = ballot64(surv);
+      const uint64_t acc = wave_reduce<AddOp<uint64_t>>(surv ? rlen : 0u);
+      const uint64_t cnt = ((uint64_t)__popcll(sm) << LB_ACC_BITS) | acc;
+      wsum += sw_uniform(cnt);
       if (lane == 0) {
-        a.rflag[wt] = rm;
-        a.rtcount[wt] = rc;
-      }
-    }
-    if (dbg && wt == t_lo) {
-      __builtin_amdgcn_s_waitcnt(0);
-      dbg[4] = __builtin_amdgcn_s_memrealtime();
-    }
-  }
-  if (a.kill_out) return;
-  __shared__ unsigned long long s_bs[FW][2];
-  if (lane == 0) {
-    s_bs[wv][0] = wsum;
-    s_bs[wv][1] = rsum;
-  }
-  __syncthreads();
-  if (j == 0) {
-    uint64_t t = 0, r = 0;
-    for (uint32_t w = 0; w < FW; w++) {
-      t += s_bs[w][0];
-      r += s_bs[w][1];
-    }
-    a.bsum[blockIdx.x] = t;
-    if (a.ro_split) a.rbsum[blockIdx.x] = r;
+        a.sflag[wt] = sm;
+        a.tcount[wt] = cnt;
+      }
+      if (a.ro_split) {
+        const uint64_t rm = ballot64(surv && ro);
+        const uint64_t racc = wave_reduce<AddOp<uint64_t>>(surv && ro ? rlen : 0u);
+        const uint64_t rc = ((uint64_t)__popcll(rm) << LB_ACC_BITS) | racc;
+        rsum += sw_uniform(rc);
+        if (lane == 0) {
+          a.rflag[wt] = rm;
+          a.rtcount[wt] = rc;
+        }
+      }
+      if (dbg && wt == t_lo) {
+        __builtin_amdgcn_s_waitcnt(0);
+        dbg[4] = __builtin_amdgcn_s_memrealtime();
+      }
+    }
+    if (!a.kill_out) {
+      if (lane == 0) {
+        s_bs[wv][0] = wsum;
+        s_bs[wv][1] = rsum;
+      }
+      __syncthreads();
+      if (j == 0) {
+        uint64_t t = 0, r = 0;
+        for (uint32_t w = 0; w < FW; w++) {
+          t += s_bs[w][0];
+          r += s_bs[w][1];
+        }
+        a.bsum[c] = t;
+        if (a.ro_split) a.rbsum[c] = r;
+      }
+    }
+    c += gridDim.x;
+    if (c >= nch) break;
+    __syncthreads();
   }
   if (dbg) {
     __builtin_amdgcn_s_waitcnt(0);
@@ -1161,59 +1167,63 @@
   if (pos >= m) return;
   const uint32_t n64 = (m - pos + 63) / 64;
   const uint64_t nnz = a.in.nnz;
-  const uint32_t R = sw_tiles_per_wg(n64, gridDim.x);
-  const uint32_t t_lo = min(blockIdx.x * R, n64), t_hi = min(t_lo + R, n64);
-  uint64_t wsum = 0, rsum = 0;
-  for (uint32_t wt = t_lo + wv; wt < t_hi; wt += SW_CHUNK / 64) {
-    const uint32_t p = pos + wt * 64 + lane;
-    uint64_t kw = 0;
-    for (uint32_t r = 0; r < a.kill_ranks; r++) kw |= a.kill_in[r * a.kill_stride + wt];
-    const bool kill = (kw >> lane) & 1ull;
-    bool surv = false, ro = false;
-    uint32_t len = 0;
-    if (p < m) {
-      const uint32_t tid = a.in.tid ? a.in.tid[p] : p;
-      const bool cand = a.cand_state ? a.state[p] == ST_UNDECIDED : true;
-      const uint32_t s = (uint32_t)min((uint64_t)a.in.off[p], nnz);
-      const uint32_t e = (uint32_t)min((uint64_t)a.in.off[p + 1], nnz);
-      len = e > s ? e - s : 0u;
-      if (cand && kill) a.state[tid] = ST_ABORT;
-      surv = cand && !kill;
-      ro = a.ro_split && a.hasw[tid] == 0;
-    }
-    const uint64_t sm = ballot64(surv);
-    const uint64_t acc = wave_reduce<AddOp<uint64_t>>(surv ? len : 0u);
-    const uint64_t cnt = ((uint64_t)__popcll(sm) << LB_ACC_BITS) | acc;
-    wsum += cnt;
+  const uint32_t R = sw_chunk_tiles(n64, a.nblocks);
+  const uint32_t nch = (n64 + R - 1) / R;
+  __shared__ unsigned long long s_bs[SW_CHUNK / 64][2];
+  for (uint32_t c = blockIdx.x; c < nch; c += gridDim.x) {
+    if (c != blockIdx.x) __syncthreads();
+    const uint32_t t_lo = c * R, t_hi = min(t_lo + R, n64);
+    uint64_t wsum = 0, rsum = 0;
+    for (uint32_t wt = t_lo + wv; wt < t_hi; wt += SW_CHUNK / 64) {
+      const uint32_t p = pos + wt * 64 + lane;
+      uint64_t kw = 0;
+      for (uint32_t r = 0; r < a.kill_ranks; r++) kw |= a.kill_in[r * a.kill_stride + wt];
+      const bool kill = (kw >> lane) & 1ull;
+      bool surv = false, ro = false;
+      uint32_t len = 0;
+      if (p < m) {
+        const uint32_t tid = a.in.tid ? a.in.tid[p] : p;
+        const bool cand = a.cand_state ? a.state[p] == ST_UNDECIDED : true;
+        const uint32_t s = (uint32_t)min((uint64_t)a.in.off[p], nnz);
+        const uint32_t e = (uint32_t)min((uint64_t)a.in.off[p + 1], nnz);
+        len = e > s ? e - s : 0u;
+        if (cand && kill) a.state[tid] = ST_ABORT;
+        surv = cand && !kill;
+        ro = a.ro_split && a.hasw[tid] == 0;
+      }
+      const uint64_t sm = ballot64(surv);
+      const uint64_t acc = wave_reduce<AddOp<uint64_t>>(surv ? len : 0u);
+      const uint64_t cnt = ((uint64_t)__popcll(sm) << LB_ACC_BITS) | acc;
+      wsum += cnt;
+      if (lane == 0) {
+        a.sflag[wt] = sm;
+        a.tcount[wt] = cnt;
+      }
+      if (a.ro_split) {
+        const uint64_t rm = ballot64(surv && ro);
+        const uint64_t racc = wave_reduce<AddOp<uint64_t>>(surv && ro ? len : 0u);
+        const uint64_t rc = ((uint64_t)__popcll(rm) << LB_ACC_BITS) | racc;
+        rsum += rc;
+        if (lane == 0) {
+          a.rflag[wt] = rm;
+          a.rtcount[wt] = rc;
+        }
+      }
+    }
     if (lane == 0) {
-      a.sflag[wt] = sm;
-      a.tcount[wt] = cnt;
-    }
-    if (a.ro_split) {
-      const uint64_t rm = ballot64(surv && ro);
-      const uint64_t racc = wave_reduce<AddOp<uint64_t>>(surv && ro ? len : 0u);
-      const uint64_t rc = ((uint64_t)__popcll(rm) << LB_ACC_BITS) | racc;
-      rsum += rc;
-      if (lane == 0) {
-        a.rflag[wt] = rm;
-        a.rtcount[wt] = rc;
-      }
-    }
-  }
-  __shared__ unsigned long long s_bs[SW_CHUNK / 64][2];
-  if (lane == 0) {
-    s_bs[wv][0] = wsum;
-    s_bs[wv][1] = rsum;
-  }
-  __syncthreads();
-  if (threadIdx.x == 0) {
-    uint64_t t = 0, r = 0;
-    for (uint32_t w = 0; w < SW_CHUNK / 64; w++) {
-      t += s_bs[w][0];
-      r += s_bs[w][1];
-    }
-    a.bsum[blockIdx.x] = t;
-    if (a.ro_split) a.rbsum[blockIdx.x] = r;
+      s_bs[wv][0] = wsum;
+      s_bs[wv][1] = rsum;
+    }
+    __syncthreads();
+    if (threadIdx.x == 0) {
+      uint64_t t = 0, r = 0;
+      for (uint32_t w = 0; w < SW_CHUNK / 64; w++) {
+        t += s_bs[w][0];
+        r += s_bs[w][1];
+      }
+      a.bsum[c] = t;
+      if (a.ro_split) a.rbsum[c] = r;
+    }
   }
 }
 
@@ -1345,173 +1355,187 @@
   if (pos >= m) return;
   const uint32_t n64 = (m - pos + 63) / 64;
   const uint64_t nnz = a.in.nnz;
-  const uint32_t R = sw_tiles_per_wg(n64, a.nblocks);
-  const uint32_t t_lo = min(blockIdx.x * R, n64), t_hi = min(t_lo + R, n64);
-  if (t_lo >= t_hi && blockIdx.x) return;
-  uint64_t* dbg = (a.cdbg && blockIdx.x == 0 && threadIdx.x == 0) ? a.cdbg : nullptr;
-  if (dbg) dbg[0] = __builtin_amdgcn_s_memrealtime();
-  __shared__ unsigned long long s_tb[SW_CMP_MAXR];
+  const uint32_t R = sw_chunk_tiles(n64, a.nblocks);
+  const uint32_t nch = (n64 + R - 1) / R;
+  static_assert(SW_CHUNK_TILES_MAX == 64, "one lane of wave 0 per tile base");
+  __shared__ unsigned long long s_tb[SW_CHUNK_TILES_MAX];
   __shared__ unsigned long long s_part[SW_CHUNK / 64][4];
   __shared__ uint32_t s_split, s_rnext;
-  if (R > SW_CMP_MAXR) {
-    if (threadIdx.x == 0) atomicOr(a.err, ERR_TILE);
-    return;
-  }
-  {
-    uint64_t pre = 0, all = 0, rpre = 0, rall = 0;
-    constexpr uint32_t TU = 4;
-    for (uint32_t q0 = threadIdx.x; q0 < a.nblocks; q0 += SW_CHUNK * TU) {
-      uint64_t v[TU], r[TU];
-#pragma unroll
-      for (uint32_t u = 0; u < TU; u++) {
-        const uint32_t q = q0 + u * SW_CHUNK;
-        v[u] = q < a.nblocks ? a.bsum[q] : 0ull;
-        r[u] = (a.ro_split && q < a.nblocks) ? a.rbsum[q] : 0ull;
-      }
-#pragma unroll
-      for (uint32_t u = 0; u < TU; u++) {
-        const uint32_t q = q0 + u * SW_CHUNK;
-        all += v[u];
-        rall += r[u];
-        if (q < blockIdx.x) {
-          pre += v[u];
-          rpre += r[u];
-        }
-      }
-    }
-    pre = wave_reduce<AddOp<uint64_t>>(pre);
-    all = wave_reduce<AddOp<uint64_t>>(all);
-    rpre = wave_reduce<AddOp<uint64_t>>(rpre);
-    rall = wave_reduce<AddOp<uint64_t>>(rall);
-    if (lane == 0) {
-      s_part[wv][0] = pre;
-      s_part[wv][1] = all;
-      s_part[wv][2] = rpre;
-      s_part[wv][3] = rall;
-    }
-    __syncthreads();
-    if (threadIdx.x == 0) {
-      uint64_t p0 = 0, a0 = 0, rp = 0, ra = 0;
-      for (uint32_t w = 0; w < SW_CHUNK / 64; w++) {
-        p0 += s_part[w][0];
-        a0 += s_part[w][1];
-        rp += s_part[w][2];
-        ra += s_part[w][3];
-      }
-      const uint32_t tot = (uint32_t)(a0 >> LB_ACC_BITS);
-      const uint32_t in_n = m - pos;
-      const bool handoff =
-          tot > a.abandon_min && (uint64_t)tot * a.abandon_den > (uint64_t)in_n * a.abandon_num;
-      const bool split = a.ro_split && !handoff;
-      s_split = split ? 1u : 0u;
-      s_part[0][0] = split ? p0 - rp : p0;
-      s_rnext = (uint32_t)(rp >> LB_ACC_BITS);
-      if (blockIdx.x == 0) {
-        const uint64_t keep = split ? a0 - ra : a0;
-        const uint32_t kt = (uint32_t)(keep >> LB_ACC_BITS);
-        const uint64_t acc = keep & ((1ull << LB_ACC_BITS) - 1);
-        a.lv_next->m = kt;
-        a.lv_next->acc = (uint32_t)acc;
-        a.off_out[kt] = (uint32_t)acc;
-        if (a.ro_split) *a.ro_count = split ? (uint32_t)(ra >> LB_ACC_BITS) : 0u;
-        if (handoff) atomicMax(a.abandon_out, a.level + 1);
-      }
-    }
-    __syncthreads();
-  }
-  const bool split = s_split != 0;
-  if (dbg) dbg[1] = __builtin_amdgcn_s_memrealtime();
-  if (wv == 0) {
+  uint32_t c = blockIdx.x;
+  if (c >= nch) return;
+  uint64_t* dbg = (a.cdbg && c == 0 && threadIdx.x == 0) ? a.cdbg : nullptr;
+  if (dbg) dbg[0] = __builtin_amdgcn_s_memrealtime();
+  uint64_t p0 = 0, rp = 0, all0 = 0, rall0 = 0;
+  bool handoff = false;
+  uint32_t c_done = 0;
+  for (bool first = true;; first = false) {
+    {
+      const uint32_t hi = first ? nch : c;
+      uint64_t pre = 0, all = 0, rpre = 0, rall = 0;
+      constexpr uint32_t TU = 4;
+      for (uint32_t q0 = c_done + threadIdx.x; q0 < hi; q0 += SW_CHUNK * TU) {
+        uint64_t v[TU], r[TU];
+#pragma unroll
+        for (uint32_t u = 0; u < TU; u++) {
+          const uint32_t q = q0 + u * SW_CHUNK;
+          v[u] = q < hi ? a.bsum[q] : 0ull;
+          r[u] = (a.ro_split && q < hi) ? a.rbsum[q] : 0ull;
+        }
+#pragma unroll
+        for (uint32_t u = 0; u < TU; u++) {
+          const uint32_t q = q0 + u * SW_CHUNK;
+          all += v[u];
+          rall += r[u];
+          if (q < c) {
+            pre += v[u];
+            rpre += r[u];
+          }
+        }
+      }
+      pre = wave_reduce<AddOp<uint64_t>>(pre);
+      all = wave_reduce<AddOp<uint64_t>>(all);
+      rpre = wave_reduce<AddOp<uint64_t>>(rpre);
+      rall = wave_reduce<AddOp<uint64_t>>(rall);
+      if (lane == 0) {
+        s_part[wv][0] = pre;
+        s_part[wv][1] = all;
+        s_part[wv][2] = rpre;
+        s_part[wv][3] = rall;
+      }
+      __syncthreads();
+      if (threadIdx.x == 0) {
+        uint64_t a0 = 0, ra = 0;
+        for (uint32_t w = 0; w < SW_CHUNK / 64; w++) {
+          p0 += s_part[w][0];
+          a0 += s_part[w][1];
+          rp += s_part[w][2];
+          ra += s_part[w][3];
+        }
+        if (first) {
+          all0 = a0;
+          rall0 = ra;
+          const uint32_t tot = (uint32_t)(a0 >> LB_ACC_BITS);
+          const uint32_t in_n = m - pos;
+          handoff = tot > a.abandon_min && (uint64_t)tot * a.abandon_den > (uint64_t)in_n * a.abandon_num;
+          s_split = (a.ro_split && !handoff) ? 1u : 0u;
+        }
+        if (c == 0) {
+          const bool split = s_split != 0;
+          const uint64_t keep = split ? all0 - rall0 : all0;
+          const uint32_t kt = (uint32_t)(keep >> LB_ACC_BITS);
+          const uint64_t acc = keep & ((1ull << LB_ACC_BITS) - 1);
+          a.lv_next->m = kt;
+          a.lv_next->acc = (uint32_t)acc;
+          a.off_out[kt] = (uint32_t)acc;
+          if (a.ro_split) *a.ro_count = split ? (uint32_t)(rall0 >> LB_ACC_BITS) : 0u;
+          if (handoff) atomicMax(a.abandon_out, a.level + 1);
+        }
+        s_part[0][0] = s_split ? p0 - rp : p0;
+        s_rnext = (uint32_t)(rp >> LB_ACC_BITS);
+      }
+      __syncthreads();
+    }
+    const bool split = s_split != 0;
+    if (dbg) dbg[1] = __builtin_amdgcn_s_memrealtime();
+    const uint32_t t_lo = c * R, t_hi = min(t_lo + R, n64);
     uint64_t run = s_part[0][0];
-    for (uint32_t c0 = t_lo; c0 < t_hi; c0 += 64) {
-      const uint32_t q = c0 + lane;
-      const uint64_t v = (q < t_hi ? a.tcount[q] : 0ull) - ((split && q < t_hi) ? a.rtcount[q] : 0ull);
-      uint64_t tot;
-      const uint64_t ex = wave_excl<AddOp<uint64_t>>(v, tot);
-      if (q < t_hi) s_tb[q - t_lo] = run + ex;
-      run += tot;
-    }
-  }
-  __syncthreads();
-  if (dbg) dbg[2] = __builtin_amdgcn_s_memrealtime();
-  constexpr uint32_t CB = 4;
-  for (uint32_t w0 = t_lo + wv; w0 < t_hi; w0 += FW * CB) {
-    uint64_t wordv[CB], rwordv[CB];
-    uint32_t sv[CB], ev[CB], tv[CB];
-#pragma unroll
-    for (uint32_t i = 0; i < CB; i++) {
-      const uint32_t wt = w0 + FW * i;
-      const uint32_t pc = min(pos + min(wt, n64 - 1) * 64 + lane, m - 1);
-      wordv[i] = wt < t_hi ? a.sflag[wt] : 0ull;
-      rwordv[i] = (split && wt < t_hi) ? a.rflag[wt] : 0ull;
-      sv[i] = a.in.off[pc];
-      ev[i] = a.in.off[pc + 1];
-      tv[i] = a.in.tid ? a.in.tid[pc] : pc;
-    }
-#pragma unroll
-    for (uint32_t i = 0; i < CB; i++) {
-      const uint32_t wt = w0 + FW * i;
-      const uint64_t rword = rwordv[i];
-      const uint64_t word = wordv[i] & ~rword;
-      if (rword) {
-        uint32_t rb = 0;
-        if (lane == 0) rb = atomicAdd(&s_rnext, (uint32_t)__popcll(rword));
-        rb = __shfl(rb, 0);
-        if ((rword >> lane) & 1ull) {
-          const uint32_t rs = (uint32_t)min((uint64_t)sv[i], nnz);
-          a.ro_out[rb + (uint32_t)__popcll(rword & lanemask_lt())] =
-              RoEnt{tv[i], rs, max(rs, (uint32_t)min((uint64_t)ev[i], nnz)), 0u};
-        }
-      }
-      if (!word) continue;
-      const uint64_t base = s_tb[wt - t_lo];
-      const uint32_t tb = (uint32_t)(base >> LB_ACC_BITS);
-      const uint32_t abase = (uint32_t)(base & ((1ull << LB_ACC_BITS) - 1));
-      const bool surv = (word >> lane) & 1ull;
-      uint32_t s = 0, len = 0;
-      if (surv) {
-        s = (uint32_t)min((uint64_t)sv[i], nnz);
-        len = (uint32_t)min((uint64_t)ev[i], nnz) - s;
-      }
-      uint32_t atot;
-      const uint32_t aex = wave_excl<AddOp<uint32_t>>(len, atot);
-      if (surv) {
-        const uint32_t r = tb + (uint32_t)__popcll(word & lanemask_lt());
-        a.tid_out[r] = tv[i];
-        a.off_out[r] = abase + aex;
-      }
-      const uint32_t incl = aex + len;
-      for (uint32_t q0 = 0; q0 < atot; q0 += 64 * 4) {
-        uint32_t src[4];
-        bool in[4];
-#pragma unroll
-        for (uint32_t r = 0; r < 4; r++) {
-          const uint32_t q = q0 + 64 * r + lane;
-          uint32_t lo = 0;
-#pragma unroll
-          for (uint32_t st = 32; st > 0; st >>= 1) {
-            const uint32_t v = __shfl(incl, lo + st - 1);
-            if (v <= q) lo += st;
+    for (uint32_t b_lo = t_lo; b_lo < t_hi; b_lo += SW_CHUNK_TILES_MAX) {
+      const uint32_t b_hi = min(b_lo + SW_CHUNK_TILES_MAX, t_hi);
+      if (b_lo != t_lo) __syncthreads();
+      if (wv == 0) {
+        const uint32_t q = b_lo + lane;
+        const uint64_t v = (q < b_hi ? a.tcount[q] : 0ull) - ((split && q < b_hi) ? a.rtcount[q] : 0ull);
+        uint64_t tot;
+        const uint64_t ex = wave_excl<AddOp<uint64_t>>(v, tot);
+        if (q < b_hi) s_tb[lane] = run + ex;
+        run += tot;
+      }
+      __syncthreads();
+      if (dbg) dbg[2] = __builtin_amdgcn_s_memrealtime();
+      constexpr uint32_t CB = 4;
+      for (uint32_t w0 = b_lo + wv; w0 < b_hi; w0 += FW * CB) {
+        uint64_t wordv[CB], rwordv[CB];
+        uint32_t sv[CB], ev[CB], tv[CB];
+#pragma unroll
+        for (uint32_t i = 0; i < CB; i++) {
+          const uint32_t wt = w0 + FW * i;
+          const uint32_t pc = min(pos + min(wt, n64 - 1) * 64 + lane, m - 1);
+          wordv[i] = wt < b_hi ? a.sflag[wt] : 0ull;
+          rwordv[i] = (split && wt < b_hi) ? a.rflag[wt] : 0ull;
+          sv[i] = a.in.off[pc];
+          ev[i] = a.in.off[pc + 1];
+          tv[i] = a.in.tid ? a.in.tid[pc] : pc;
+        }
+#pragma unroll
+        for (uint32_t i = 0; i < CB; i++) {
+          const uint32_t wt = w0 + FW * i;
+          const uint64_t rword = rwordv[i];
+          const uint64_t word = wordv[i] & ~rword;
+          if (rword) {
+            uint32_t rb = 0;
+            if (lane == 0) rb = atomicAdd(&s_rnext, (uint32_t)__popcll(rword));
+            rb = __shfl(rb, 0);
+            if ((rword >> lane) & 1ull) {
+              const uint32_t rs = (uint32_t)min((uint64_t)sv[i], nnz);
+              a.ro_out[rb + (uint32_t)__popcll(rword & lanemask_lt())] =
+                  RoEnt{tv[i], rs, max(rs, (uint32_t)min((uint64_t)ev[i], nnz)), 0u};
+            }
           }
-          in[r] = q < atot;
-          src[r] = __shfl(s, lo) + (q - __shfl(aex, lo));
-        }
-        uint64_t kk[4];
-        uint8_t aa[4];
-#pragma unroll
-        for (uint32_t r = 0; r < 4; r++) {
-          kk[r] = in[r] ? a.in.keys[src[r]] : 0ull;
-          aa[r] = in[r] ? a.in.acctype[src[r]] : (uint8_t)0;
-        }
-#pragma unroll
-        for (uint32_t r = 0; r < 4; r++) {
-          if (!in[r]) continue;
-          const uint32_t q = q0 + 64 * r + lane;
-          a.keys_out[abase + q] = kk[r];
-          a.acc_out[abase + q] = aa[r];
-        }
-      }
-    }
+          if (!word) continue;
+          const uint64_t base = s_tb[wt - b_lo];
+          const uint32_t tb = (uint32_t)(base >> LB_ACC_BITS);
+          const uint32_t abase = (uint32_t)(base & ((1ull << LB_ACC_BITS) - 1));
+          const bool surv = (word >> lane) & 1ull;
+          uint32_t s = 0, len = 0;
+          if (surv) {
+            s = (uint32_t)min((uint64_t)sv[i], nnz);
+            len = (uint32_t)min((uint64_t)ev[i], nnz) - s;
+          }
+          uint32_t atot;
+          const uint32_t aex = wave_excl<AddOp<uint32_t>>(len, atot);
+          if (surv) {
+            const uint32_t r = tb + (uint32_t)__popcll(word & lanemask_lt());
+            a.tid_out[r] = tv[i];
+            a.off_out[r] = abase + aex;
+          }
+          const uint32_t incl = aex + len;
+          for (uint32_t q0 = 0; q0 < atot; q0 += 64 * 4) {
+            uint32_t src[4];
+            bool in[4];
+#pragma unroll
+            for (uint32_t r = 0; r < 4; r++) {
+              const uint32_t q = q0 + 64 * r + lane;
+              uint32_t lo = 0;
+#pragma unroll
+              for (uint32_t st = 32; st > 0; st >>= 1) {
+                const uint32_t v = __shfl(incl, lo + st - 1);
+                if (v <= q) lo += st;
+              }
+              in[r] = q < atot;
+              src[r] = __shfl(s, lo) + (q - __shfl(aex, lo));
+            }
+            uint64_t kk[4];
+            uint8_t aa[4];
+#pragma unroll
+            for (uint32_t r = 0; r < 4; r++) {
+              kk[r] = in[r] ? a.in.keys[src[r]] : 0ull;
+              aa[r] = in[r] ? a.in.acctype[src[r]] : (uint8_t)0;
+            }
+#pragma unroll
+            for (uint32_t r = 0; r < 4; r++) {
+              if (!in[r]) continue;
+              const uint32_t q = q0 + 64 * r + lane;
+              a.keys_out[abase + q] = kk[r];
+              a.acc_out[abase + q] = aa[r];
+            }
+          }
+        }
+      }
+    }
+    c_done = c;
+    c += gridDim.x;
+    if (c >= nch) break;
+    __syncthreads();
   }
   if (dbg) {
     __builtin_amdgcn_s_waitcnt(0);
diff --git a/include/dcc.h b/include/dcc.h
--- a/include/dcc.h
+++ b/include/dcc.h
@@ -96,6 +96,7 @@
 #define DCC_OPT_COMM_SOLO 13
 #define DCC_OPT_PIPE_PARTITION 14
 #define DCC_OPT_PIPE_CHAIN 15
+#define DCC_OPT_SWEEP_GRID 16
 int dcc_set_option(dcc_ctx* ctx, int option, int64_t value);
 int dcc_reserve(dcc_ctx* ctx, uint64_t max_txn, uint64_t max_nnz);
 int dcc_copy_bandwidth(dcc_ctx* ctx, uint64_t bytes, int reps, double* gbps);
```

New measurement: 5.884 billion txns/s. 5.7% lower.
